# kensho-technologies/pyctcdecode

Measured on AMD Instinct MI355X. Metric: logit-frames/sec (whole node) at beam=100, V=1024, 4-gram LM, higher is better.
Workload: dtype f64

## Files before the change

### include/ctcdec.h

```cpp
#ifndef CTCDEC_H
#define CTCDEC_H

#include <stddef.h>
#include <stdint.h>

#ifdef __cplusplus
extern "C" {
#endif

typedef struct ctcdec_decoder ctcdec_decoder;
typedef struct ctcdec_result ctcdec_result;

enum ctcdec_status {
  CTCDEC_OK = 0,
  CTCDEC_ERR_ARG = -1,
  CTCDEC_ERR_IO = -2,
  CTCDEC_ERR_DEVICE = -3,
  CTCDEC_ERR_LIMIT = -4,
  CTCDEC_ERR_INTERNAL = -5
};

enum ctcdec_dtype { CTCDEC_F32 = 0, CTCDEC_F64 = 1, CTCDEC_F16 = 2, CTCDEC_BF16 = 3 };

#define CTCDEC_MAX_BEAM_WIDTH 256
#define CTCDEC_MAX_LM_ORDER 6
#define CTCDEC_MAX_VOCAB 65535
#define CTCDEC_MAX_LMS 4

typedef struct ctcdec_params {
  int32_t beam_width;
  int32_t prune_history;
  int32_t n_best;
  int32_t want_lm_state;
  double beam_prune_logp;
  double token_min_logp;
  double hotword_weight;
  double alpha;
  double beta;
  double unk_score_offset;
  double log_base_change;
  int32_t lm_score_boundary;
  int32_t first_frame;
  int32_t texts_only;
  int32_t token_frames;
} ctcdec_params;

enum ctcdec_token_logp { CTCDEC_TOKEN_LOGP_MEAN = 2, CTCDEC_TOKEN_LOGP_MIN = 3, CTCDEC_TOKEN_LOGP_MAX = 4 };

typedef struct ctcdec_lm_state {
  int32_t length;
  uint32_t words[CTCDEC_MAX_LM_ORDER - 1];
  float backoff[CTCDEC_MAX_LM_ORDER - 1];
} ctcdec_lm_state;

int ctcdec_create(const char* labels_blob, const int64_t* labels_off, int32_t n_labels,
                  int32_t is_bpe, int32_t device, ctcdec_decoder** out);
void ctcdec_destroy(ctcdec_decoder* dec);

int ctcdec_lm_load_arpa(ctcdec_decoder* dec, const char* path, int32_t* order_out);

int ctcdec_lm_save_flat(const ctcdec_decoder* dec, const char* path);
int ctcdec_lm_load_flat(ctcdec_decoder* dec, const char* path, int32_t* order_out);

int ctcdec_lm_load_kenlm(ctcdec_decoder* dec, const char* path, int32_t* order_out);
int ctcdec_is_kenlm_binary(const char* path);
int ctcdec_arpa_to_kenlm_binary(const char* arpa_path, const char* out_path, float probing_multiplier);

int ctcdec_lm_set_unigrams(ctcdec_decoder* dec, int32_t has_unigrams, const char* blob,
                           const int64_t* off, int64_t n_unigrams, int64_t* n_kept_out);

int ctcdec_lm_share(ctcdec_decoder* dst, const ctcdec_decoder* src);

int ctcdec_lm_clone(ctcdec_decoder* dst, const ctcdec_decoder* src);

int ctcdec_lm_share_multi(ctcdec_decoder* dst, const ctcdec_decoder* const* srcs, int32_t n);
int ctcdec_lm_set_params(ctcdec_decoder* dec, int32_t k , double alpha, double beta,
                         double unk_score_offset, int32_t lm_score_boundary);
int ctcdec_lm_count(const ctcdec_decoder* dec, int32_t* n_out);

int ctcdec_lm_prefix_flags(const ctcdec_decoder* dec, const char* str_utf8, int64_t len,
                           uint32_t* flags_out);

int ctcdec_lm_word_index(const ctcdec_decoder* dec, const char* word_utf8, int64_t len,
                         uint32_t* index_out);
int ctcdec_lm_word_string(const ctcdec_decoder* dec, uint32_t index, const char** str_out,
                          int64_t* len_out);

int ctcdec_lm_start_state(const ctcdec_decoder* dec, int32_t begin_sentence, ctcdec_lm_state* out);
int ctcdec_lm_base_score(const ctcdec_decoder* dec, const ctcdec_lm_state* in, uint32_t word_index,
                         ctcdec_lm_state* out, float* log10_prob_out);

int ctcdec_set_hotwords(ctcdec_decoder* dec, const char* blob, const int64_t* off, int64_t n_words);

int ctcdec_set_hotword_sets(ctcdec_decoder* dec, const char* blob, const int64_t* off, int64_t n_words,
                            const int64_t* set_off, int32_t n_sets, const double* set_weight,
                            const int32_t* utt_set, int32_t n_utts);

int ctcdec_decode_batch(ctcdec_decoder* dec, const void* const* utt_logits,
                        const int32_t* utt_frames, int32_t n_utts, int32_t dtype, int32_t is_device,
                        const ctcdec_params* params, const ctcdec_lm_state* start_states,
                        ctcdec_result** out);

typedef struct ctcdec_beam_in {
  double logit_score;
  double raw_lm_score;
  ctcdec_lm_state lm_state;
  int32_t last_char;
  int32_t partial_start;
  int32_t partial_end_frame;
  int32_t reserved;
  int64_t text_begin, text_end;
  int64_t partial_begin, partial_end;
  const ctcdec_lm_state* more_states;
} ctcdec_beam_in;
int ctcdec_decode_stream_batch(ctcdec_decoder* dec, const void* const* utt_logits,
                               const int32_t* utt_frames, int32_t n_streams, int32_t dtype,
                               int32_t is_device, const ctcdec_params* params,
                               const int32_t* first_frame ,
                               const ctcdec_beam_in* beams, const int64_t* beam_off ,
                               const char* text_blob, int32_t force_next_word, int32_t is_end,
                               ctcdec_result** out);

typedef struct ctcdec_stream ctcdec_stream;
int ctcdec_stream_open(ctcdec_decoder* dec, int32_t n_streams, const ctcdec_lm_state* start_states, ctcdec_stream** out);
int ctcdec_stream_push(ctcdec_stream* st, const void* const* chunk_logits, const int32_t* chunk_frames, int32_t dtype,
                       int32_t is_device, const ctcdec_params* params, const int32_t* first_frame,
                       int32_t force_next_word, int32_t is_end, int32_t want_result, ctcdec_result** out);
int ctcdec_stream_read(ctcdec_stream* st, const ctcdec_params* params, ctcdec_result** out);
int ctcdec_stream_import(ctcdec_stream* st, const ctcdec_beam_in* beams, const int64_t* beam_off ,
                         const char* text_blob, int64_t text_bytes);
int ctcdec_stream_frames(const ctcdec_stream* st, int64_t* frames_out);
int ctcdec_stream_ledger_bytes(const ctcdec_stream* st, int64_t* bytes_out);
void ctcdec_stream_close(ctcdec_stream* st);

int32_t ctcdec_result_num_utts(const ctcdec_result* r);
int32_t ctcdec_result_num_beams(const ctcdec_result* r, int32_t utt);
int ctcdec_result_text(const ctcdec_result* r, int32_t utt, int32_t beam, const char** str_out,
                       int64_t* len_out);
int ctcdec_result_scores(const ctcdec_result* r, int32_t utt, int32_t beam, double* logit_score,
                         double* lm_score);
int ctcdec_result_frames(const ctcdec_result* r, int32_t utt, int32_t beam, int32_t* n_words,
                         const int32_t** word_off, const int32_t** start, const int32_t** end);
int ctcdec_result_lm_state(const ctcdec_result* r, int32_t utt, int32_t beam, ctcdec_lm_state* out);
int ctcdec_result_lm_state_of(const ctcdec_result* r, int32_t utt, int32_t beam, int32_t k,
                              ctcdec_lm_state* out);
typedef struct ctcdec_packed {
  int64_t n_utts, n_beams, n_words;
  const int64_t* beam_off;
  const char* text_blob;
  const int64_t* text_off;
  const double* logit_score;
  const double* lm_score;
  const int64_t* word_cnt_off;
  const int32_t* word_byte_off;
  const int32_t* word_start;
  const int32_t* word_end;
  const ctcdec_lm_state* lm_state;
  const char* partial_blob;
  const int64_t* partial_off;
  const int32_t* src_beam;
  const int32_t* last_char;
  const int32_t* partial_start;
  const int32_t* partial_end;
  const double* raw_lm_score;
} ctcdec_packed;
int ctcdec_result_pack(ctcdec_result* r, ctcdec_packed* out);
int ctcdec_result_texts(ctcdec_result* r, const char** blob_out, const int64_t** off_out, int64_t* n_out);
int ctcdec_result_texts_joined(ctcdec_result* r, char sep, const char** blob_out, int64_t* bytes_out, int64_t* n_out);
int ctcdec_result_text_blocks(ctcdec_result* r, const char** pool_out, const int64_t** off_out, const int64_t** len_out,
                              int64_t* n_out);

int ctcdec_result_token_frames(ctcdec_result* r, const int64_t** tok_off, const int32_t** label, const int32_t** start,
                               const int32_t** end, int64_t* n_tokens);

int ctcdec_result_token_logp(ctcdec_result* r, const double** logp, int64_t* n_tokens);

typedef struct ctcdec_alignment ctcdec_alignment;
int ctcdec_align_batch(ctcdec_decoder* dec, const void* const* utt_logits, const int32_t* utt_frames, int32_t n_utts,
                       int32_t dtype, int32_t is_device, const int32_t* targets, const int64_t* target_off, int32_t fold,
                       int64_t bp_budget, ctcdec_alignment** out);
int ctcdec_alignment_paths(const ctcdec_alignment* a, const int64_t** path_off, const int32_t** path, const double** score,
                           int64_t* n_utts);
int ctcdec_alignment_tokens(const ctcdec_alignment* a, const int64_t** tok_off, const int32_t** label, const int32_t** start,
// ... 23 lines not shown
```

### pyctcdecode_amd/_binding.py

```python
from __future__ import annotations

import ctypes as C
import os
from typing import List, Optional, Sequence

import numpy as np

_HERE = os.path.dirname(os.path.abspath(__file__))
LIB_PATH = os.path.join(_HERE, "libctcdec.so")

MAX_CTX = 5


class Params(C.Structure):
    _fields_ = [
        ("beam_width", C.c_int32),
        ("prune_history", C.c_int32),
        ("n_best", C.c_int32),
        ("want_lm_state", C.c_int32),
        ("beam_prune_logp", C.c_double),
        ("token_min_logp", C.c_double),
        ("hotword_weight", C.c_double),
        ("alpha", C.c_double),
        ("beta", C.c_double),
        ("unk_score_offset", C.c_double),
        ("log_base_change", C.c_double),
        ("lm_score_boundary", C.c_int32),
        ("first_frame", C.c_int32),
        ("texts_only", C.c_int32),
        ("token_frames", C.c_int32),
    ]


class LmState(C.Structure):
    _fields_ = [("length", C.c_int32), ("words", C.c_uint32 * MAX_CTX), ("backoff", C.c_float * MAX_CTX)]


class Packed(C.Structure):
    _fields_ = [
        ("n_utts", C.c_int64),
        ("n_beams", C.c_int64),
        ("n_words", C.c_int64),
        ("beam_off", C.POINTER(C.c_int64)),
        ("text_blob", C.c_void_p),
        ("text_off", C.POINTER(C.c_int64)),
        ("logit_score", C.POINTER(C.c_double)),
        ("lm_score", C.POINTER(C.c_double)),
        ("word_cnt_off", C.POINTER(C.c_int64)),
        ("word_byte_off", C.POINTER(C.c_int32)),
        ("word_start", C.POINTER(C.c_int32)),
        ("word_end", C.POINTER(C.c_int32)),
        ("lm_state", C.POINTER(LmState)),
        ("partial_blob", C.c_void_p),
        ("partial_off", C.POINTER(C.c_int64)),
        ("src_beam", C.POINTER(C.c_int32)),
        ("last_char", C.POINTER(C.c_int32)),
        ("partial_start", C.POINTER(C.c_int32)),
        ("partial_end", C.POINTER(C.c_int32)),
        ("raw_lm_score", C.POINTER(C.c_double)),
    ]


class BeamIn(C.Structure):
    _fields_ = [
        ("logit_score", C.c_double),
        ("raw_lm_score", C.c_double),
        ("lm_state", LmState),
        ("last_char", C.c_int32),
        ("partial_start", C.c_int32),
        ("partial_end_frame", C.c_int32),
        ("reserved", C.c_int32),
        ("text_begin", C.c_int64),
        ("text_end", C.c_int64),
        ("partial_begin", C.c_int64),
        ("partial_end", C.c_int64),
        ("more_states", C.POINTER(LmState)),
    ]


_VP = C.c_void_p
_PROTOS = {
    "ctcdec_create": (C.c_int, [C.c_char_p, C.POINTER(C.c_int64), C.c_int32, C.c_int32, C.c_int32, C.POINTER(_VP)]),
    "ctcdec_destroy": (None, [_VP]),
    "ctcdec_lm_load_arpa": (C.c_int, [_VP, C.c_char_p, C.POINTER(C.c_int32)]),
    "ctcdec_lm_save_flat": (C.c_int, [_VP, C.c_char_p]),
    "ctcdec_lm_load_flat": (C.c_int, [_VP, C.c_char_p, C.POINTER(C.c_int32)]),
    "ctcdec_lm_load_kenlm": (C.c_int, [_VP, C.c_char_p, C.POINTER(C.c_int32)]),
    "ctcdec_is_kenlm_binary": (C.c_int, [C.c_char_p]),
    "ctcdec_arpa_to_kenlm_binary": (C.c_int, [C.c_char_p, C.c_char_p, C.c_float]),
    "ctcdec_lm_set_unigrams": (C.c_int, [_VP, C.c_int32, C.c_char_p, C.POINTER(C.c_int64), C.c_int64,
                                         C.POINTER(C.c_int64)]),
    "ctcdec_lm_share": (C.c_int, [_VP, _VP]),
    "ctcdec_lm_clone": (C.c_int, [_VP, _VP]),
    "ctcdec_lm_share_multi": (C.c_int, [_VP, C.POINTER(_VP), C.c_int32]),
    "ctcdec_lm_set_params": (C.c_int, [_VP, C.c_int32, C.c_double, C.c_double, C.c_double, C.c_int32]),
    "ctcdec_lm_count": (C.c_int, [_VP, C.POINTER(C.c_int32)]),
    "ctcdec_lm_prefix_flags": (C.c_int, [_VP, C.c_char_p, C.c_int64, C.POINTER(C.c_uint32)]),
    "ctcdec_lm_word_index": (C.c_int, [_VP, C.c_char_p, C.c_int64, C.POINTER(C.c_uint32)]),
    "ctcdec_lm_word_string": (C.c_int, [_VP, C.c_uint32, C.POINTER(_VP), C.POINTER(C.c_int64)]),
    "ctcdec_lm_start_state": (C.c_int, [_VP, C.c_int32, C.POINTER(LmState)]),
    "ctcdec_lm_base_score": (C.c_int, [_VP, C.POINTER(LmState), C.c_uint32, C.POINTER(LmState),
                                       C.POINTER(C.c_float)]),
    "ctcdec_set_hotwords": (C.c_int, [_VP, C.c_char_p, C.POINTER(C.c_int64), C.c_int64]),
    "ctcdec_set_hotword_sets": (C.c_int, [_VP, C.c_char_p, C.POINTER(C.c_int64), C.c_int64, C.POINTER(C.c_int64), C.c_int32,
                                          C.POINTER(C.c_double), C.POINTER(C.c_int32), C.c_int32]),
    "ctcdec_decode_batch": (C.c_int, [_VP, C.POINTER(_VP), C.POINTER(C.c_int32), C.c_int32, C.c_int32, C.c_int32,
                                      C.POINTER(Params), C.POINTER(LmState), C.POINTER(_VP)]),
    "ctcdec_decode_stream_batch": (C.c_int, [_VP, C.POINTER(_VP), C.POINTER(C.c_int32), C.c_int32, C.c_int32, C.c_int32,
                                             C.POINTER(Params), C.POINTER(C.c_int32), C.POINTER(BeamIn),
                                             C.POINTER(C.c_int64), C.c_char_p, C.c_int32, C.c_int32, C.POINTER(_VP)]),
    "ctcdec_stream_open": (C.c_int, [_VP, C.c_int32, C.POINTER(LmState), C.POINTER(_VP)]),
    "ctcdec_stream_push": (C.c_int, [_VP, C.POINTER(_VP), C.POINTER(C.c_int32), C.c_int32, C.c_int32, C.POINTER(Params),
                                     C.POINTER(C.c_int32), C.c_int32, C.c_int32, C.c_int32, C.POINTER(_VP)]),
    "ctcdec_stream_read": (C.c_int, [_VP, C.POINTER(Params), C.POINTER(_VP)]),
    "ctcdec_stream_import": (C.c_int, [_VP, C.POINTER(BeamIn), C.POINTER(C.c_int64), C.c_char_p, C.c_int64]),
    "ctcdec_stream_frames": (C.c_int, [_VP, C.POINTER(C.c_int64)]),
    "ctcdec_stream_ledger_bytes": (C.c_int, [_VP, C.POINTER(C.c_int64)]),
    "ctcdec_stream_close": (None, [_VP]),
    "ctcdec_result_num_utts": (C.c_int32, [_VP]),
    "ctcdec_result_num_beams": (C.c_int32, [_VP, C.c_int32]),
    "ctcdec_result_text": (C.c_int, [_VP, C.c_int32, C.c_int32, C.POINTER(_VP), C.POINTER(C.c_int64)]),
    "ctcdec_result_scores": (C.c_int, [_VP, C.c_int32, C.c_int32, C.POINTER(C.c_double), C.POINTER(C.c_double)]),
    "ctcdec_result_frames": (C.c_int, [_VP, C.c_int32, C.c_int32, C.POINTER(C.c_int32),
                                       C.POINTER(C.POINTER(C.c_int32)), C.POINTER(C.POINTER(C.c_int32)),
                                       C.POINTER(C.POINTER(C.c_int32))]),
    "ctcdec_result_lm_state": (C.c_int, [_VP, C.c_int32, C.c_int32, C.POINTER(LmState)]),
    "ctcdec_frame_survivors": (C.c_int, [_VP, _VP, C.c_int32, C.c_int32, C.c_int32, C.c_double, C.c_int32,
                                         C.POINTER(C.c_int32), C.POINTER(C.c_int32), C.POINTER(C.c_double)]),
    "ctcdec_result_lm_state_of": (C.c_int, [_VP, C.c_int32, C.c_int32, C.c_int32, C.POINTER(LmState)]),
    "ctcdec_result_pack": (C.c_int, [_VP, C.POINTER(Packed)]),
    "ctcdec_result_texts": (C.c_int, [_VP, C.POINTER(C.c_void_p), C.POINTER(C.POINTER(C.c_int64)), C.POINTER(C.c_int64)]),
    "ctcdec_result_texts_joined": (C.c_int, [_VP, C.c_char, C.POINTER(C.c_void_p), C.POINTER(C.c_int64), C.POINTER(C.c_int64)]),
    "ctcdec_result_text_blocks": (C.c_int, [_VP, C.POINTER(C.c_void_p), C.POINTER(C.POINTER(C.c_int64)),
                                           C.POINTER(C.POINTER(C.c_int64)), C.POINTER(C.c_int64)]),
    "ctcdec_result_token_frames": (C.c_int, [_VP, C.POINTER(C.POINTER(C.c_int64)), C.POINTER(C.POINTER(C.c_int32)),
                                            C.POINTER(C.POINTER(C.c_int32)), C.POINTER(C.POINTER(C.c_int32)),
                                            C.POINTER(C.c_int64)]),
    "ctcdec_result_token_logp": (C.c_int, [_VP, C.POINTER(C.POINTER(C.c_double)), C.POINTER(C.c_int64)]),
    "ctcdec_align_batch": (C.c_int, [_VP, C.POINTER(_VP), C.POINTER(C.c_int32), C.c_int32, C.c_int32, C.c_int32,
                                     C.POINTER(C.c_int32), C.POINTER(C.c_int64), C.c_int32, C.c_int64, C.POINTER(_VP)]),
    "ctcdec_alignment_paths": (C.c_int, [_VP, C.POINTER(C.POINTER(C.c_int64)), C.POINTER(C.POINTER(C.c_int32)),
                                         C.POINTER(C.POINTER(C.c_double)), C.POINTER(C.c_int64)]),
    "ctcdec_alignment_tokens": (C.c_int, [_VP, C.POINTER(C.POINTER(C.c_int64)), C.POINTER(C.POINTER(C.c_int32)),
                                          C.POINTER(C.POINTER(C.c_int32)), C.POINTER(C.POINTER(C.c_int32)),
                                          C.POINTER(C.POINTER(C.c_double)), C.POINTER(C.c_int64)]),
    "ctcdec_alignment_timing": (C.c_int, [_VP, C.POINTER(C.c_double), C.POINTER(C.c_int32)]),
    "ctcdec_alignment_free": (None, [_VP]),
    "ctcdec_result_timing": (C.c_int, [_VP, C.POINTER(C.c_double)]),
    "ctcdec_result_beam_kernel": (C.c_int, [_VP]),
    "ctcdec_device": (C.c_int, []),
    "ctcdec_result_free": (None, [_VP]),
    "ctcdec_profile_phases": (C.c_int, [_VP, C.c_int32, C.POINTER(C.c_uint64), C.c_int32]),
    "ctcdec_last_error": (C.c_char_p, []),
    "ctcdec_version": (C.c_char_p, []),
}
MAX_BEAM_WIDTH = 256
EXPORTED_SYMBOLS = tuple(_PROTOS)


class NativeError(RuntimeError):
    pass


class Library:

    def __init__(self, path: str = LIB_PATH):
        if not os.path.exists(path):
            raise ImportError(
                "%s is missing: build the HIP extension first (python -c 'import __graft_entry__ as g; "
                "g.build()'). pyctcdecode_amd has no CPU fallback." % path
            )
        self.path = path
        try:
            import torch
        except ImportError:
            pass
        self.dll = C.CDLL(path)
        for name, (res, args) in _PROTOS.items():
            fn = getattr(self.dll, name)
            fn.restype = res
            fn.argtypes = args

    def check(self, rc: int) -> None:
        if rc == 0:
            return
        msg = (self.dll.ctcdec_last_error() or b"").decode("utf-8", "replace")
        if rc == -1:
            raise ValueError(msg)
        if rc == -2:
            raise OSError(msg)
        if rc == -4:
            raise NotImplementedError(msg)
        raise NativeError("libctcdec error %d: %s" % (rc, msg))


_LIB: Optional[Library] = None
_PYTEXTS = None


def _pytexts():
    global _PYTEXTS
    if _PYTEXTS is None:
        path = os.path.join(_HERE, "_pytexts.so")
        _PYTEXTS = False
        if os.path.exists(path):
            try:
                dll = C.PyDLL(path)
                dll.ctcdec_py_split_texts.restype = C.py_object
                dll.ctcdec_py_split_texts.argtypes = [C.c_void_p, C.c_int64, C.c_int64, C.c_char]
                dll.ctcdec_py_texts_from_blocks.restype = C.py_object
                dll.ctcdec_py_texts_from_blocks.argtypes = [C.c_void_p, C.POINTER(C.c_int64), C.POINTER(C.c_int64), C.c_int64]
                dll.ctcdec_py_output_beams.restype = C.py_object
                dll.ctcdec_py_output_beams.argtypes = [C.py_object, C.c_int64, C.POINTER(C.c_int64), C.POINTER(C.c_int64), C.c_void_p,
                                                       C.POINTER(C.c_double), C.POINTER(C.c_double), C.POINTER(C.c_int64),
                                                       C.POINTER(C.c_int32), C.POINTER(C.c_int32), C.py_object, C.py_object]
                dll.ctcdec_py_lm_beams.restype = C.py_object
                dll.ctcdec_py_lm_beams.argtypes = [C.py_object, C.c_int64, C.POINTER(C.c_int64), C.POINTER(C.c_int64), C.c_void_p,
                                                   C.POINTER(C.c_int64), C.c_void_p, C.POINTER(C.c_int32), C.py_object,
                                                   C.POINTER(C.c_int64), C.POINTER(C.c_int32), C.POINTER(C.c_int32),
                                                   C.POINTER(C.c_int32), C.POINTER(C.c_int32), C.POINTER(C.c_double),
                                                   C.POINTER(C.c_double), C.py_object]
                _PYTEXTS = dll
            except (OSError, AttributeError):
                _PYTEXTS = False
    return _PYTEXTS


def texts_of(lib: "Library", res) -> Optional[list]:
    dll = _pytexts()
    if not dll:
        return None
    pool, off, ln, n = C.c_void_p(), C.POINTER(C.c_int64)(), C.POINTER(C.c_int64)(), C.c_int64()
    lib.check(lib.dll.ctcdec_result_text_blocks(res, C.byref(pool), C.byref(off), C.byref(ln), C.byref(n)))
    if n.value == 0:
        return []
    return dll.ctcdec_py_texts_from_blocks(pool, off, ln, n.value)


def output_beams(cls, pk: "Packed", states: Optional[list], frames_of=None) -> Optional[list]:
    dll = _pytexts()
    if not dll:
        return None
    return dll.ctcdec_py_output_beams(cls, pk.n_utts, pk.beam_off, pk.text_off, pk.text_blob, pk.logit_score, pk.lm_score,
                                      pk.word_cnt_off, pk.word_start, pk.word_end, states, frames_of)


def lm_beams(cls, n_streams: int, pk: "Packed", labels: list, frames_of=None) -> Optional[list]:
    dll = _pytexts()
    if not dll:
        return None
    return dll.ctcdec_py_lm_beams(cls, n_streams, pk.beam_off, pk.text_off, pk.text_blob, pk.partial_off, pk.partial_blob,
                                  pk.last_char, labels, pk.word_cnt_off, pk.word_start, pk.word_end, pk.partial_start,
                                  pk.partial_end, pk.logit_score, pk.lm_score, frames_of)


def split_texts(blob_ptr, nbytes: int, n: int, sep: bytes):
    dll = _pytexts()
    if dll:
        return dll.ctcdec_py_split_texts(blob_ptr, nbytes, n, sep)
    return C.string_at(blob_ptr, nbytes).decode("utf-8").split(sep.decode("ascii"))


def get_library() -> Library:
    global _LIB
    if _LIB is None:
        _LIB = Library()
    return _LIB


def pack_strings(strings: Sequence[str]):
    enc = [s.encode("utf-8") for s in strings]
    off = np.zeros(len(enc) + 1, dtype=np.int64)
    if enc:
        off[1:] = np.cumsum([len(e) for e in enc])
    blob = b"".join(enc)
    return blob, off


def off_ptr(off: np.ndarray):
    return off.ctypes.data_as(C.POINTER(C.c_int64))
```

### pyctcdecode_amd/csrc/api.cpp

```cpp
#include <math.h>
#include <cmath>
#include <stdio.h>
#include <stdlib.h>
#include <string.h>

#include <algorithm>
#include <atomic>
#include <chrono>
#include <condition_variable>
#include <functional>
#include <mutex>
#include <memory>
#include <string>
#include <thread>
#include <utility>
#include <vector>

#include "../../include/ctcdec.h"
#include "backend.h"
#include "beam_core.h"
#include "beam_wave.h"
#include "host_tables.h"

using namespace ctc;

static thread_local std::string g_err;
static std::mutex g_device_mu;
static int fail(int code, const std::string& msg) {
  g_err = msg;
  return code;
}

namespace {

template <bool HOST>
struct Buf {
  void* p = nullptr;
  size_t cap = 0;
  Buf() = default;
  Buf(const Buf&) = delete;
  Buf& operator=(const Buf&) = delete;
  Buf(Buf&& o) noexcept : p(std::exchange(o.p, nullptr)), cap(std::exchange(o.cap, 0)) {}
  Buf& operator=(Buf&& o) noexcept {
    std::swap(p, o.p);
    std::swap(cap, o.cap);
    return *this;
  }
  ~Buf() { drop(); }
  int ensure(size_t bytes, std::string* err) {
    if (bytes <= cap && p) return 0;
    drop();
    const size_t want = HOST ? bytes + bytes / 4 + 4096 : bytes + bytes / 8 + 256;
    p = HOST ? be::alloc_host(want, err) : be::alloc(want, err);
    if (!p) return -1;
    cap = want;
    return 0;
  }
  void drop() {
    if (p) HOST ? be::release_host(p) : be::release(p);
    p = nullptr;
    cap = 0;
  }
};
using DevBuf = Buf<false>;
using HostBuf = Buf<true>;

template <class T>
int upload(DevBuf& b, const std::vector<T>& v, std::string* err) {
  size_t bytes = std::max<size_t>(sizeof(T) * v.size(), 16);
  if (b.ensure(bytes, err)) return -1;
  if (!v.empty() && be::h2d(b.p, v.data(), sizeof(T) * v.size(), err)) return -1;
  return 0;
}

struct BeamResult {
  std::string text;
  std::vector<int32_t> word_off, start, end;
  double logit = 0, lm = 0;
  ctcdec_lm_state state;
  std::vector<ctcdec_lm_state> xstates;
  std::string partial;
  int32_t src = -1, last_char = -1, pstart = -1, pend = -1;
  double raw_lm = 0;
  std::vector<int32_t> tok;
};

struct StreamIn {
  const int32_t* first_frame;
  const ctcdec_beam_in* beams;
  const int64_t* beam_off;
  const char* text_blob;
  int32_t fold, eos;
};

}

class ReplayPool {
 public:
  explicit ReplayPool(int n) {
    for (int i = 0; i < n; ++i) workers_.emplace_back([this] { loop(); });
  }
  ~ReplayPool() {
    {
      std::lock_guard<std::mutex> g(m_);
      stop_ = true;
    }
    cv_.notify_all();
    for (auto& t : workers_) t.join();
  }
  int size() const { return (int)workers_.size(); }
  void run(int32_t n, int32_t chunk, const std::function<void(int32_t, int32_t)>& fn) {
    {
      std::lock_guard<std::mutex> g(m_);
      fn_ = &fn;
      n_ = n;
      chunk_ = chunk;
      next_.store(0);
      pending_ = (int)workers_.size();
      ++epoch_;
    }
    cv_.notify_all();
    work();
    std::unique_lock<std::mutex> g(m_);
    done_.wait(g, [this] { return pending_ == 0; });
    fn_ = nullptr;
  }

 private:
  void work() {
    for (;;) {
      int32_t u0 = next_.fetch_add(chunk_);
      if (u0 >= n_) return;
      (*fn_)(u0, std::min(n_, u0 + chunk_));
    }
  }
  void loop() {
    uint64_t seen = 0;
    for (;;) {
      {
        std::unique_lock<std::mutex> g(m_);
        cv_.wait(g, [&] { return stop_ || epoch_ != seen; });
        if (stop_) return;
        seen = epoch_;
      }
      work();
      {
        std::lock_guard<std::mutex> g(m_);
        if (--pending_ == 0) done_.notify_one();
      }
    }
  }
  std::vector<std::thread> workers_;
  std::mutex m_;
  std::condition_variable cv_, done_;
  const std::function<void(int32_t, int32_t)>* fn_ = nullptr;
  std::atomic<int32_t> next_{0};
  int32_t n_ = 0, chunk_ = 1;
  int pending_ = 0;
  uint64_t epoch_ = 0;
  bool stop_ = false;
};

struct ctcdec_decoder {
  std::unique_ptr<ReplayPool> replay_pool;
  HostAlphabet alpha;
  std::shared_ptr<HostLM> lm_ptr = std::make_shared<HostLM>();
  HostLM& lm_ref() { return *lm_ptr; }
  const HostLM& lm_ref() const { return *lm_ptr; }
  bool has_lm = false;
  std::unique_ptr<HostMulti> multi;
  double x_alpha[MAX_LMS] = {0}, x_beta[MAX_LMS] = {0}, x_unk[MAX_LMS] = {0};
  int32_t x_boundary[MAX_LMS] = {0};
  int n_lms() const { return multi ? (int)multi->lms.size() : 1; }
  int hist_order() const { return multi ? multi->order : lm_ptr->order; }
  HostHotwords hot;
  bool tables_dirty = true, hot_dirty = true;
  struct HotSets {
    bool armed = false;
    std::vector<std::vector<std::string>> words;
    std::vector<double> weight;
    std::vector<int32_t> utt_set;
    bool built = false;
    std::vector<HostHotwords> sets;
  };
  HotSets hot_next, hot_call;
  DevBuf d_hsets, d_htab, d_htok, d_hutt;
  HostBuf h_hot;
  DevBuf d_tok, d_tok_hot, d_uni, d_pref, d_hot;
  DevBuf d_xuni[MAX_LMS - 1], d_winfo[MAX_LMS], w_xstate, w_impx;
  HostBuf h_xstate;
  DevBuf w_logits, w_ptrs, w_row0, w_rowsum, w_isprob, w_scnt, w_sid, w_slp, w_flags, w_text, w_emit, w_toff,
      w_eoff, w_start, w_out, w_nout, w_status, w_tok, w_head, w_prof, w_imp, w_impoff, w_ff, w_cold, w_pay, w_tscr, w_tsoff, w_tpool,
      d_toktext, d_tokbytes, w_slow, w_order, w_side, w_truns, w_tlogp, w_tmiss, w_ledrow;
  DevBuf w_alse, w_alab, w_apath, w_atok, w_atlp, w_ascore, w_abp, w_autts;
  bool slicing = false;
  uint32_t max_label_bytes = 1;
  bool arenas_worst_case = false;
  HostBuf h_tok, h_out, h_small, h_truns;
  int dense_calls = 0;
  HostBuf h_stage;
  size_t stage_used = 0;
  bool profile = false;
  unsigned long long prof[N_PROF] = {0};
};

template <class T>
static int upload_staged(ctcdec_decoder* dec, DevBuf& b, const std::vector<T>& v, std::string* err) {
  const size_t bytes = sizeof(T) * v.size();
  const size_t room = dec->h_stage.p ? dec->h_stage.cap - dec->stage_used : 0;
  if (bytes == 0 || bytes > room) return upload(b, v, err);
  if (b.ensure(std::max<size_t>(bytes, 16), err)) return -1;
  char* src = (char*)dec->h_stage.p + dec->stage_used;
  memcpy(src, v.data(), bytes);
  dec->stage_used += (bytes + 63) & ~(size_t)63;
  return be::h2d_async(b.p, src, bytes, err);
}

struct HotCallScope {
  ctcdec_decoder* dec;
  explicit HotCallScope(ctcdec_decoder* d) : dec(d) {
    if (!dec) return;
    dec->hot_call = std::move(dec->hot_next);
    dec->hot_next = ctcdec_decoder::HotSets();
  }
  ~HotCallScope() {
    if (dec) dec->hot_call = ctcdec_decoder::HotSets();
  }
};

static void build_hot_sets(ctcdec_decoder::HotSets& h) {
  if (h.built) return;
  h.sets.resize(h.words.size());
  for (size_t k = 0; k < h.words.size(); ++k) h.sets[k].build_table(h.words[k]);
  bool none = false;
  for (int32_t& s : h.utt_set) {
    if (s < 0) {
      s = (int32_t)h.words.size();
      none = true;
    }
  }
  if (none) {
    h.sets.emplace_back();
    h.weight.push_back(0.0);
  }
  h.built = true;
}

static const HostHotwords& import_hot(const ctcdec_decoder* dec, int64_t u) {
  const ctcdec_decoder::HotSets& h = dec->hot_call;
  return h.armed ? h.sets[(size_t)h.utt_set[(size_t)u]] : dec->hot;
}

static int upload_hot_sets(ctcdec_decoder* dec, be::BeamArgs* ba, std::string* err) {
  ctcdec_decoder::HotSets& h = dec->hot_call;
  build_hot_sets(h);
  const size_t K = h.sets.size(), V = dec->alpha.labels.size(), n = h.utt_set.size();
  std::vector<size_t> toff(K + 1, 0);
  for (size_t k = 0; k < K; ++k) toff[k + 1] = toff[k] + h.sets[k].table.size();
  const size_t b_sets = K * sizeof(HotSet), b_utt = n * sizeof(int32_t), b_tab = toff[K] * sizeof(HotEntry);
  const size_t o_utt = (b_sets + 63) & ~(size_t)63, o_tab = (o_utt + b_utt + 63) & ~(size_t)63;
  if (dec->d_hsets.ensure(std::max<size_t>(b_sets, 16), err) || dec->d_hutt.ensure(std::max<size_t>(b_utt, 16), err) ||
      dec->d_htab.ensure(std::max<size_t>(b_tab, 16), err) || dec->d_htok.ensure(std::max<size_t>(K * V * sizeof(TokHot), 16), err) ||
      dec->h_hot.ensure(o_tab + b_tab + 64, err))
    return -1;
  char* stage = (char*)dec->h_hot.p;
  HotSet* hs = (HotSet*)stage;
  for (size_t k = 0; k < K; ++k) {
    const HostHotwords& w = h.sets[k];
    hs[k].hot = w.table.empty() ? nullptr : (const HotEntry*)dec->d_htab.p + toff[k];
    hs[k].hot_mask = w.mask;
    hs[k].tok_hot = (const TokHot*)dec->d_htok.p + k * V;
    hs[k].weight = h.weight[k];
    if (!w.table.empty()) memcpy(stage + o_tab + toff[k] * sizeof(HotEntry), w.table.data(), w.table.size() * sizeof(HotEntry));
  }
  memcpy(stage + o_utt, h.utt_set.data(), b_utt);
  if (be::h2d_async(dec->d_hsets.p, stage, b_sets, err) || be::h2d_async(dec->d_hutt.p, stage + o_utt, b_utt, err) ||
      (b_tab && be::h2d_async(dec->d_htab.p, stage + o_tab, b_tab, err)))
    return -1;
  ba->hot_sets = (const HotSet*)dec->d_hsets.p;
  ba->utt_hot = (const int32_t*)dec->d_hutt.p;
  ba->n_hot_sets = (int32_t)K;
  return 0;
}

// ... 421 lines not shown
        if (br != BR_APPEND && opener != NONE) {
          tk[opener * 3 + 1] = toks[k].wstart;
          opener = NONE;
        }
        if (br == BR_BOUNDARY || br == BR_APPEND) {
          last = tk.size() / 3;
          if (br == BR_BOUNDARY) opener = last;
          tk.push_back((int32_t)tok);
          tk.push_back(br == BR_APPEND ? toks[k].wstart - 1 : -1);
          tk.push_back(-1);
        }
      }
    }
    if (br == BR_BOUNDARY) {
      close_word(toks[k].wstart, toks[k].wend, true);
      text += d->alpha.clean[tok];
    } else if (br == BR_SPACE) {
      close_word(toks[k].wstart, toks[k].wend, true);
    } else if (br == BR_APPEND) {
      text += d->alpha.labels[tok];
    } else if (br == BR_FINAL) {
      close_word(toks[k].wstart, toks[k].wend, true);
    } else if (br == BR_IMPORT && st) {
      const ctcdec_beam_in& in = st->beams[imp0 + tok];
      r->src = (int32_t)tok;
      text.assign(st->text_blob + in.text_begin, (size_t)(in.text_end - in.text_begin));
      if (!text.empty()) text.push_back(' ');
      open = text.size();
      text.append(st->text_blob + in.partial_begin, (size_t)(in.partial_end - in.partial_begin));
    }
  }
  if (want_tok) {
    if (last != NONE) tk[last * 3 + 2] = open_e;
    if (opener != NONE) tk[opener * 3 + 1] = open_s;
  }
  r->partial.assign(text, open, std::string::npos);
  text.resize(open);
  if (!text.empty() && text.back() == ' ') text.pop_back();
  r->word_off.push_back((int32_t)text.size());
}

static void fill_result(const OutBeam& ob, const LmState* xs, int K, BeamResult* r) {
  r->logit = ob.logit_score;
  r->lm = ob.lm_score;
  export_lm_state(ob.state, &r->state);
  if (xs) {
    r->xstates.resize((size_t)(K - 1));
    for (int x = 0; x < K - 1; ++x) export_lm_state(xs[x], &r->xstates[(size_t)x]);
  }
  r->last_char = ob.last_char == NO_CHAR ? -1 : (int32_t)ob.last_char;
  r->pstart = ob.pstart;
  r->pend = ob.pend;
  r->raw_lm = ob.raw_lm;
}

static_assert(LOGP_MEAN == CTCDEC_TOKEN_LOGP_MEAN && LOGP_MIN == CTCDEC_TOKEN_LOGP_MIN && LOGP_MAX == CTCDEC_TOKEN_LOGP_MAX, "token_logp.h");
static int32_t logp_fold(const ctcdec_params* p) {
  return p && p->token_frames >= LOGP_MEAN && p->token_frames <= LOGP_MAX ? p->token_frames : 0;
}

using Clock = std::chrono::steady_clock;
static double ms(Clock::time_point a, Clock::time_point b) { return std::chrono::duration<double, std::milli>(b - a).count(); }
static size_t dtype_size(int32_t dtype) { return dtype == CTCDEC_F32 ? 4 : dtype == CTCDEC_F64 ? 8 : 2; }

enum LmStateErr { LM_STATE_OK = 0, LM_STATE_LENGTH, LM_STATE_WORD };
static LmStateErr copy_lm_state(const ctcdec_lm_state& in, size_t n_words, LmState* out) {
  memset(out, 0, sizeof(*out));
  if (in.length < 0 || in.length > MAX_CTX) return LM_STATE_LENGTH;
  out->len = in.length;
  for (int j = 0; j < out->len; ++j) {
    if (in.words[j] >= n_words) return LM_STATE_WORD;
    out->words[j] = in.words[j];
    out->backoff[j] = in.backoff[j];
  }
  return LM_STATE_OK;
}

typedef std::function<int(std::string*)> AfterLaunch;
struct DecodeMode {
  const StreamIn* stream = nullptr;
  ctcdec_stream* rs = nullptr;
  bool want_result = true;
  const AfterLaunch* after_launch = nullptr;
};
static int decode_impl(ctcdec_decoder* dec, const void* const* utt_logits, const int32_t* utt_frames, int32_t n_utts,
                       int32_t dtype, int32_t is_device, const ctcdec_params* p, const ctcdec_lm_state* start_states,
                       const DecodeMode& mode, ctcdec_result** out);
static int decode_host_sliced(ctcdec_decoder* dec, const void* const* utt_logits, const int32_t* utt_frames, int32_t n_utts,
                              int32_t dtype, const ctcdec_params* p, const ctcdec_lm_state* start_states, int n_slices,
                              ctcdec_result** out);
static int host_slices_wanted(const ctcdec_decoder* dec, const int32_t* utt_frames, int32_t n_utts, int32_t dtype);

int ctcdec_decode_batch(ctcdec_decoder* dec, const void* const* utt_logits, const int32_t* utt_frames,
                        int32_t n_utts, int32_t dtype, int32_t is_device, const ctcdec_params* p,
                        const ctcdec_lm_state* start_states, ctcdec_result** out) {
  HotCallScope hot_scope(dec);
  if (dec && p && out && !is_device && !dec->hot_call.armed && !logp_fold(p) && n_utts > 0 && utt_logits && utt_frames && dtype >= CTCDEC_F32 && dtype <= CTCDEC_BF16) {
    const int n_slices = host_slices_wanted(dec, utt_frames, n_utts, dtype);
    if (n_slices >= 2) {
      const int rc = decode_host_sliced(dec, utt_logits, utt_frames, n_utts, dtype, p, start_states, n_slices, out);
      if (rc != 1) return rc;
    }
  }
  return decode_impl(dec, utt_logits, utt_frames, n_utts, dtype, is_device, p, start_states, DecodeMode(), out);
}

int ctcdec_decode_stream_batch(ctcdec_decoder* dec, const void* const* utt_logits, const int32_t* utt_frames,
                               int32_t n_streams, int32_t dtype, int32_t is_device, const ctcdec_params* p,
                               const int32_t* first_frame, const ctcdec_beam_in* beams, const int64_t* beam_off,
                               const char* text_blob, int32_t force_next_word, int32_t is_end, ctcdec_result** out) {
  if (!first_frame || !beams || !beam_off || !text_blob) return fail(CTCDEC_ERR_ARG, "bad arguments");
  const StreamIn st{first_frame, beams, beam_off, text_blob, (force_next_word || is_end) ? 1 : 0, is_end ? 1 : 0};
  HotCallScope hot_scope(dec);
  return decode_impl(dec, utt_logits, utt_frames, n_streams, dtype, is_device, p, nullptr, DecodeMode{&st}, out);
}

static std::string build_import(const ctcdec_decoder* dec, const StreamIn& st, int64_t k, ImportBeam* m,
                                LmState* more , const HostHotwords& hot) {
  const ctcdec_beam_in& in = st.beams[k];
  memset(m, 0, sizeof(*m));
  if (in.text_end < in.text_begin || in.partial_end < in.partial_begin) return "bad beam text range";
  const char* t = st.text_blob + in.text_begin;
  const size_t tn = (size_t)(in.text_end - in.text_begin);
  const uint32_t n_hist = dec->has_lm ? (uint32_t)std::max(1, dec->hist_order() - 1) : 1u;
  uint64_t th = 0;
  std::vector<uint64_t> wh;
  uint32_t hw = 0;
  size_t a = 0;
  while (a < tn) {
    while (a < tn && t[a] == ' ') ++a;
    size_t b = a;
    while (b < tn && t[b] != ' ') ++b;
    if (b > a) {
      uint64_t h = hash_bytes(t + a, b - a);
      th = text_push(th, h);
      wh.push_back(h);
      uint32_t ml = 0, cp = 0;
      if (!hot.table.empty() && hot_lookup(hot.table.data(), hot.mask, h, &ml, &cp) && cp) ++hw;
    }
    a = b;
  }
  m->text_h = th;
  m->hw_cnt = hw;
  m->ring_cnt = (uint32_t)std::min<size_t>(n_hist, wh.size());
  for (uint32_t j = 0; j < m->ring_cnt; ++j) m->ring[j] = wh[wh.size() - 1 - j];
  const char* pp = st.text_blob + in.partial_begin;
  const size_t pn = (size_t)(in.partial_end - in.partial_begin);
  m->part_h = hash_bytes(pp, pn);
  m->plen = utf8_length(pp, pn);
  if (m->plen > 0xFFFF) return "partial word too long";
  uint32_t m2 = 0, wid = 0;
  if (pn > 0) {
    uint32_t fl = 0, w = 0;
    const std::vector<PrefixEntry>& ptab = dec->multi ? dec->multi->prefix_table : dec->lm_ref().prefix_table;
    const uint64_t pmask = dec->multi ? dec->multi->prefix_mask : dec->lm_ref().prefix_mask;
    if (dec->has_lm && prefix_lookup(ptab.data(), pmask, m->part_h, &w, &fl)) {
      m2 |= PF_ON_TABLE | (fl & PF_PARTIAL_MASK);
      wid = w;
    }
    uint32_t ml = 0, cp = 0;
    if (!hot.table.empty() && hot_lookup(hot.table.data(), hot.mask, m->part_h, &ml, &cp))
      m2 |= M2_HOT_ON | (cp ? M2_HOT_COMPLETE : 0u) | ((ml & 0xFFFFu) << 8);
  }
  m->m2 = m2;
  m->word_id = wid;
  if (in.last_char >= (int32_t)dec->alpha.labels.size()) return "last_char out of range";
  m->last_char = in.last_char < 0 ? NO_CHAR : (uint32_t)in.last_char;
  m->pstart = in.partial_start;
  m->pend = in.partial_end_frame;
  m->logit_score = in.logit_score;
  m->raw_lm = dec->has_lm ? in.raw_lm_score : 0.0;
  const char* const bad_state[] = {nullptr, "bad LM state in beam", "bad LM state word in beam"};
  if (dec->has_lm) {
    if (const LmStateErr e = copy_lm_state(in.lm_state, dec->lm_ref().words.size(), &m->state)) return bad_state[e];
  }
  if (dec->multi) {
    if (!in.more_states) return "beam lacks the states of the further language models";
    for (int x = 1; x < dec->n_lms(); ++x)
      if (const LmStateErr e = copy_lm_state(in.more_states[x - 1], dec->multi->lms[(size_t)x]->words.size(), &more[x - 1]))
        return bad_state[e];
  }
  return "";
}


struct PruneStage {
  ctcdec_decoder* dec = nullptr;
  const std::vector<const void*>* ptrs = nullptr;
  int32_t n_utts = 0, dtype = 0;
  int64_t R = 0;
  int V = 0;
  double token_min_logp = 0;
  bool resident = false;
  int max_surv = 0;
  uint32_t flags[8] = {0, 0, 0, 0, 0, 0, 0, 0};
  uint32_t surv_total = 0;
  Clock::time_point t_setup, t_queued, t_flags;
};

struct DecodeCall : DecodeMode {
  ctcdec_decoder* dec = nullptr;
  const ctcdec_params* p = nullptr;
  const void* const* utt_logits = nullptr;
  const int32_t* utt_frames = nullptr;
  const ctcdec_lm_state* start_states = nullptr;
  ctcdec_result** out = nullptr;
  int32_t n_utts = 0, dtype = 0, is_device = 0, fold = 0;
  int V = 0, K = 1, B = 0, n_best = 0;
  int64_t R = 0;
  std::vector<int64_t> row0;
  std::vector<const void*> ptrs;
  std::vector<uint64_t> toff, eoff;
  bool arenas_full = false;
  unsigned long long tok_cap = 0;
  size_t xstate_bytes = 0;
  bool device_texts = false, by_input = false, late_beam = false;
  be::BeamArgs ba{};
  PruneStage prune;
  uint32_t *n_out = nullptr, *status = nullptr;
  unsigned long long* heads_pinned = nullptr;
  unsigned long long head = 0;
  bool outgrown_redone = false;
  int32_t led = 0;
  std::vector<int64_t> led_rows;
  bool host_timing = false;
  Clock::time_point t_begin, t_launch, t_kernel, t_end;
  std::string err;
  std::unique_ptr<ctcdec_result> res;
  std::unique_lock<std::mutex> device_lock;
};

static int check_stream_tokens(DecodeCall& c) {
  const ctcdec_stream* rs = c.rs;
  if (c.p->token_frames != 0 && rs->has_import)
    return fail(CTCDEC_ERR_ARG, "token frames are not available to a stream that holds imported beams: their chains do not reach back");
  const bool first = rs->pushes == 0;
  if (c.fold && !first && rs->led_fold != c.fold)
    return fail(CTCDEC_ERR_ARG, rs->led_fold ? "a stream keeps the confidence fold its first chunk asked for"
                                             : "token confidences have to be asked for from a stream's first chunk on");
  c.led = first ? c.fold : rs->led_fold;
  if (c.led && !first)
    for (int32_t u = 0; u < c.n_utts; ++u)
      if ((int64_t)c.stream->first_frame[u] != (int64_t)rs->led_first[(size_t)u] + rs->frames[(size_t)u])
        return fail(CTCDEC_ERR_ARG, "stream " + std::to_string(u) + ": first_frame " + std::to_string(c.stream->first_frame[u]) +
                                        " does not continue the stream (token confidences: expected " +
                                        std::to_string((int64_t)rs->led_first[(size_t)u] + rs->frames[(size_t)u]) + ")");
  return CTCDEC_OK;
}

static int check_call(DecodeCall& c) {
  const ctcdec_params* p = c.p;
  if (!c.dec || !p || !c.out || c.n_utts < 0 || (c.n_utts > 0 && (!c.utt_logits || !c.utt_frames)))
    return fail(CTCDEC_ERR_ARG, "bad arguments");
  if (c.dtype < CTCDEC_F32 || c.dtype > CTCDEC_BF16) return fail(CTCDEC_ERR_ARG, "dtype must be f32, f64, f16 or bf16");
  if (p->beam_width < 1) return fail(CTCDEC_ERR_ARG, "beam_width must be >= 1");
  if (p->beam_width > CTCDEC_MAX_BEAM_WIDTH)
    return fail(CTCDEC_ERR_LIMIT, "beam_width above the supported maximum of 256");
  c.fold = logp_fold(p);
  if (c.fold && c.stream && !c.rs)
    return fail(CTCDEC_ERR_ARG, "token confidences are not available to streaming decodes whose beams the caller hands in");
  if (c.rs)
    if (int rc = check_stream_tokens(c)) return rc;
  c.t_begin = Clock::now();
  c.res.reset(new ctcdec_result());
  c.res->utts.resize((size_t)c.n_utts);
  return CTCDEC_OK;
}

static int open_call(DecodeCall& c) {
  ctcdec_decoder* dec = c.dec;
  const int32_t n_utts = c.n_utts;
  std::string& err = c.err;
  c.K = dec->has_lm ? dec->n_lms() : 1;
  if (dec->hot_call.armed) {
    if ((int32_t)dec->hot_call.utt_set.size() != n_utts) return fail(CTCDEC_ERR_ARG, "hot-word sets armed for another number of utterances");
    if (c.stream && !c.rs) build_hot_sets(dec->hot_call);
  }
  c.device_lock = std::unique_lock<std::mutex>(g_device_mu);
  if (be::bind_thread(&err)) return fail(CTCDEC_ERR_DEVICE, err);
  if (sync_tables(dec, &err)) return fail(CTCDEC_ERR_DEVICE, err);
  c.V = (int)dec->alpha.labels.size();
  c.B = c.p->beam_width;
  c.n_best = c.p->n_best > 0 ? std::min(c.p->n_best, c.B) : c.B;
  c.host_timing = getenv("CTCDEC_HOST_TIMING") != nullptr;
  dec->stage_used = 0;
  if (dec->h_stage.ensure((size_t)n_utts * (64 + sizeof(LmState) * (size_t)c.K) + 4096, &err)) return fail(CTCDEC_ERR_DEVICE, err);
  c.row0.assign((size_t)n_utts + 1, 0);
  for (int32_t u = 0; u < n_utts; ++u) {
    if (c.utt_frames[u] < 0) return fail(CTCDEC_ERR_ARG, "negative frame count");
    c.row0[(size_t)u + 1] = c.row0[(size_t)u] + c.utt_frames[u];
  }
  c.R = c.row0[(size_t)n_utts];
  return CTCDEC_OK;
}

static int stage_logits(DecodeCall& c) {
  ctcdec_decoder* dec = c.dec;
  std::string& err = c.err;
  const int32_t n_utts = c.n_utts;
  const size_t row_bytes = (size_t)c.V * dtype_size(c.dtype);
  c.ptrs.resize((size_t)n_utts);
  if (c.is_device) {
    for (int32_t u = 0; u < n_utts; ++u) c.ptrs[(size_t)u] = c.utt_logits[u];
  } else {
    if (dec->w_logits.ensure((size_t)std::max<int64_t>(c.R, 1) * row_bytes, &err)) return fail(CTCDEC_ERR_DEVICE, err);
    for (int32_t u = 0; u < n_utts;) {
      char* dst = (char*)dec->w_logits.p + (size_t)c.row0[(size_t)u] * row_bytes;
// ... 52 lines not shown
  for (int32_t u = 0; u <= n_utts; ++u) eo[(size_t)u] = (uint64_t)u * cap;
  if (upload(rs->eoff, eo, &err)) return fail(CTCDEC_ERR_DEVICE, err);
  rs->emit = std::move(grown);
  rs->emit_cap = cap;
  return CTCDEC_OK;
}

static int stage_imports(DecodeCall& c) {
  ctcdec_decoder* dec = c.dec;
  const StreamIn* stream = c.stream;
  std::string& err = c.err;
  const int32_t n_utts = c.n_utts;
  const int K = c.K;
  const int64_t n_imp_total = stream->beam_off[n_utts];
  std::vector<ImportBeam> imps((size_t)std::max<int64_t>(n_imp_total, 1));
  std::vector<LmState> imps_x(K > 1 ? (size_t)std::max<int64_t>(n_imp_total, 1) * (size_t)(K - 1) : 0);
  std::vector<int64_t> ioff(stream->beam_off, stream->beam_off + n_utts + 1);
  std::vector<int32_t> ff(stream->first_frame, stream->first_frame + n_utts);
  for (int32_t u = 0; u < n_utts; ++u) {
    int64_t cnt = ioff[(size_t)u + 1] - ioff[(size_t)u];
    if (cnt < 1 || cnt > beam_bucket(c.B))
      return fail(CTCDEC_ERR_ARG, "a stream must carry between 1 and beam-capacity beams");
    c.ba.max_import = std::max<int32_t>(c.ba.max_import, (int32_t)cnt);
    for (int64_t k = ioff[(size_t)u]; k < ioff[(size_t)u + 1]; ++k) {
      std::string e = build_import(dec, *stream, k, &imps[(size_t)k], K > 1 ? &imps_x[(size_t)k * (size_t)(K - 1)] : nullptr,
                                   import_hot(dec, u));
      if (!e.empty()) return fail(CTCDEC_ERR_ARG, e);
    }
  }
  if (upload(dec->w_imp, imps, &err) || upload(dec->w_impoff, ioff, &err) || upload(dec->w_ff, ff, &err))
    return fail(CTCDEC_ERR_DEVICE, err);
  if (K > 1 && upload(dec->w_impx, imps_x, &err)) return fail(CTCDEC_ERR_DEVICE, err);
  return CTCDEC_OK;
}

static int reserve_beam_workspace(DecodeCall& c) {
  ctcdec_decoder* dec = c.dec;
  std::string& err = c.err;
  const int32_t n_utts = c.n_utts;
  c.tok_cap = (unsigned long long)c.n_best * (unsigned long long)(c.R + 2 * (int64_t)n_utts);
  if (c.rs) {
    unsigned long long depth = 0;
    for (int32_t u = 0; u < n_utts; ++u)
      depth += (unsigned long long)(c.rs->frames[(size_t)u] + c.utt_frames[u] + c.rs->pushes + 3);
    c.tok_cap = c.want_result ? (unsigned long long)c.n_best * depth : 1ull;
  }
  if (dec->w_text.ensure(c.toff[(size_t)n_utts] * sizeof(TextNode), &err) ||
      (!c.rs && (dec->w_emit.ensure(c.eoff[(size_t)n_utts] * sizeof(EmitNode), &err) || upload_staged(dec, dec->w_eoff, c.eoff, &err))) ||
      upload_staged(dec, dec->w_toff, c.toff, &err) || dec->w_out.ensure((size_t)n_utts * c.n_best * sizeof(OutBeam), &err) ||
      dec->w_nout.ensure((size_t)n_utts * 4, &err) || dec->w_status.ensure((size_t)n_utts * 4, &err) ||
      dec->w_tok.ensure((size_t)std::max<unsigned long long>(c.tok_cap, 1) * sizeof(EmitNode), &err) ||
      dec->w_head.ensure(16, &err) || dec->w_cold.ensure((size_t)n_utts * 2 * COLD_STRIDE * sizeof(ColdRec), &err))
    return fail(CTCDEC_ERR_DEVICE, err);
  return CTCDEC_OK;
}

static int stage_start_states(DecodeCall& c) {
  ctcdec_decoder* dec = c.dec;
  const int K = c.K;
  c.xstate_bytes = K > 1 ? (size_t)c.n_utts * c.n_best * (size_t)(K - 1) * sizeof(LmState) : 0;
  if (!(c.stream && !c.rs) && dec->has_lm) {
    std::vector<LmState> st((size_t)c.n_utts * K);
    for (int32_t u = 0; u < c.n_utts; ++u) {
      for (int k = 0; k < K; ++k) {
        LmState& s = st[(size_t)u * K + k];
        const HostLM& lm = K > 1 ? *dec->multi->lms[(size_t)k] : dec->lm_ref();
        const ctcdec_lm_state* given = c.start_states ? &c.start_states[(size_t)u * K + k] : nullptr;
        if (!given || given->length < 0) {
          const bool boundary = k == 0 ? c.p->lm_score_boundary != 0 : dec->x_boundary[k] != 0;
          memset(&s, 0, sizeof(s));
          lm.start_state(boundary, &s);
        } else if (const LmStateErr e = copy_lm_state(*given, lm.words.size(), &s)) {
          return fail(CTCDEC_ERR_ARG, e == LM_STATE_LENGTH ? "LM start state too long" : "bad LM state word");
        }
      }
    }
    if (upload_staged(dec, dec->w_start, st, &c.err)) return fail(CTCDEC_ERR_DEVICE, c.err);
    c.ba.start_states = (const LmState*)dec->w_start.p;
  }
  if (c.xstate_bytes && dec->w_xstate.ensure(c.xstate_bytes, &c.err)) return fail(CTCDEC_ERR_DEVICE, c.err);
  return CTCDEC_OK;
}

static int reserve_device_texts(DecodeCall& c) {
  ctcdec_decoder* dec = c.dec;
  std::vector<uint64_t> soff((size_t)c.n_utts + 1, 0);
  for (int32_t u = 0; u < c.n_utts; ++u)
    soff[(size_t)u + 1] = soff[(size_t)u] + (((uint64_t)c.utt_frames[u] + 2) * (uint64_t)(dec->max_label_bytes + 1) + 15) / 16 * 16;
  if (dec->w_tscr.ensure((size_t)soff[(size_t)c.n_utts] + 16, &c.err) || dec->w_tpool.ensure((size_t)soff[(size_t)c.n_utts] + 16, &c.err) ||
      upload_staged(dec, dec->w_tsoff, soff, &c.err))
    return fail(CTCDEC_ERR_DEVICE, c.err);
  c.ba.text_scratch = (uint8_t*)dec->w_tscr.p;
  c.ba.text_soff = (const uint64_t*)dec->w_tsoff.p;
  c.ba.text_pool = (uint8_t*)dec->w_tpool.p;
  c.ba.text_pool_cap = soff[(size_t)c.n_utts];
  return CTCDEC_OK;
}

static int stage_longest_first(DecodeCall& c) {
  const int32_t* utt_frames = c.utt_frames;
  if (c.n_utts <= be::cus() * 2 || getenv("CTCDEC_NO_LPT_ORDER")) return CTCDEC_OK;
  bool ragged = false;
  for (int32_t u = 1; u < c.n_utts; ++u) ragged = ragged || utt_frames[u] != utt_frames[0];
  if (!ragged) return CTCDEC_OK;
  std::vector<int32_t> order((size_t)c.n_utts);
  for (int32_t u = 0; u < c.n_utts; ++u) order[(size_t)u] = u;
  std::stable_sort(order.begin(), order.end(), [&](int32_t x, int32_t y) { return utt_frames[x] > utt_frames[y]; });
  if (upload(c.dec->w_order, order, &c.err)) return fail(CTCDEC_ERR_DEVICE, c.err);
  c.ba.order = (const int32_t*)c.dec->w_order.p;
  return CTCDEC_OK;
}

static int fill_beam_args(DecodeCall& c) {
  ctcdec_decoder* dec = c.dec;
  const ctcdec_params* p = c.p;
  const StreamIn* stream = c.stream;
  ctcdec_stream* rs = c.rs;
  be::BeamArgs& ba = c.ba;
  device_tables(dec, &ba.tables);
  DecodeParams& dp = ba.params;
  memset(&dp, 0, sizeof(dp));
  dp.beam_width = c.B;
  dp.prune_history = p->prune_history ? 1 : 0;
  dp.n_best = c.n_best;
  dp.first_frame = p->first_frame;
  dp.beam_prune_logp = p->beam_prune_logp;
  dp.token_min_logp = p->token_min_logp;
  dp.hot_weight = p->hotword_weight;
  dp.alpha = p->alpha;
  dp.beta = p->beta;
  dp.unk = p->unk_score_offset;
  dp.log_base_change = p->log_base_change;
  dp.score_boundary = p->lm_score_boundary ? 1 : 0;
  dp.fold = stream ? stream->fold : 1;
  dp.eos = stream ? stream->eos : 1;
  dp.no_label_runs = getenv("CTCDEC_NO_LABEL_RUNS") != nullptr ? 1 : 0;
  c.device_texts = p->texts_only != 0 && p->token_frames == 0 && c.n_best == 1 && !stream && getenv("CTCDEC_HOST_REPLAY") == nullptr;
  dp.texts_only = c.device_texts ? 1 : 0;
  ba.n_utts = c.n_utts;
  ba.utt_row0 = (const int64_t*)dec->w_row0.p;
  ba.text_nodes = (TextNode*)dec->w_text.p;
  ba.text_off = (const uint64_t*)dec->w_toff.p;
  ba.out_xstates = c.xstate_bytes ? (LmState*)dec->w_xstate.p : nullptr;
  ba.out = (OutBeam*)dec->w_out.p;
  ba.out_stride = c.n_best;
  ba.n_out = (uint32_t*)dec->w_nout.p;
  ba.status = (uint32_t*)dec->w_status.p;
  ba.tok_pool = (EmitNode*)dec->w_tok.p;
  ba.tok_pool_head = (unsigned long long*)dec->w_head.p;
  ba.tok_pool_cap = c.tok_cap;
  ba.first_frames = stream ? (const int32_t*)dec->w_ff.p : nullptr;
  ba.cold = (ColdRec*)dec->w_cold.p;
  ba.want_out = 1;
  ba.total_rows = c.R;
  if (c.device_texts)
    if (int rc = reserve_device_texts(c)) return rc;
  if (int rc = stage_longest_first(c)) return rc;
  if (rs) {
    ba.emit_nodes = (EmitNode*)rs->emit.p;
    ba.emit_off = (const uint64_t*)rs->eoff.p;
    ba.imports = (const ImportBeam*)rs->carry.p;
    ba.import_xstates = c.K > 1 ? (const LmState*)rs->carry_x.p : nullptr;
    ba.resident_in = 1;
    ba.carry_out = (ImportBeam*)rs->carry.p;
    ba.carry_xstates = c.K > 1 ? (LmState*)rs->carry_x.p : nullptr;
    ba.sstate = (StreamState*)rs->sstate.p;
    ba.carry_stride = ctcdec_stream::CAP;
    ba.want_out = c.want_result ? 1 : 0;
  } else {
    ba.emit_nodes = (EmitNode*)dec->w_emit.p;
    ba.emit_off = (const uint64_t*)dec->w_eoff.p;
    if (stream) {
      ba.imports = (const ImportBeam*)dec->w_imp.p;
      ba.import_xstates = c.K > 1 ? (const LmState*)dec->w_impx.p : nullptr;
      ba.import_off = (const int64_t*)dec->w_impoff.p;
    }
  }
  if (dec->profile) {
    if (dec->w_prof.ensure(N_PROF * 8, &c.err) || be::zero(dec->w_prof.p, N_PROF * 8, &c.err)) return fail(CTCDEC_ERR_DEVICE, c.err);
    ba.prof = (unsigned long long*)dec->w_prof.p;
  }
  if (dec->w_flags.ensure(32, &c.err) || dec->w_head.ensure(16, &c.err)) return fail(CTCDEC_ERR_DEVICE, c.err);
  c.by_input = !rs && be::beam_kernel_depends_on_input(ba);
  c.late_beam = rs != nullptr || c.by_input;
  return CTCDEC_OK;
}

static int reserve_pay(DecodeCall& c) {
  be::BeamArgs& ba = c.ba;
  ba.pay = nullptr;
  ba.pay_stride = 0;
  if (be::wave_kernel_chosen(ba)) {
    ba.pay_stride = (uint64_t)wave_pay_stride(ba.params);
    if (c.dec->w_pay.ensure((size_t)c.n_utts * (size_t)ba.pay_stride * sizeof(PoolPay), &c.err)) return fail(CTCDEC_ERR_DEVICE, c.err);
    ba.pay = (PoolPay*)c.dec->w_pay.p;
  }
  return CTCDEC_OK;
}

static int run_beam(DecodeCall& c) {
  if (be::zero(c.dec->w_head.p, 16, &c.err)) return fail(CTCDEC_ERR_DEVICE, c.err);
  if (c.dec->hot_call.armed && !c.ba.hot_sets && upload_hot_sets(c.dec, &c.ba, &c.err)) return fail(CTCDEC_ERR_DEVICE, c.err);
  if (be::launch_beam(c.ba, &c.err)) return fail(CTCDEC_ERR_DEVICE, c.err);
  return CTCDEC_OK;
}

static int beam_ready(DecodeCall& c, int max_surv) {
  c.ba.surv_cnt = (const uint32_t*)c.dec->w_scnt.p;
  c.ba.surv_id = (const uint16_t*)c.dec->w_sid.p;
  c.ba.surv_lp = (const double*)c.dec->w_slp.p;
  c.ba.params.max_surv = max_surv;
  return c.by_input ? CTCDEC_OK : reserve_pay(c);
}

static int max_surv_bound(double token_min_logp, int V) {
  int max_surv = V;
  if (token_min_logp > log(1e-15)) {
    double bound = floor(exp(-token_min_logp)) + 2.0;
    if (bound < (double)V) max_surv = (int)bound;
  }
  return max_surv < 1 ? 1 : max_surv;
}

static int prune_stage(PruneStage& s, DecodeCall* beam) {
  ctcdec_decoder* dec = s.dec;
  std::string err;
  const int V = s.V;
  const size_t rows = (size_t)std::max<int64_t>(s.R, 1);
  uint32_t* flags = s.flags;
  s.max_surv = max_surv_bound(s.token_min_logp, V);
  for (int attempt = 0;; ++attempt) {
    const size_t max_surv = (size_t)s.max_surv;
    if (dec->w_rowsum.ensure(rows * 8, &err) || dec->w_isprob.ensure((size_t)s.n_utts * 4, &err) ||
        dec->w_scnt.ensure(rows * 4, &err) || dec->w_sid.ensure(rows * max_surv * 2, &err) ||
        dec->w_slp.ensure(rows * max_surv * 8, &err) || dec->w_flags.ensure(32, &err) || dec->w_slow.ensure(rows * 4, &err))
      return fail(CTCDEC_ERR_DEVICE, err);
    if (be::zero(dec->w_flags.p, 32, &err)) return fail(CTCDEC_ERR_DEVICE, err);
    be::PruneArgs pa;
    pa.utt_logits = (const void* const*)dec->w_ptrs.p;
    pa.utt_row0 = (const int64_t*)dec->w_row0.p;
    pa.n_utts = s.n_utts;
    pa.n_rows = s.R;
    pa.n_labels = V;
    pa.dtype = s.dtype;
    pa.token_min_logp = s.token_min_logp;
    pa.max_surv = s.max_surv;
    pa.row_sum = (double*)dec->w_rowsum.p;
    pa.utt_is_prob = (uint32_t*)dec->w_isprob.p;
    pa.surv_cnt = (uint32_t*)dec->w_scnt.p;
    pa.surv_id = (uint16_t*)dec->w_sid.p;
    pa.surv_lp = (double*)dec->w_slp.p;
    pa.overflow = (uint32_t*)dec->w_flags.p;
    pa.pass = 0;
    pa.row_base = 0;
    pa.slow_rows = (uint32_t*)dec->w_slow.p;
    const bool sliced = beam && dec->slicing;
    pa.utt_side = sliced ? (uint32_t*)dec->w_side.p : nullptr;
    pa.utt_sum = sliced ? (double*)((char*)dec->w_side.p + (((size_t)s.n_utts * 4 + 15) & ~(size_t)15)) : nullptr;
    pa.dense_hint = 0;
    if (beam && dec->dense_calls > 0 && !s.resident) {
      pa.dense_hint = 1;
      if (attempt == 0) --dec->dense_calls;
    }
    pa.rows_aligned16 = 1;
    pa.rows_aligned4 = 1;
    for (const void* q : *s.ptrs) {
      if (((uintptr_t)q & 15u) != 0) pa.rows_aligned16 = 0;
      if (((uintptr_t)q & 3u) != 0) pa.rows_aligned4 = 0;
    }
    if (beam)
      if (int rc = beam_ready(*beam, s.max_surv)) return rc;
    const bool early_beam = beam && !beam->late_beam;
    s.t_setup = Clock::now();
    if (be::launch_prune(pa, &err)) return fail(CTCDEC_ERR_DEVICE, err);
    if (early_beam)
      if (int rc = run_beam(*beam)) return rc;
    s.t_queued = Clock::now();
    if (be::d2h(flags, dec->w_flags.p, 32, &err)) return fail(CTCDEC_ERR_DEVICE, err);
    s.t_flags = Clock::now();
    s.surv_total = flags[4];
    if (beam && V <= 128 && s.R >= 1024 && (uint64_t)flags[3] * 2 > (uint64_t)s.R) dec->dense_calls = 16;
    if (flags[2]) {
      if (be::launch_sniff_exact(pa, &err) || be::d2h(flags, dec->w_flags.p, 16, &err)) return fail(CTCDEC_ERR_DEVICE, err);
    }
    if (flags[1]) {
      pa.pass = 1;
      if (be::zero(dec->w_flags.p, 4, &err) || be::zero((char*)dec->w_flags.p + 16, 4, &err)) return fail(CTCDEC_ERR_DEVICE, err);
      if (be::launch_prune(pa, &err)) return fail(CTCDEC_ERR_DEVICE, err);
      if (early_beam)
        if (int rc = run_beam(*beam)) return rc;
      if (be::d2h(flags, dec->w_flags.p, 32, &err)) return fail(CTCDEC_ERR_DEVICE, err);
      s.surv_total = flags[4];
    }
    if (!flags[0]) return CTCDEC_OK;
    if (s.max_surv == V) return fail(CTCDEC_ERR_INTERNAL, "survivor overflow at full vocabulary");
    s.max_surv = V;
  }
}

static int reserve_ledger(DecodeCall& c) {
  ctcdec_stream* rs = c.rs;
  std::string& err = c.err;
  const int32_t n = c.n_utts;
  const bool first = rs->pushes == 0;
  if (first) {
    rs->led_used.assign((size_t)n, 0);
    rs->led_first.assign(c.stream->first_frame, c.stream->first_frame + n);
  }
  uint64_t need_rows = 0, need_ent = 0;
  for (int32_t u = 0; u < n; ++u) {
    const uint64_t chunk = (uint64_t)c.utt_frames[u] * (uint64_t)c.prune.max_surv;
    if (chunk > UINT32_MAX || (uint64_t)rs->frames[(size_t)u] + (uint64_t)c.utt_frames[u] > UINT32_MAX)
      return fail(CTCDEC_ERR_LIMIT, "token confidences: a chunk of more than 2^32 survivor entries, or a stream of more than 2^32 frames");
    need_rows = std::max<uint64_t>(need_rows, (uint64_t)rs->frames[(size_t)u] + (uint64_t)c.utt_frames[u]);
    need_ent = std::max<uint64_t>(need_ent, rs->led_used[(size_t)u] + chunk);
  }
  if (need_rows > rs->led_row_cap || need_ent > rs->led_ent_cap || !rs->led_off.p) {
    const uint64_t row_cap = std::max<uint64_t>(std::max<uint64_t>(2 * need_rows, 2 * rs->led_row_cap), 1024);
    const uint64_t ent_cap = std::max<uint64_t>(std::max<uint64_t>(2 * need_ent, 2 * rs->led_ent_cap), 4096);
    DevBuf off, id, lp;
    if (off.ensure((size_t)n * (row_cap + 1) * 8, &err) || id.ensure((size_t)n * ent_cap * 2, &err) || lp.ensure((size_t)n * ent_cap * 8, &err))
      return fail(CTCDEC_ERR_DEVICE, err);
    for (int32_t u = 0; u < n && rs->led_off.p && !first; ++u) {
      const size_t rows = (size_t)rs->frames[(size_t)u], used = (size_t)rs->led_used[(size_t)u];
      if (be::d2d((char*)off.p + (size_t)u * (row_cap + 1) * 8, (const char*)rs->led_off.p + (size_t)u * (rs->led_row_cap + 1) * 8, (rows + 1) * 8, &err) ||
          (used && (be::d2d((char*)id.p + (size_t)u * ent_cap * 2, (const char*)rs->led_id.p + (size_t)u * rs->led_ent_cap * 2, used * 2, &err) ||
                    be::d2d((char*)lp.p + (size_t)u * ent_cap * 8, (const char*)rs->led_lp.p + (size_t)u * rs->led_ent_cap * 8, used * 8, &err))))
        return fail(CTCDEC_ERR_DEVICE, err);
    }
    rs->led_off = std::move(off);
    rs->led_id = std::move(id);
    rs->led_lp = std::move(lp);
    rs->led_row_cap = row_cap;
    rs->led_ent_cap = ent_cap;
  }
  if (first && be::zero((char*)rs->sstate.p + rs->sstate_bytes(), (size_t)n * 8 + 8, &err)) return fail(CTCDEC_ERR_DEVICE, err);
  rs->led_fold = c.led;
  return CTCDEC_OK;
}

static int append_ledger(DecodeCall& c) {
  ctcdec_stream* rs = c.rs;
  ctcdec_decoder* dec = c.dec;
  const int32_t n = c.n_utts;
  const uint32_t max_surv = (uint32_t)c.prune.max_surv;
#ifdef CTC_SIM
  const uint32_t* cnt = (const uint32_t*)dec->w_scnt.p;
  const uint16_t* sid = (const uint16_t*)dec->w_sid.p;
  const double* slp = (const double*)dec->w_slp.p;
  uint64_t* used_out = (uint64_t*)((char*)rs->sstate.p + rs->sstate_bytes());
  for (int32_t u = 0; u < n; ++u) {
    uint64_t* ro = (uint64_t*)rs->led_off.p + (size_t)u * (rs->led_row_cap + 1);
    uint16_t* did = (uint16_t*)rs->led_id.p + (size_t)u * rs->led_ent_cap;
    double* dlp = (double*)rs->led_lp.p + (size_t)u * rs->led_ent_cap;
    const size_t r0 = (size_t)rs->frames[(size_t)u];
    if (r0 == 0) ro[0] = 0;
    uint64_t base = ro[r0];
    for (int32_t t = 0; t < c.utt_frames[u]; ++t) {
      const size_t src = (size_t)c.row0[(size_t)u] + (size_t)t;
      const uint32_t k = ledger_row_count(cnt[src], max_surv);
      if (base + k > rs->led_ent_cap || r0 + (size_t)t + 1 > rs->led_row_cap) {
        used_out[n] = 1;
        break;
      }
      ledger_put_row(sid + src * max_surv, slp + src * max_surv, k, did + base, dlp + base);
      base += k;
      ro[r0 + (size_t)t + 1] = base;
    }
    used_out[u] = base;
  }
#else
  std::vector<uint32_t> r0((size_t)n);
  for (int32_t u = 0; u < n; ++u) r0[(size_t)u] = (uint32_t)rs->frames[(size_t)u];
  if (upload_staged(dec, dec->w_ledrow, r0, &c.err)) return fail(CTCDEC_ERR_DEVICE, c.err);
  be::LedgerAppendArgs la;
  la.n_streams = n;
  la.utt_row0 = (const int64_t*)dec->w_row0.p;
  la.surv_cnt = (const uint32_t*)dec->w_scnt.p;
  la.surv_id = (const uint16_t*)dec->w_sid.p;
  la.surv_lp = (const double*)dec->w_slp.p;
  la.max_surv = (int32_t)max_surv;
  la.led_row0 = (const uint32_t*)dec->w_ledrow.p;
  la.row_off = (uint64_t*)rs->led_off.p;
  la.id = (uint16_t*)rs->led_id.p;
  la.lp = (double*)rs->led_lp.p;
  la.row_cap = rs->led_row_cap;
  la.ent_cap = rs->led_ent_cap;
  la.used_out = (uint64_t*)((char*)rs->sstate.p + rs->sstate_bytes());
  la.overrun = la.used_out + n;
  if (be::launch_ledger_append(la, &c.err)) return fail(CTCDEC_ERR_DEVICE, c.err);
#endif
  return CTCDEC_OK;
}

static int prune_and_launch(DecodeCall& c) {
  PruneStage& s = c.prune;
  s = PruneStage{c.dec, &c.ptrs, c.n_utts, c.dtype, c.R, c.V, c.p->token_min_logp, c.rs != nullptr};
  s.t_setup = s.t_queued = s.t_flags = c.t_begin;
  if (int rc = prune_stage(s, &c)) return rc;
  if (c.by_input) {
    const double mean = c.R > 0 ? (double)s.surv_total / (double)c.R : 0.0;
    c.ba.surv_x16 = (int32_t)std::min(1.0e6, std::max(1.0, mean * 16.0 + 0.5));
    if (int rc = reserve_pay(c)) return rc;
  }
  if (c.led)
    if (int rc = reserve_ledger(c)) return rc;
  if (c.late_beam)
    if (int rc = run_beam(c)) return rc;
  return c.led && c.R > 0 ? append_ledger(c) : CTCDEC_OK;
}

static int redo_outgrown(DecodeCall& c) {
  ctcdec_decoder* dec = c.dec;
  std::string& err = c.err;
  const int32_t n_utts = c.n_utts;
  if (getenv("CTCDEC_ARENA_TRACE")) fprintf(stderr, "[ctcdec host] node arenas outgrown: beam stage redone with the worst case\n");
  dec->arenas_worst_case = true;
  c.arenas_full = true;
  c.outgrown_redone = true;
  size_arenas(c, true);
  if (dec->w_text.ensure(c.toff[(size_t)n_utts] * sizeof(TextNode), &err) ||
      dec->w_emit.ensure(c.eoff[(size_t)n_utts] * sizeof(EmitNode), &err) || upload(dec->w_toff, c.toff, &err) ||
      upload(dec->w_eoff, c.eoff, &err))
    return fail(CTCDEC_ERR_DEVICE, err);
  c.ba.text_nodes = (TextNode*)dec->w_text.p;
  c.ba.emit_nodes = (EmitNode*)dec->w_emit.p;
  c.ba.text_off = (const uint64_t*)dec->w_toff.p;
  c.ba.emit_off = (const uint64_t*)dec->w_eoff.p;
  if (be::zero(dec->w_head.p, 16, &err) || be::launch_beam(c.ba, &err) ||
      be::d2h(c.n_out, dec->w_nout.p, (size_t)n_utts * 4, &err) || be::d2h(c.status, dec->w_status.p, (size_t)n_utts * 4, &err) ||
      be::d2h(&c.head, dec->w_head.p, 8, &err))
    return fail(CTCDEC_ERR_DEVICE, err);
  return CTCDEC_OK;
}

static int refresh_stream_mirrors(DecodeCall& c) {
  ctcdec_stream* rs = c.rs;
  const size_t n = (size_t)c.n_utts;
  bool overrun = false;
  if (c.led) {
    rs->led_back.resize(2 * n + n + 1);
    if (be::d2h(rs->led_back.data(), rs->sstate.p, rs->sstate_bytes() + n * 8 + 8, &c.err)) return fail(CTCDEC_ERR_DEVICE, c.err);
    memcpy(rs->mirror.data(), rs->led_back.data(), rs->sstate_bytes());
    for (size_t u = 0; u < n; ++u) rs->led_used[u] = rs->led_back[2 * n + u];
    overrun = rs->led_back[3 * n] != 0;
  } else if (be::d2h(rs->mirror.data(), rs->sstate.p, rs->sstate_bytes(), &c.err)) {
    return fail(CTCDEC_ERR_DEVICE, c.err);
  }
  for (int32_t u = 0; u < c.n_utts; ++u) rs->frames[(size_t)u] += c.utt_frames[u];
  rs->pushes += 1;
  if (c.led) c.led_rows.assign(rs->frames.begin(), rs->frames.end());
  if (c.stream->eos) {
    for (auto& m : rs->mirror) {
      m.n_carry = 0;
      m.emit_next = 1;
      m.status = 0;
    }
    if (be::h2d(rs->sstate.p, rs->mirror.data(), (size_t)c.n_utts * sizeof(StreamState), &c.err)) return fail(CTCDEC_ERR_DEVICE, c.err);
    rs->has_import = false;
    std::fill(rs->frames.begin(), rs->frames.end(), 0);
    rs->pushes = 0;
    rs->led_fold = 0;
  }
  if (overrun) return fail(CTCDEC_ERR_INTERNAL, "survivor ledger: a chunk ran past the room reserved for it");
  return CTCDEC_OK;
}

static int collect_counters(DecodeCall& c) {
  ctcdec_decoder* dec = c.dec;
  std::string& err = c.err;
  const int32_t n_utts = c.n_utts;
  c.t_launch = Clock::now();
  if (dec->h_small.ensure((size_t)n_utts * 8 + 16, &err) ||
      dec->h_out.ensure((size_t)n_utts * c.n_best * sizeof(OutBeam), &err))
    return fail(CTCDEC_ERR_DEVICE, err);
  c.n_out = (uint32_t*)dec->h_small.p;
  c.status = c.n_out + n_utts;
  c.heads_pinned = (unsigned long long*)(c.status + n_utts);
  if (be::d2h_async(c.n_out, dec->w_nout.p, (size_t)n_utts * 4, &err) ||
      be::d2h_async(c.status, dec->w_status.p, (size_t)n_utts * 4, &err) || be::d2h_async(c.heads_pinned, dec->w_head.p, 16, &err) ||
      be::sync(&err))
    return fail(CTCDEC_ERR_DEVICE, err);
  c.head = c.heads_pinned[0];
  if (!c.arenas_full) {
    bool outgrown = false;
    for (int32_t u = 0; u < n_utts; ++u) outgrown = outgrown || (c.status[u] & (ST_TEXT_OVERFLOW | ST_EMIT_OVERFLOW)) != 0;
    if (outgrown)
      if (int rc = redo_outgrown(c)) return rc;
  }
  c.t_kernel = Clock::now();
  if (c.rs)
    if (int rc = refresh_stream_mirrors(c)) return rc;
  for (int32_t u = 0; u < n_utts; ++u)
    if (c.status[u] & ST_NO_BEAMS)
      return fail(CTCDEC_ERR_ARG, "max() arg is an empty sequence (utterance " + std::to_string(u) +
                                      ": no beam survived -- non-finite scores or a positive beam_prune_logp)");
  for (int32_t u = 0; u < n_utts; ++u)
    if (c.status[u]) return fail(CTCDEC_ERR_INTERNAL, "beam kernel status " + std::to_string(c.status[u]) +
                                                          " for utterance " + std::to_string(u));
  return CTCDEC_OK;
}

static int kernel_stats(DecodeCall& c) {
  ctcdec_result* res = c.res.get();
#ifndef CTC_SIM
  if (c.led && c.R > 0 && c.host_timing)
    fprintf(stderr, "[ctcdec host] survivor ledger: surv_ledger_append kernel %.4f ms, %zu bytes reserved\n", be::last_ledger_append_ms(),
            c.rs->led_bytes());
#endif
  be::last_timing(&res->ms[0], &res->ms[1]);
  res->beam_kernel = be::last_beam_kernel();
  if (c.dec->profile && be::d2h(c.dec->prof, c.dec->w_prof.p, N_PROF * 8, &c.err)) return fail(CTCDEC_ERR_DEVICE, c.err);
  return CTCDEC_OK;
}
static void close_call(DecodeCall& c) {
  c.t_end = Clock::now();
  c.res->ms[2] = ms(c.t_begin, c.t_end);
  *c.out = c.res.release();
}

static int finish_device_texts(DecodeCall& c) {
  ctcdec_result* res = c.res.get();
  std::string& err = c.err;
  unsigned long long heads[2] = {c.heads_pinned[0], c.heads_pinned[1]};
  if (c.outgrown_redone && be::d2h(heads, c.dec->w_head.p, 16, &err)) return fail(CTCDEC_ERR_DEVICE, err);
  res->device_texts = true;
  res->dev_out.resize((size_t)c.n_utts);
  res->dev_texts.resize((size_t)heads[1]);
  if (be::d2h(res->dev_out.data(), c.dec->w_out.p, (size_t)c.n_utts * sizeof(OutBeam), &err) ||
      (heads[1] && be::d2h(&res->dev_texts[0], c.dec->w_tpool.p, (size_t)heads[1], &err)))
    return fail(CTCDEC_ERR_DEVICE, err);
  for (int32_t u = 0; u < c.n_utts; ++u) {
    const OutBeam& ob = res->dev_out[(size_t)u];
    if (c.n_out[u] != 1 || (unsigned long long)ob.tok_off + ob.tok_cnt > heads[1]) return fail(CTCDEC_ERR_INTERNAL, "text pool range");
  }
  if (int rc = kernel_stats(c)) return rc;
  close_call(c);
  if (c.host_timing) {
    const PruneStage& s = c.prune;
    fprintf(stderr, "[ctcdec host] texts from the device: %llu bytes, native call %.3f ms (kernels %.3f + %.3f): setup %.3f, launches %.3f, "
                    "wait for the kernels %.3f, counters back %.3f, records + texts back %.3f\n", heads[1], res->ms[2], res->ms[0], res->ms[1],
            ms(c.t_begin, s.t_setup), ms(s.t_setup, s.t_queued), ms(s.t_queued, s.t_flags), ms(s.t_flags, c.t_kernel), ms(c.t_kernel, Clock::now()));
  }
  return CTCDEC_OK;
}

static int finish_stream_push(DecodeCall& c) {
  const ctcdec_result* res = c.res.get();
  if (int rc = kernel_stats(c)) return rc;
  close_call(c);
  if (c.host_timing)
    fprintf(stderr, "[ctcdec host] stream push: setup+prune+launch %.3f ms, wait beam kernel %.3f ms, total %.3f ms (prune kernel %.3f, beam kernel %.3f)\n",
            ms(c.t_begin, c.t_launch), ms(c.t_launch, c.t_kernel), ms(c.t_begin, Clock::now()), res->ms[0], res->ms[1]);
  return CTCDEC_OK;
}

static int stream_token_confidences(DecodeCall& c);
static int token_confidences(DecodeCall& c) {
  if (c.rs) return stream_token_confidences(c);
  ctcdec_decoder* dec = c.dec;
  ctcdec_result* res = c.res.get();
  std::string& err = c.err;
  const int max_surv = c.prune.max_surv;
  double logp_ms[3] = {0, 0, 0};
  auto t0 = Clock::now();
  if (c.R > (int64_t)UINT32_MAX) return fail(CTCDEC_ERR_LIMIT, "token confidences: more than 2^32 frames in one call");
  size_t nt = 0;
  for (const auto& beams : res->utts)
    for (const BeamResult& b : beams) nt += b.tok.size() / 3;
  if (dec->h_truns.ensure(std::max<size_t>(nt, 1) * sizeof(TokRun), &err)) return fail(CTCDEC_ERR_DEVICE, err);
  TokRun* runs = (TokRun*)dec->h_truns.p;
  size_t o = 0;
  for (int32_t u = 0; u < c.n_utts; ++u)
    for (const BeamResult& b : res->utts[(size_t)u]) {
      const int32_t* t = b.tok.data();
      for (size_t k = 0, n = b.tok.size() / 3; k < n; ++k, ++o, t += 3) {
        const int64_t s = (int64_t)t[1] - c.p->first_frame, e = (int64_t)t[2] - c.p->first_frame;
        if (t[0] < 0 || t[0] >= c.V || s < 0 || e <= s || e > c.utt_frames[u]) return fail(CTCDEC_ERR_INTERNAL, "token frames out of range");
        runs[o] = TokRun{(uint32_t)(c.row0[(size_t)u] + s), (uint32_t)(e - s), (uint32_t)t[0]};
      }
    }
  res->tk_logp.resize(nt);
  uint32_t missing = 0;
#ifdef CTC_SIM
  for (size_t i = 0; i < nt; ++i) {
    const uint32_t* cnt = (const uint32_t*)dec->w_scnt.p;
    const uint16_t* sid = (const uint16_t*)dec->w_sid.p;
    const double* slp = (const double*)dec->w_slp.p;
    missing += c.fold == LOGP_MEAN  ? token_logp_of<LOGP_MEAN>(runs[i], cnt, sid, slp, (uint32_t)max_surv, &res->tk_logp[i])
               : c.fold == LOGP_MIN ? token_logp_of<LOGP_MIN>(runs[i], cnt, sid, slp, (uint32_t)max_surv, &res->tk_logp[i])
                                    : token_logp_of<LOGP_MAX>(runs[i], cnt, sid, slp, (uint32_t)max_surv, &res->tk_logp[i]);
  }
  (void)t0;
#else
  if (nt) {
    if (dec->w_truns.ensure(nt * sizeof(TokRun), &err) || be::h2d(dec->w_truns.p, runs, nt * sizeof(TokRun), &err) ||
        dec->w_tlogp.ensure(nt * 8, &err) || dec->w_tmiss.ensure(16, &err) || be::zero(dec->w_tmiss.p, 16, &err))
      return fail(CTCDEC_ERR_DEVICE, err);
    be::TokenLogpArgs ta;
    ta.runs = (const TokRun*)dec->w_truns.p;
    ta.n_tokens = (int64_t)nt;
    ta.fold = c.fold;
    ta.surv_cnt = (const uint32_t*)dec->w_scnt.p;
    ta.surv_id = (const uint16_t*)dec->w_sid.p;
    ta.surv_lp = (const double*)dec->w_slp.p;
    ta.max_surv = max_surv;
    ta.out = (double*)dec->w_tlogp.p;
    ta.missing = (uint32_t*)dec->w_tmiss.p;
    auto t1 = Clock::now();
    if (be::launch_token_logp(ta, &err)) return fail(CTCDEC_ERR_DEVICE, err);
    if (c.host_timing) logp_ms[1] = be::last_token_logp_ms();
    auto t2 = Clock::now();
    if (be::d2h(res->tk_logp.data(), dec->w_tlogp.p, nt * 8, &err) || be::d2h(&missing, dec->w_tmiss.p, 4, &err))
      return fail(CTCDEC_ERR_DEVICE, err);
    logp_ms[0] = ms(t0, t1);
    logp_ms[2] = ms(t2, Clock::now());
  }
#endif
  if (missing)
    return fail(CTCDEC_ERR_INTERNAL, "token confidences: " + std::to_string(missing) + " token frames whose label is not among the frame's survivors");
  res->has_logp = true;
  if (c.host_timing)
    fprintf(stderr, "[ctcdec host] token confidences: %zu tokens, pack + upload %.3f ms, kernel %.3f ms, download %.3f ms\n", nt,
            logp_ms[0], logp_ms[1], logp_ms[2]);
  return CTCDEC_OK;
// ... 42 lines not shown
    be::LedgerLogpArgs ta;
    ta.runs = (const LedgerRun*)dec->w_truns.p;
    ta.n_tokens = (int64_t)nt;
    ta.fold = c.fold;
    ta.row_off = (const uint64_t*)rs->led_off.p;
    ta.id = (const uint16_t*)rs->led_id.p;
    ta.lp = (const double*)rs->led_lp.p;
    ta.row_cap = rs->led_row_cap;
    ta.ent_cap = rs->led_ent_cap;
    ta.out = (double*)dec->w_tlogp.p;
    ta.missing = (uint32_t*)dec->w_tmiss.p;
    if (be::launch_ledger_logp(ta, &err)) return fail(CTCDEC_ERR_DEVICE, err);
    if (c.host_timing) kernel_ms = be::last_ledger_logp_ms();
    if (be::d2h(res->tk_logp.data(), dec->w_tlogp.p, nt * 8, &err) || be::d2h(&missing, dec->w_tmiss.p, 4, &err))
      return fail(CTCDEC_ERR_DEVICE, err);
  }
#endif
  if (missing)
    return fail(CTCDEC_ERR_INTERNAL, "token confidences: " + std::to_string(missing) + " token frames whose label is not in the frame's ledger row");
  res->has_logp = true;
  if (c.host_timing)
    fprintf(stderr, "[ctcdec host] stream token confidences: %zu tokens, token_logp_ledger kernel %.3f ms, all of it %.3f ms\n", nt, kernel_ms,
            ms(t0, Clock::now()));
  return CTCDEC_OK;
}

static int finish_beams(DecodeCall& c) {
  ctcdec_decoder* dec = c.dec;
  ctcdec_result* res = c.res.get();
  std::string& err = c.err;
  const int32_t n_utts = c.n_utts;
  const int n_best = c.n_best, K = c.K;
  const unsigned long long head = c.head;
  const OutBeam* obs = (const OutBeam*)dec->h_out.p;
  if (be::d2h(dec->h_out.p, dec->w_out.p, (size_t)n_utts * n_best * sizeof(OutBeam), &err))
    return fail(CTCDEC_ERR_DEVICE, err);
  if (dec->h_tok.ensure((size_t)head * sizeof(EmitNode) + 16, &err)) return fail(CTCDEC_ERR_DEVICE, err);
  const EmitNode* toks = (const EmitNode*)dec->h_tok.p;
  if (head && be::d2h(dec->h_tok.p, dec->w_tok.p, (size_t)head * sizeof(EmitNode), &err))
    return fail(CTCDEC_ERR_DEVICE, err);
  const LmState* xst = nullptr;
  if (c.xstate_bytes) {
    if (dec->h_xstate.ensure(c.xstate_bytes, &err) || be::d2h(dec->h_xstate.p, dec->w_xstate.p, c.xstate_bytes, &err))
      return fail(CTCDEC_ERR_DEVICE, err);
    xst = (const LmState*)dec->h_xstate.p;
  }
  auto t_copy = Clock::now();
  if (int rc = kernel_stats(c)) return rc;
  for (int32_t u = 0; u < n_utts; ++u)
    for (uint32_t k = 0; k < c.n_out[u]; ++k) {
      const OutBeam& ob = obs[(size_t)u * n_best + k];
      if ((unsigned long long)ob.tok_off + ob.tok_cnt > head) return fail(CTCDEC_ERR_INTERNAL, "token pool range");
    }
  const bool want_tok = c.p->token_frames != 0;
  const StreamIn* stream = c.stream;
  res->has_tokens = want_tok;
  auto replay_range = [&](int32_t u0, int32_t u1) {
    for (int32_t u = u0; u < u1; ++u) {
      auto& beams = res->utts[(size_t)u];
      beams.resize(c.n_out[u]);
      for (uint32_t k = 0; k < c.n_out[u]; ++k) {
        const OutBeam& ob = obs[(size_t)u * n_best + k];
        BeamResult& r = beams[k];
        fill_result(ob, xst ? &xst[((size_t)u * n_best + k) * (size_t)(K - 1)] : nullptr, K, &r);
        replay(dec, toks + ob.tok_off, ob.tok_cnt, stream, stream ? stream->beam_off[u] : 0, &r, want_tok, (int32_t)ob.pad[0],
               (int32_t)ob.pad[1]);
      }
    }
  };
  if (head > 50000 && n_utts >= 16) {
    if (!dec->replay_pool) {
      unsigned want = 31u;
      if (const char* env = getenv("CTCDEC_REPLAY_THREADS")) want = (unsigned)std::max(0, atoi(env) - 1);
      const unsigned hw = std::max(1u, std::thread::hardware_concurrency());
      dec->replay_pool.reset(new ReplayPool((int)std::min(want, hw > 1 ? hw - 1 : 0u)));
    }
    const std::function<void(int32_t, int32_t)> job = replay_range;
    dec->replay_pool->run(n_utts, 4, job);
  } else {
    replay_range(0, n_utts);
  }
  if (c.fold)
    if (int rc = token_confidences(c)) return rc;
  close_call(c);
  if (c.host_timing)
    fprintf(stderr, "[ctcdec host] setup+launch %.3f ms, wait kernels %.3f ms, copy back %.3f ms (%llu tokens), replay %.3f ms\n",
            ms(c.t_begin, c.t_launch), ms(c.t_launch, c.t_kernel), ms(c.t_kernel, t_copy), head, ms(t_copy, c.t_end));
  return CTCDEC_OK;
}

static int decode_impl(ctcdec_decoder* dec, const void* const* utt_logits, const int32_t* utt_frames, int32_t n_utts,
                       int32_t dtype, int32_t is_device, const ctcdec_params* p, const ctcdec_lm_state* start_states,
                       const DecodeMode& mode, ctcdec_result** out) {
  DecodeCall c{mode, dec, p, utt_logits, utt_frames, start_states, out, n_utts, dtype, is_device};
  if (int rc = check_call(c)) return rc;
  if (n_utts == 0) {
    *out = c.res.release();
    return CTCDEC_OK;
  }
  if (int rc = open_call(c)) return rc;
  if (int rc = stage_logits(c)) return rc;
  c.arenas_full = c.rs != nullptr || dec->arenas_worst_case || getenv("CTCDEC_WORST_CASE_ARENAS") != nullptr;
  size_arenas(c, c.arenas_full);
  if (int rc = c.rs ? stage_resident_input(c) : c.stream ? stage_imports(c) : CTCDEC_OK) return rc;
  if (int rc = reserve_beam_workspace(c)) return rc;
  if (int rc = stage_start_states(c)) return rc;
  if (int rc = fill_beam_args(c)) return rc;
  if (int rc = prune_and_launch(c)) return rc;
  if (c.after_launch && *c.after_launch && (*c.after_launch)(&c.err)) return fail(CTCDEC_ERR_DEVICE, c.err);
  if (int rc = collect_counters(c)) return rc;
  return c.device_texts ? finish_device_texts(c) : c.want_result ? finish_beams(c) : finish_stream_push(c);
}

int ctcdec_stream_open(ctcdec_decoder* dec, int32_t n_streams, const ctcdec_lm_state* start_states, ctcdec_stream** out) {
  if (!dec || !out || n_streams < 1) return fail(CTCDEC_ERR_ARG, "bad arguments");
  std::string err;
  std::lock_guard<std::mutex> device_lock(g_device_mu);
  if (be::bind_thread(&err)) return fail(CTCDEC_ERR_DEVICE, err);
  std::unique_ptr<ctcdec_stream> st(new ctcdec_stream());
  st->dec = dec;
  st->n = n_streams;
  st->K = dec->has_lm ? dec->n_lms() : 1;
  if (start_states && dec->has_lm) st->start_states.assign(start_states, start_states + (size_t)n_streams * st->K);
  st->mirror.assign((size_t)n_streams, StreamState{0u, 1u, 0u, 0u});
  st->frames.assign((size_t)n_streams, 0);
  st->imp_off.assign((size_t)n_streams + 1, 0);
  if (st->carry.ensure((size_t)n_streams * ctcdec_stream::CAP * sizeof(ImportBeam), &err) ||
      (st->K > 1 && st->carry_x.ensure((size_t)n_streams * ctcdec_stream::CAP * (size_t)(st->K - 1) * sizeof(LmState), &err)) ||
      st->sstate.ensure((size_t)n_streams * (sizeof(StreamState) + 8) + 8, &err) ||
      be::h2d(st->sstate.p, st->mirror.data(), (size_t)n_streams * sizeof(StreamState), &err))
    return fail(CTCDEC_ERR_DEVICE, err);
  *out = st.release();
  return CTCDEC_OK;
}

int ctcdec_stream_push(ctcdec_stream* st, const void* const* chunk_logits, const int32_t* chunk_frames, int32_t dtype,
                       int32_t is_device, const ctcdec_params* params, const int32_t* first_frame, int32_t force_next_word,
                       int32_t is_end, int32_t want_result, ctcdec_result** out) {
  if (!st || !params || !chunk_frames) return fail(CTCDEC_ERR_ARG, "bad arguments");
  if ((want_result || is_end) && !out) return fail(CTCDEC_ERR_ARG, "a result is wanted but there is nowhere to put it");
  std::vector<int32_t> ff((size_t)st->n);
  const bool led = st->led_fold != 0 && st->pushes > 0;
  for (int32_t u = 0; u < st->n; ++u)
    ff[(size_t)u] = first_frame ? first_frame[u] : (int32_t)st->frames[(size_t)u] + (led ? st->led_first[(size_t)u] : 0);
  const StreamIn sin{ff.data(), st->has_import ? st->imp_beams.data() : nullptr, st->imp_off.data(), st->imp_blob.data(),
                     (force_next_word || is_end) ? 1 : 0, is_end ? 1 : 0};
  ctcdec_result* res = nullptr;
  HotCallScope hot_scope(st->dec);
  const int rc = decode_impl(st->dec, chunk_logits, chunk_frames, st->n, dtype, is_device, params,
                             st->start_states.empty() ? nullptr : st->start_states.data(),
                             DecodeMode{&sin, st, want_result != 0 || is_end != 0}, &res);
  if (rc != CTCDEC_OK) return rc;
  if (out) *out = res;
  else ctcdec_result_free(res);
  return CTCDEC_OK;
}

int ctcdec_stream_read(ctcdec_stream* st, const ctcdec_params* params, ctcdec_result** out) {
  if (!st || !params || !out) return fail(CTCDEC_ERR_ARG, "bad arguments");
  std::vector<const void*> ptrs((size_t)st->n, nullptr);
  std::vector<int32_t> zero((size_t)st->n, 0);
  return ctcdec_stream_push(st, ptrs.data(), zero.data(), CTCDEC_F32, 0, params, nullptr, 0, 0, 1, out);
}

int ctcdec_stream_import(ctcdec_stream* st, const ctcdec_beam_in* beams, const int64_t* beam_off, const char* text_blob,
                         int64_t text_bytes) {
  if (!st || !beams || !beam_off || !text_blob || text_bytes < 0) return fail(CTCDEC_ERR_ARG, "bad arguments");
  ctcdec_decoder* dec = st->dec;
  HotCallScope hot_scope(dec);
  if (dec->hot_call.armed) {
    if ((int32_t)dec->hot_call.utt_set.size() != st->n) return fail(CTCDEC_ERR_ARG, "hot-word sets armed for another number of streams");
    build_hot_sets(dec->hot_call);
  }
  std::string err;
  std::lock_guard<std::mutex> device_lock(g_device_mu);
  if (be::bind_thread(&err)) return fail(CTCDEC_ERR_DEVICE, err);
  if (sync_tables(dec, &err)) return fail(CTCDEC_ERR_DEVICE, err);
  const int K = st->K;
  const StreamIn sin{nullptr, beams, beam_off, text_blob, 0, 0};
  std::vector<ImportBeam> imps((size_t)st->n * ctcdec_stream::CAP);
  std::vector<LmState> imps_x(K > 1 ? imps.size() * (size_t)(K - 1) : 0);
  for (int32_t u = 0; u < st->n; ++u) {
    const int64_t cnt = beam_off[u + 1] - beam_off[u];
    if (cnt < 1 || cnt > ctcdec_stream::CAP) return fail(CTCDEC_ERR_ARG, "a stream must carry between 1 and 256 beams");
    for (int64_t k = 0; k < cnt; ++k) {
      const size_t slot = (size_t)u * ctcdec_stream::CAP + (size_t)k;
      std::string e = build_import(dec, sin, beam_off[u] + k, &imps[slot], K > 1 ? &imps_x[slot * (size_t)(K - 1)] : nullptr,
                                   import_hot(dec, u));
      if (!e.empty()) return fail(CTCDEC_ERR_ARG, e);
    }
  }
  for (int32_t u = 0; u < st->n; ++u) st->mirror[(size_t)u].n_carry = (uint32_t)(beam_off[u + 1] - beam_off[u]);
  if (be::h2d(st->carry.p, imps.data(), imps.size() * sizeof(ImportBeam), &err) ||
// ... 790 lines not shown
```

### pyctcdecode_amd/csrc/backend.h

```cpp
#pragma once
#include <stddef.h>
#include <stdint.h>

#include <string>

#include "beam_core.h"
#include "ctc_align.h"
#include "surv_ledger.h"
#include "token_logp.h"

namespace ctc {
namespace be {

const char* name();
int init(int device, std::string* err);
int bind_thread(std::string* err);
int current_device();
void* alloc(size_t bytes, std::string* err);
void release(void* p);
void* alloc_host(size_t bytes, std::string* err);
void release_host(void* p);
int h2d(void* dst, const void* src, size_t bytes, std::string* err);
int d2h(void* dst, const void* src, size_t bytes, std::string* err);
int d2d(void* dst, const void* src, size_t bytes, std::string* err);
int zero(void* dst, size_t bytes, std::string* err);
int sync(std::string* err);
int h2d_2d_overlapped(void* dst, size_t dpitch, const void* src, size_t spitch, size_t width, size_t height, std::string* err);
int d2h_async(void* dst, const void* src, size_t bytes, std::string* err);
int h2d_async(void* dst, const void* src, size_t bytes, std::string* err);
int cus();

struct PruneArgs {
  const void* const* utt_logits;
  const int64_t* utt_row0;
  int32_t n_utts;
  int64_t n_rows;
  int32_t n_labels;
  int32_t dtype;
  double token_min_logp;
  int32_t max_surv;
  double* row_sum;
  uint32_t* utt_is_prob;
  uint32_t* surv_cnt;
  uint16_t* surv_id;
  double* surv_lp;
  uint32_t* overflow;
  int32_t pass;
  int32_t rows_aligned16;
  int32_t rows_aligned4;
  int64_t row_base;
  uint32_t* slow_rows;
  uint32_t* utt_side;
  double* utt_sum;
  int32_t dense_hint;
  int32_t f32_np;
  const uint8_t* np_prog;
  const uint16_t* np_leaf;
  int32_t np_n_leaf;
  int32_t np_uniform8;
};
int launch_prune(const PruneArgs& a, std::string* err);
int launch_sniff_exact(const PruneArgs& a, std::string* err);

struct BeamArgs {
  DeviceTables tables;
  DecodeParams params;
  int32_t n_utts;
  const int64_t* utt_row0;
  const uint32_t* surv_cnt;
  const uint16_t* surv_id;
  const double* surv_lp;
  TextNode* text_nodes;
  EmitNode* emit_nodes;
  const uint64_t* text_off;
  const uint64_t* emit_off;
  const LmState* start_states;
  LmState* out_xstates;
  OutBeam* out;
  int32_t out_stride;
  uint32_t* n_out;
  uint32_t* status;
  EmitNode* tok_pool;
  unsigned long long* tok_pool_head;
  unsigned long long tok_pool_cap;
  unsigned long long* prof;
  const ImportBeam* imports;
  const LmState* import_xstates;
  const int64_t* import_off;
  const int32_t* first_frames;
  ColdRec* cold;
  PoolPay* pay;
  uint64_t pay_stride;
  int32_t max_import;
  ImportBeam* carry_out;
  LmState* carry_xstates;
  StreamState* sstate;
  int32_t carry_stride;
  int32_t want_out;
  uint8_t* text_scratch;
  const uint64_t* text_soff;
  uint8_t* text_pool;
  unsigned long long text_pool_cap;
  const int32_t* order;
  int32_t resident_in;
  int32_t surv_x16;
  int64_t total_rows;
  unsigned long long* wave_clock;
  int32_t prio_mode;
  unsigned long long* progress;
  unsigned long long total_frames;
  float inv_n_utts;
  const float* block_weight;
  const HotSet* hot_sets = nullptr;
  const int32_t* utt_hot = nullptr;
  int32_t n_hot_sets = 0;
};
int launch_beam(const BeamArgs& a, std::string* err);
bool wave_kernel_chosen(const BeamArgs& a);
bool beam_kernel_depends_on_input(const BeamArgs& a);

struct TokenLogpArgs {
  const TokRun* runs;
  int64_t n_tokens;
  int32_t fold;
  const uint32_t* surv_cnt;
  const uint16_t* surv_id;
  const double* surv_lp;
  int32_t max_surv;
  double* out;
  uint32_t* missing;
};
int launch_token_logp(const TokenLogpArgs& a, std::string* err);
double last_token_logp_ms();

struct LedgerAppendArgs {
  int32_t n_streams;
  const int64_t* utt_row0;
  const uint32_t* surv_cnt;
  const uint16_t* surv_id;
  const double* surv_lp;
  int32_t max_surv;
  const uint32_t* led_row0;
  uint64_t* row_off;
  uint16_t* id;
  double* lp;
  uint64_t row_cap, ent_cap;
  uint64_t* used_out;
  uint64_t* overrun;
};
int launch_ledger_append(const LedgerAppendArgs& a, std::string* err);
struct LedgerLogpArgs {
  const LedgerRun* runs;
  int64_t n_tokens;
  int32_t fold;
  const uint64_t* row_off;
  const uint16_t* id;
  const double* lp;
  uint64_t row_cap, ent_cap;
  double* out;
  uint32_t* missing;
};
int launch_ledger_logp(const LedgerLogpArgs& a, std::string* err);
double last_ledger_append_ms();
double last_ledger_logp_ms();

struct RowLseArgs {
  const void* const* utt_logits;
  const int64_t* utt_row0;
  const uint32_t* utt_is_prob;
  int32_t n_utts;
  int64_t n_rows;
  int32_t n_labels;
  int32_t dtype;
  double* lse;
};
int launch_row_lse(const RowLseArgs& a, std::string* err);
struct ViterbiArgs {
  const AlignUtt* utts;
  int32_t n_utts;
  int32_t n_labels;
  int32_t dtype;
  int32_t blank;
  int32_t fold;
  int32_t max_chunks;
  double clip_lo;
};
int launch_ctc_viterbi(const ViterbiArgs& a, std::string* err);
void align_timing_reset();
void align_timing(double* row_lse_ms, double* viterbi_ms);

void last_timing(double* prune_ms, double* beam_ms);
int last_beam_kernel();

}
}
```

### pyctcdecode_amd/csrc/backend_hip.hip

```cpp
#include <hip/hip_runtime.h>
#include <hip/hip_fp16.h>
#include <algorithm>
#include <type_traits>
#include <vector>
#include <math.h>
#include <stdio.h>
#include <stdlib.h>

#include "backend.h"
#include "beam_core.h"
#include "beam_wave.h"
#include "set_order.h"
#include "np_f32.h"
#include "set_order_small.h"
#include "np_sum.h"
#include "text_wave.h"
#include "wave_ops_hip.h"

namespace ctc {
namespace be {

static hipStream_t g_stream = nullptr;
static hipStream_t g_copy_stream = nullptr;
static hipEvent_t g_ev[3] = {nullptr, nullptr, nullptr};
static int g_device = -1;
static int g_cus = 256;
static bool g_timing_valid = false;

#define HIP_TRY(expr)                                                                    \
  do {                                                                                   \
    hipError_t e_ = (expr);                                                              \
    if (e_ != hipSuccess) {                                                              \
      if (err) *err = std::string(#expr) + ": " + hipGetErrorString(e_);                 \
      return -1;                                                                         \
    }                                                                                    \
  } while (0)

const char* name() { return "hip-gfx950"; }

int init(int device, std::string* err) {
  if (g_stream) {
    int n = 0;
    (void)hipGetDeviceCount(&n);
    if (device < 0 || device >= n) device = 0;
    if (device != g_device) {
      if (err) *err = "this process already decodes on device " + std::to_string(g_device) + "; device " + std::to_string(device) +
                      " needs its own process (one process per GPU)";
      return -1;
    }
    return bind_thread(err);
  }
  int n = 0;
  hipError_t e = hipGetDeviceCount(&n);
  if (e != hipSuccess || n == 0) {
    if (err) *err = "no HIP device available (libctcdec has no CPU fallback)";
    return -1;
  }
  if (device < 0 || device >= n) device = 0;
  HIP_TRY(hipSetDevice(device));
  if (!g_stream) {
    HIP_TRY(hipStreamCreateWithFlags(&g_stream, hipStreamNonBlocking));
    HIP_TRY(hipStreamCreateWithFlags(&g_copy_stream, hipStreamNonBlocking));
    for (int k = 0; k < 3; ++k) HIP_TRY(hipEventCreate(&g_ev[k]));
  }
  g_device = device;
  hipDeviceProp_t prop;
  if (hipGetDeviceProperties(&prop, device) == hipSuccess && prop.multiProcessorCount > 0) g_cus = prop.multiProcessorCount;
  return 0;
}

int bind_thread(std::string* err) {
  if (g_device >= 0) HIP_TRY(hipSetDevice(g_device));
  return 0;
}
int current_device() { return g_device; }

void* alloc(size_t bytes, std::string* err) {
  void* p = nullptr;
  hipError_t e = hipMalloc(&p, bytes ? bytes : 16);
  if (e != hipSuccess) {
    if (err) *err = std::string("hipMalloc(") + std::to_string(bytes) + "): " + hipGetErrorString(e);
    return nullptr;
  }
  return p;
}
void release(void* p) { (void)hipFree(p); }
void* alloc_host(size_t bytes, std::string* err) {
  void* p = nullptr;
  hipError_t e = hipHostMalloc(&p, bytes ? bytes : 16, hipHostMallocDefault);
  if (e != hipSuccess) {
    if (err) *err = std::string("hipHostMalloc(") + std::to_string(bytes) + "): " + hipGetErrorString(e);
    return nullptr;
  }
  return p;
}
void release_host(void* p) { (void)hipHostFree(p); }
int h2d(void* d, const void* s, size_t n, std::string* err) {
  HIP_TRY(hipMemcpyAsync(d, s, n, hipMemcpyHostToDevice, g_stream));
  HIP_TRY(hipStreamSynchronize(g_stream));
  return 0;
}
int h2d_2d_overlapped(void* d, size_t dpitch, const void* s, size_t spitch, size_t width, size_t height, std::string* err) {
  hipStream_t copy = g_copy_stream;
  if (height == 0 || width == 0) return 0;
  if (height == 1 || (dpitch == width && spitch == width)) HIP_TRY(hipMemcpyAsync(d, s, width * height, hipMemcpyHostToDevice, copy));
  else HIP_TRY(hipMemcpy2DAsync(d, dpitch, s, spitch, width, height, hipMemcpyHostToDevice, copy));
  HIP_TRY(hipStreamSynchronize(copy));
  return 0;
}
int d2h(void* d, const void* s, size_t n, std::string* err) {
  HIP_TRY(hipMemcpyAsync(d, s, n, hipMemcpyDeviceToHost, g_stream));
  HIP_TRY(hipStreamSynchronize(g_stream));
  return 0;
}
int d2d(void* d, const void* s, size_t n, std::string* err) {
  HIP_TRY(hipMemcpyAsync(d, s, n, hipMemcpyDeviceToDevice, g_stream));
  return 0;
}
int zero(void* d, size_t n, std::string* err) {
  HIP_TRY(hipMemsetAsync(d, 0, n, g_stream));
  return 0;
}
int sync(std::string* err) {
  HIP_TRY(hipStreamSynchronize(g_stream));
  return 0;
}

int d2h_async(void* d, const void* s, size_t n, std::string* err) {
  HIP_TRY(hipMemcpyAsync(d, s, n, hipMemcpyDeviceToHost, g_stream));
  return 0;
}
int h2d_async(void* d, const void* s, size_t n, std::string* err) {
  HIP_TRY(hipMemcpyAsync(d, s, n, hipMemcpyHostToDevice, g_stream));
  return 0;
}
int cus() { return g_cus; }

void last_timing(double* prune_ms, double* beam_ms) {
  *prune_ms = 0;
  *beam_ms = 0;
  if (!g_timing_valid) return;
  float a = 0, b = 0;
  if (hipEventSynchronize(g_ev[2]) != hipSuccess) return;
  if (hipEventElapsedTime(&a, g_ev[0], g_ev[1]) == hipSuccess) *prune_ms = a;
  if (hipEventElapsedTime(&b, g_ev[1], g_ev[2]) == hipSuccess) *beam_ms = b;
}

template <typename T>
__device__ __forceinline__ double ld(const T* p, size_t i) {
  return (double)p[i];
}
struct half_bits { uint16_t u; };
struct bf16_bits { uint16_t u; };
template <>
__device__ __forceinline__ double ld<half_bits>(const half_bits* p, size_t i) {
  return (double)__half2float(__ushort_as_half(p[i].u));
}
template <>
__device__ __forceinline__ double ld<bf16_bits>(const bf16_bits* p, size_t i) {
  return (double)__uint_as_float(((uint32_t)p[i].u) << 16);
}

__device__ __forceinline__ int find_utt(const int64_t* row0, int n_utts, int64_t row) {
  int lo = 0, hi = n_utts - 1;
  while (lo < hi) {
    int mid = (lo + hi + 1) >> 1;
    if (row0[mid] <= row) lo = mid; else hi = mid - 1;
  }
  return lo;
}

constexpr int PRUNE_WAVES = 4;

__global__ __launch_bounds__(64) void utt_sniff(PruneArgs a) {
  const int u = blockIdx.x;
  const int lane = threadIdx.x;
  const int64_t r0 = a.utt_row0[u], r1 = a.utt_row0[u + 1];
  double s = 0.0, c = 0.0;
  {
// ... 1770 lines not shown
    wa.progress = nullptr;
    wa.total_frames = 0;
    wa.inv_n_utts = 0.f;
    wa.block_weight = nullptr;
    const bool dump_times = getenv("CTCDEC_WAVE_TIMES") != nullptr;
    if (wa.prio_mode >= 32 || dump_times) {
      static unsigned long long* g_progress = nullptr;
      if (!g_progress) HIP_TRY(hipMalloc((void**)&g_progress, 16));
      HIP_TRY(hipMemsetAsync(g_progress, 0, 16, g_stream));
      wa.progress = g_progress;
      wa.total_frames = (unsigned long long)a.total_rows;
      wa.inv_n_utts = 1.0f / (float)a.n_utts;
      if (a.total_rows >= (1ll << 32)) wa.prio_mode = 0;
      if (wa.prio_mode == 33 || dump_times) {
        static float* g_weigh = nullptr;
        static int g_weigh_cap = 0;
        if (a.n_utts > g_weigh_cap) {
          if (g_weigh) HIP_TRY(hipFree(g_weigh));
          g_weigh = nullptr;
          g_weigh_cap = 0;
          HIP_TRY(hipMalloc((void**)&g_weigh, (size_t)a.n_utts * 16));
          g_weigh_cap = a.n_utts;
        }
        WeighArgs w;
        w.utt_row0 = a.utt_row0;
        w.surv_cnt = a.surv_cnt;
        w.n_utts = a.n_utts;
        w.total = g_weigh;
        w.per_frame = g_weigh + (size_t)a.n_utts;
        w.block_weight = g_weigh + (size_t)a.n_utts * 2;
        w.order = (int32_t*)(g_weigh + (size_t)a.n_utts * 3);
        const bool keep_order = a.order != nullptr || getenv("CTCDEC_NO_PLACE") != nullptr || a.n_utts > PLACE_MAX || wa.prio_mode != 33;
        w.given_order = a.order;
        w.simds = keep_order ? -1 : 4 * g_cus;
        w.gain = getenv("CTCDEC_WEIGH_GAIN") ? (float)atof(getenv("CTCDEC_WEIGH_GAIN")) : WEIGH_GAIN;
        w.snake = getenv("CTCDEC_PLACE_SNAKE") ? atoi(getenv("CTCDEC_PLACE_SNAKE")) : 1;
        hipLaunchKernelGGL(utt_weigh, dim3((unsigned)a.n_utts), dim3(64), 0, g_stream, w);
        hipLaunchKernelGGL(utt_place, dim3((unsigned)((a.n_utts + PLACE_PER_BLOCK - 1) / PLACE_PER_BLOCK)), dim3(256), 0, g_stream, w);
        HIP_TRY(hipGetLastError());
        wa.block_weight = w.block_weight;
        if (!keep_order) wa.order = w.order;
      }
    }
    const char* wt = getenv("CTCDEC_WAVE_TIMES");
    wa.wave_clock = nullptr;
    if (wt && wt[0]) HIP_TRY(hipMalloc((void**)&wa.wave_clock, (size_t)a.n_utts * 32));
    const int rc = launch_wave(wa, g_stream, err);
    if (rc) return rc;
    HIP_TRY(hipGetLastError());
    if (wa.wave_clock) {
      std::vector<unsigned long long> h((size_t)a.n_utts * 4);
      HIP_TRY(hipStreamSynchronize(g_stream));
      HIP_TRY(hipMemcpy(h.data(), wa.wave_clock, h.size() * 8, hipMemcpyDeviceToHost));
      HIP_TRY(hipFree(wa.wave_clock));
      if (FILE* f = fopen(wt, "wb")) {
        fwrite(h.data(), 8, h.size(), f);
        fclose(f);
      }
      if (wa.block_weight) {
        std::vector<float> bw((size_t)a.n_utts);
        HIP_TRY(hipMemcpy(bw.data(), wa.block_weight, bw.size() * 4, hipMemcpyDeviceToHost));
        if (FILE* f = fopen((std::string(wt) + ".w").c_str(), "wb")) {
          fwrite(bw.data(), 4, bw.size(), f);
          fclose(f);
        }
      }
    }
    g_last_kernel = 1;
  } else if (a.n_utts > 0) {
    const char* gt = getenv("CTCDEC_GROUP_THREADS");
    const bool wide = a.tables.n_lms <= 1 && (gt ? gt[0] == '5' : a.n_utts <= g_cus);
    LdsShape shape = make_shape(a.params.beam_width, a.params.max_surv, group_cand(beam_bucket(a.params.beam_width), wide));
    size_t lds = lds_bytes(shape);
    if (lds > 160 * 1024) {
      if (err) *err = "beam table does not fit LDS (" + std::to_string(lds) + " bytes)";
      return -1;
    }
    int rc;
    rc = launch_group(a, shape, lds, a.tables.n_lms > 1 ? 2 : (wide ? 1 : 0), g_stream, err);
    if (rc) return rc;
    HIP_TRY(hipGetLastError());
    g_last_kernel = 2;
  }
  if (a.n_utts > 0 && a.params.texts_only && a.text_scratch) {
    hipLaunchKernelGGL(assemble_texts, dim3((unsigned)a.n_utts), dim3(64), 0, g_stream, a);
    HIP_TRY(hipGetLastError());
  }
  HIP_TRY(hipEventRecord(g_ev[2], g_stream));
  g_timing_valid = true;
  return 0;
}

template <int FOLD>
__global__ __launch_bounds__(256) void token_logp(TokenLogpArgs a) {
  const int64_t i = (int64_t)blockIdx.x * 256 + threadIdx.x;
  if (i >= a.n_tokens) return;
  double v;
  const uint32_t missing = token_logp_of<FOLD>(a.runs[i], a.surv_cnt, a.surv_id, a.surv_lp, (uint32_t)a.max_surv, &v);
  a.out[i] = v;
  if (missing) atomicAdd(a.missing, missing);
}

static hipEvent_t g_logp_ev[2] = {nullptr, nullptr};
int launch_token_logp(const TokenLogpArgs& a, std::string* err) {
  if (a.n_tokens <= 0) return 0;
  if (!g_logp_ev[0])
    for (int k = 0; k < 2; ++k) HIP_TRY(hipEventCreate(&g_logp_ev[k]));
  const dim3 grid((unsigned)((a.n_tokens + 255) / 256)), block(256);
  HIP_TRY(hipEventRecord(g_logp_ev[0], g_stream));
  if (a.fold == LOGP_MEAN) hipLaunchKernelGGL(token_logp<LOGP_MEAN>, grid, block, 0, g_stream, a);
  else if (a.fold == LOGP_MIN) hipLaunchKernelGGL(token_logp<LOGP_MIN>, grid, block, 0, g_stream, a);
  else if (a.fold == LOGP_MAX) hipLaunchKernelGGL(token_logp<LOGP_MAX>, grid, block, 0, g_stream, a);
  else {
    if (err) *err = "unknown token_logp fold";
    return -1;
  }
  HIP_TRY(hipGetLastError());
  HIP_TRY(hipEventRecord(g_logp_ev[1], g_stream));
  return 0;
}
double last_token_logp_ms() {
  float ms = 0.f;
  if (!g_logp_ev[1] || hipEventSynchronize(g_logp_ev[1]) != hipSuccess) return 0.0;
  return hipEventElapsedTime(&ms, g_logp_ev[0], g_logp_ev[1]) == hipSuccess ? (double)ms : 0.0;
}

int launch_row_lse_on(const RowLseArgs& a, hipStream_t stream, std::string* err);
int launch_ctc_viterbi_on(const ViterbiArgs& a, hipStream_t stream, std::string* err);
int launch_row_lse(const RowLseArgs& a, std::string* err) { return launch_row_lse_on(a, g_stream, err); }
int launch_ctc_viterbi(const ViterbiArgs& a, std::string* err) { return launch_ctc_viterbi_on(a, g_stream, err); }

__global__ __launch_bounds__(64) void surv_ledger_append(LedgerAppendArgs a) {
  const uint32_t u = blockIdx.x, lane = threadIdx.x;
  const int64_t src0 = a.utt_row0[u];
  const uint32_t T = (uint32_t)(a.utt_row0[u + 1] - src0);
  const uint32_t r0 = a.led_row0[u];
  const uint32_t max_surv = (uint32_t)a.max_surv;
  uint64_t* ro = a.row_off + (size_t)u * (a.row_cap + 1);
  uint16_t* did = a.id + (size_t)u * a.ent_cap;
  double* dlp = a.lp + (size_t)u * a.ent_cap;
  if ((uint64_t)r0 + T > a.row_cap) {
    if (lane == 0) *a.overrun = 1;
    return;
  }
  uint64_t base = 0;
  if (r0 == 0) {
    if (lane == 0) ro[0] = 0;
  } else {
    base = ro[r0];
  }
  bool bad = false;
  for (uint32_t t0 = 0; t0 < T; t0 += 64) {
    const uint32_t t = t0 + lane;
    const size_t src = (size_t)(src0 + t);
    const uint32_t cnt = t < T ? ledger_row_count(a.surv_cnt[src], max_surv) : 0u;
    const uint32_t incl = wave_incl_scan_u32(cnt);
    const uint32_t total = (uint32_t)__builtin_amdgcn_readlane((int)incl, 63);
    const uint64_t end = base + incl;
    if (t < T) {
      if (end <= a.ent_cap) {
        ro[(size_t)r0 + t + 1] = end;
        ledger_put_row(a.surv_id + src * max_surv, a.surv_lp + src * max_surv, cnt, did + (end - cnt), dlp + (end - cnt));
      } else {
        bad = true;
      }
    }
    base += total;
// ... 60 lines not shown
```

### pyctcdecode_amd/csrc/beam_wave.h

```cpp
#pragma once
#include "beam_core.h"

namespace ctc {

typedef uint32_t u32x4 __attribute__((vector_size(16)));
typedef uint32_t u32x4a __attribute__((vector_size(16), may_alias));
typedef uint32_t u32x2a __attribute__((vector_size(8), may_alias));

CTC_HD uint64_t pack64(uint32_t lo, uint32_t hi) { return ((uint64_t)hi << 32) | lo; }
CTC_HD double bits_f64(uint64_t u) {
  union { uint64_t u; double d; } c;
  c.u = u;
  return c.d;
}
CTC_HD uint64_t f64_bits(double d) {
  union { uint64_t u; double d; } c;
  c.d = d;
  return c.u;
}
CTC_HD float bits_f32(uint32_t u) {
  union { uint32_t u; float f; } c;
  c.u = u;
  return c.f;
}
// ... 58 lines not shown
  LPtr<u32x4> pk;
  LPtr<uint64_t> pa;
  LPtr<u32x4> stage;
  LPtr<u32x4> lab;
  LPtr<uint64_t> table;
  LPtr<uint32_t> gmask;
  LPtr<double> scr;
  LPtr<uint32_t> sel;
  LPtr<uint64_t> a64, b64, c64;
  LPtr<uint32_t> b32, c32;
};

template <int BW>
CTC_HD size_t wave_lds_carve(WaveLds& o, lds_bytes_t base) {
  typedef WaveShape<BW> S;
  lds_bytes_t p = base;
  o.hA = lds_take<u32x4>(p, 16 * BW);
  o.hB = lds_take<u32x4>(p, 16 * BW);
  o.hC = lds_take<u32x4>(p, 16 * BW);
  o.a64.p = (CTC_LDS uint64_t*)o.hA.p;
  o.b64.p = (CTC_LDS uint64_t*)o.hB.p;
  o.c64.p = (CTC_LDS uint64_t*)o.hC.p;
  o.b32.p = (CTC_LDS uint32_t*)o.hB.p;
  o.c32.p = (CTC_LDS uint32_t*)o.hC.p;
  o.pk = lds_take<u32x4>(p, 16 * S::P);
  o.pa = lds_take<uint64_t>(p, 8 * S::P);
  lds_bytes_t stage0 = p;
  o.stage.p = (CTC_LDS u32x4*)p;
  o.lab = lds_take<u32x4>(p, 16 * 4 * WAVE_LAB);
  lds_bytes_t shared0 = p;
  o.table = lds_take<uint64_t>(p, 8 * S::TS);
  o.gmask.p = (CTC_LDS uint32_t*)shared0;
  o.scr.p = (CTC_LDS double*)shared0;
  o.sel.p = (CTC_LDS uint32_t*)shared0;
  size_t shared = (size_t)(p - shared0);
  if (shared < (size_t)(8 * BW)) shared = align16((size_t)(8 * BW));
  if ((size_t)(shared0 - stage0) + shared < (size_t)S::STAGE) shared = (size_t)S::STAGE - (size_t)(shared0 - stage0);
  p = shared0 + shared;
  return (size_t)(p - base);
}
template <int BW>
CTC_HD size_t wave_lds_bytes() {
  WaveLds tmp;
  return wave_lds_carve<BW>(tmp, (lds_bytes_t) nullptr);
}

CTC_HD bool wave_eligible(const DeviceTables& t, const DecodeParams& p) {
  return t.n_lms <= 1 && p.beam_width <= 128 && p.max_surv <= WAVE_SURV_CAP;
}
CTC_HD int wave_bucket(int beam_width) { return beam_width <= 64 ? 64 : beam_width <= 100 ? 100 : 128; }
CTC_HD size_t wave_pay_stride(const DecodeParams& p) { return (size_t)p.max_surv * (size_t)wave_bucket(p.beam_width); }

constexpr int W_PROF_LOAD = 0, W_PROF_COMP = 1, W_PROF_GEN = 2, W_PROF_MATCH = 3, W_PROF_FOLD = 4, W_PROF_SCORE = 5,
              W_PROF_RANK = 6, W_PROF_BUILD = 7, W_PROF_FINAL = 8, W_PROF_COMPACT = 9, W_PROF_PUSH = 10, W_PROF_PFTOK = 11,
              W_PROF_GATHER = 12, W_PROF_BIG = 13, W_PROF_TABLES = 14, W_PROF_RUN = 15, W_PROF_ST_COMP = 16, W_PROF_ST_PUSH = 17,
              W_PROF_ST_BUILD = 18, W_PROF_N = 19;

template <class Ctx, int BW, int ORD = MAX_CTX + 1, bool PROF = false>
struct WaveDecoder {
  typedef WaveShape<BW> S;
  static constexpr int SLB = S::SLB;
  static constexpr int P = S::P;
  static constexpr int PE = S::PE;

  Ctx& ctx;
  WaveLds& L;
  const UttIO& io;
  const int lane;

  int N = 1;
  uint32_t pool_n = 0;
  uint32_t pay_n = 0;
  uint64_t runmax = 0;
  uint64_t kth_key = 0;
  uint32_t text_next = 1, emit_next = 1, status = 0;
  uint32_t fflag = 0;
  uint32_t need = 0;
  uint32_t par = 0;
  uint32_t pf_cnt = 0, pf_id = 0;
  double pf_lp = 0.0;
  bool pf_live = false;
  bool run_ok = false;
  unsigned long long t_last = 0;

  CTC_HD WaveDecoder(Ctx& c, WaveLds& l, const UttIO& i) : ctx(c), L(l), io(i), lane(c.lane) {}

  CTC_HD const DeviceTables& tab() const { return ctx.tables(); }
  CTC_HD const DecodeParams& prm() const { return ctx.params(); }
  struct Hot {
    const PrefixEntry* prefixes;
    uint64_t prefix_mask;
    const HotEntry* hot;
    uint64_t hot_mask;
    const TokHot* tok_hot;
    double prune_logp, hot_weight, unk;
    uint32_t has_lm, has_trie, prune_history, beam_width;
  } H;
  CTC_HD void load_hot() {
    const DeviceTables& T_ = tab();
    const DecodeParams& P_ = prm();
    H.prefixes = T_.prefixes;
    H.prefix_mask = T_.prefix_mask;
    const HotSet hs = io.hot_set ? *io.hot_set : HotSet{T_.hot, T_.hot_mask, T_.tok_hot, P_.hot_weight};
    H.hot = hs.hot;
    H.hot_mask = hs.hot_mask;
    H.tok_hot = hs.tok_hot;
    H.prune_logp = P_.beam_prune_logp;
    H.hot_weight = hs.weight;
    H.unk = P_.unk;
    H.has_lm = T_.has_lm ? 1u : 0u;
    H.has_trie = T_.has_trie ? 1u : 0u;
    H.prune_history = P_.prune_history ? 1u : 0u;
    H.beam_width = (uint32_t)P_.beam_width;
  }

  static constexpr int CTX = (ORD - 1 < 3) ? 3 : (ORD - 1 > MAX_CTX ? MAX_CTX : (ORD - 1 <= 3 ? 3 : MAX_CTX));
  static constexpr int NODE_BYTES = CTX <= 3 ? 64 : 128;
  struct Node {
    double raw;
    uint32_t hw_cnt, ring_cnt;
    LmState st;
    uint64_t ring[MAX_CTX];
  };
  CTC_HD u32x4a* node_ptr(uint32_t idx) const { return (u32x4a*)((char*)io.text_nodes + (size_t)idx * (size_t)NODE_BYTES); }
  CTC_HD void node_load(uint32_t idx, Node& n) const {
    const u32x4a* p = node_ptr(idx);
    const u32x4 c0 = p[0], c1 = p[1], c2 = p[2], c3 = p[3];
    n.raw = bits_f64(q_lo(c0));
    n.hw_cnt = c0[2];
    n.ring_cnt = c0[3] & 0xFFu;
    n.st.len = (int32_t)(c0[3] >> 8);
    if (CTX <= 3) {
      n.st.words[0] = c1[0]; n.st.words[1] = c1[1]; n.st.words[2] = c1[2]; n.st.words[3] = 0; n.st.words[4] = 0;
      n.st.backoff[0] = bits_f32(c1[3]); n.st.backoff[1] = bits_f32(c2[0]); n.st.backoff[2] = bits_f32(c2[1]);
      n.st.backoff[3] = 0.f; n.st.backoff[4] = 0.f;
      n.ring[0] = q_hi(c2); n.ring[1] = q_lo(c3); n.ring[2] = q_hi(c3); n.ring[3] = 0; n.ring[4] = 0;
    } else {
      const u32x4 c4 = p[4], c5 = p[5];
      n.st.words[0] = c1[0]; n.st.words[1] = c1[1]; n.st.words[2] = c1[2]; n.st.words[3] = c1[3]; n.st.words[4] = c2[0];
      n.st.backoff[0] = bits_f32(c2[1]); n.st.backoff[1] = bits_f32(c2[2]); n.st.backoff[2] = bits_f32(c2[3]);
      n.st.backoff[3] = bits_f32(c3[0]); n.st.backoff[4] = bits_f32(c3[1]);
      n.ring[0] = q_hi(c3); n.ring[1] = q_lo(c4); n.ring[2] = q_hi(c4); n.ring[3] = q_lo(c5); n.ring[4] = q_hi(c5);
    }
  }
  CTC_HD void node_store(uint32_t idx, const Node& n) const {
    u32x4a* p = node_ptr(idx);
    const uint64_t rb = f64_bits(n.raw);
    p[0] = mk4((uint32_t)rb, (uint32_t)(rb >> 32), n.hw_cnt, (n.ring_cnt & 0xFFu) | ((uint32_t)n.st.len << 8));
    if (CTX <= 3) {
      p[1] = mk4(n.st.words[0], n.st.words[1], n.st.words[2], f32_bits(n.st.backoff[0]));
      p[2] = mk4(f32_bits(n.st.backoff[1]), f32_bits(n.st.backoff[2]), (uint32_t)n.ring[0], (uint32_t)(n.ring[0] >> 32));
      p[3] = mk4q(n.ring[1], n.ring[2]);
    } else {
      p[1] = mk4(n.st.words[0], n.st.words[1], n.st.words[2], n.st.words[3]);
      p[2] = mk4(n.st.words[4], f32_bits(n.st.backoff[0]), f32_bits(n.st.backoff[1]), f32_bits(n.st.backoff[2]));
      p[3] = mk4(f32_bits(n.st.backoff[3]), f32_bits(n.st.backoff[4]), (uint32_t)n.ring[0], (uint32_t)(n.ring[0] >> 32));
      p[4] = mk4q(n.ring[1], n.ring[2]);
      p[5] = mk4q(n.ring[3], n.ring[4]);
    }
  }

  template <int PHASE>
  CTC_HD void tick() {
    if (PROF && io.prof && lane == 0) {
      unsigned long long now = ctx.clock();
      io.prof[PHASE] += now - t_last;
// ... 1244 lines not shown
      uint64_t mlo[SLB], mhi[SLB];
      group_masks<SLB>(valid, rep, mlo, mhi);
CTC_UNROLL
      for (int j = 0; j < SLB; ++j) {
        const uint32_t v = (uint32_t)(j * 64 + lane);
        is_rep[j] = valid[j] && rep[j] == v;
        if (is_rep[j]) {
          while (mlo[j]) {
            const uint32_t mbit = (uint32_t)ctx.ctz64(mlo[j]);
            mlo[j] &= mlo[j] - 1ull;
            lg[j] = lse2(lg[j], bits_f64(L.b64[mbit * 2]));
            donor[j] = mbit;
          }
          while (mhi[j]) {
            const uint32_t mbit = (uint32_t)(64 + ctx.ctz64(mhi[j]));
            mhi[j] &= mhi[j] - 1ull;
            lg[j] = lse2(lg[j], bits_f64(L.b64[mbit * 2]));
            donor[j] = mbit;
          }
        }
      }
    }
    double score[SLB];
    uint64_t pass_key = 0;
CTC_UNROLL
    for (int j = 0; j < SLB; ++j) {
      score[j] = 0.0;
      if (!is_rep[j]) continue;
      const uint32_t v = (uint32_t)(j * 64 + lane);
      if (fold) {
        const uint32_t d = donor[j];
        const u32x4 d1 = L.hB[d], d2 = L.hC[d];
        const uint32_t m2 = d1[3];
        const uint32_t pl = d1[2] >> 16;
        double lmhw;
        if (eos) {
          const ColdRec dcr = cold_cur()[d];
          Node src;
          node_load(dcr.tnode, src);
          const uint32_t cnt = src.hw_cnt + ((pl > 0 && (m2 & M2_HOT_COMPLETE)) ? 1u : 0u);
          if (tab().has_lm) {
            LmState st = src.st, end;
            const uint32_t wid = pl > 0 ? dcr.wid : 0u;
            const uint32_t wfl = pl > 0 ? m2 : 0u;
            const float base_s = lm_base_score<ORD>(tab(), st, wid, &end);
            double end_score = 0.0;
            if (prm().score_boundary) {
              LmState tmp;
              end_score = (double)lm_base_score<ORD>(tab(), end, tab().eos_id, &tmp);
            }
            const double raw = src.raw + lm_word_score(tab(), prm(), base_s, wfl, end_score, true);
            lmhw = raw + H.hot_weight * (double)cnt;
          } else {
            lmhw = H.hot_weight * (double)cnt;
          }
        } else {
          lmhw = pl > 0 ? cold_cur()[d].c_lmhw : bits_f64(q_lo(d2));
        }
        score[j] = tab().has_lm ? lg[j] + lmhw : lg[j] + lmhw + 0.0;
      } else {
        const u32x4 k1 = L.hB[v];
        const uint32_t pl = k1[2] >> 16;
        score[j] = total_score(tab(), lg[j], bits_f64(L.c64[v * 2]), pl > 0 ? cold_cur()[v].pscore : 0.0, pl);
      }
      const uint64_t k = asc_key(score[j]);
      if (k > pass_key) pass_key = k;
    }
    runmax = ctx.wave_max_u64(pass_key);
    if (runmax < asc_key(-INFINITY)) runmax = asc_key(-INFINITY);
CTC_UNROLL
    for (int j = 0; j < SLB; ++j) {
      if ((uint32_t)(j * 64) >= Q) continue;
      pool_put(is_rep[j], mk4q(score_sort_key(score[j]), 0), (uint32_t)(j * 64 + lane), donor[j], lg[j], f64_bits(score[j]), 0u,
               0u, 0u);
    }
    ctx.wsync();
    uint32_t n = rank_pool(key_to_score(runmax) + prm().beam_prune_logp, false);
    if (n > (uint32_t)prm().beam_width) n = (uint32_t)prm().beam_width;
    if (n == 0) status |= ST_NO_BEAMS;
    if (io.carry_out && !eos) carry_beams(n, fold);
    uint32_t n_out = io.want_out ? n : 0u;
    if (prm().n_best > 0 && n_out > (uint32_t)prm().n_best) n_out = (uint32_t)prm().n_best;
    if (prm().texts_only != 0 && n_out > 0) {
      if (lane == 0) {
        const uint64_t a2 = L.pa[L.sel[0] & 0x7FFFFFFFu];
        const PoolPay& pp = io.pay[((uint32_t)a2 >> 16) & 0xFFFFu];
        const uint32_t d = (uint32_t)(a2 >> 32);
        OutBeam& ob = io.out[0];
        ob.logit_score = pp.logit;
        ob.lm_score = bits_f64(pp.part_h);
        ob.raw_lm = 0.0;
        ob.tok_off = 0;
        ob.tok_cnt = 0;
        ob.state.len = -1;
        ob.last_char = NO_CHAR;
        ob.pstart = ob.pend = -1;
        ob.pad[0] = 0;
        ob.pad[1] = cold_cur()[d].enode;
        *io.n_out = 1;
        *io.status = status;
      }
      return;
    }
    uint32_t len[SLB], off[SLB];
    uint32_t total = 0;
CTC_UNROLL
    for (int j = 0; j < SLB; ++j) {
      const uint32_t r = (uint32_t)(j * 64 + lane);
      len[j] = 0;
      off[j] = 0;
      if (r < n_out) {
        const uint32_t d = (uint32_t)(L.pa[L.sel[r] & 0x7FFFFFFFu] >> 32);
        len[j] = cold_cur()[d].depth + ((fold && (L.b32[d * 4 + 2] >> 16) > 0) ? 1u : 0u);
      }
      off[j] = total + ctx.wave_excl_sum_u32(len[j]);
      total += ctx.wave_sum_u32(len[j]);
    }
    unsigned long long base = 0;
    if (lane == 0) {
      base = ctx.global_add(io.tok_pool_head, (unsigned long long)total);
      if (base + total > io.tok_pool_cap) {
        status |= ST_TOK_OVERFLOW;
        base = 0;
      }
    }
    base = ctx.bcast64(base, 0);
    status = ctx.wave_or_u32(status);
    const bool tok_ok = !(status & ST_TOK_OVERFLOW);
CTC_UNROLL
    for (int j = 0; j < SLB; ++j) {
      const uint32_t r = (uint32_t)(j * 64 + lane);
      if (r >= n_out) continue;
      const uint64_t a2 = L.pa[L.sel[r] & 0x7FFFFFFFu];
      const PoolPay& pp = io.pay[((uint32_t)a2 >> 16) & 0xFFFFu];
      const uint32_t d = (uint32_t)(a2 >> 32);
      const ColdRec cr = cold_cur()[d];
      OutBeam& ob = io.out[r];
      ob.logit_score = pp.logit;
      ob.lm_score = bits_f64(pp.part_h);
      const u32x4 d1 = L.hB[d], d2 = L.hC[d];
      const uint32_t meta1 = d1[2];
      const uint32_t pl = meta1 >> 16;
      const bool closes = fold && pl > 0;
      const uint32_t o = (uint32_t)(base + off[j]);
      ob.tok_off = o;
      ob.tok_cnt = tok_ok ? len[j] : 0;
      ob.pad[0] = (uint32_t)cr.pstart;
      ob.pad[1] = (uint32_t)cr.pend;
      ob.last_char = fold ? NO_CHAR : (meta1 & 0xFFFFu);
      ob.pstart = fold ? -1 : cr.pstart;
      ob.pend = fold ? -1 : cr.pend;
      Node node;
      node_load(closes ? cr.cnode : cr.tnode, node);
      ob.raw_lm = node.raw;
      if (!tab().has_lm) {
        ob.state.len = -1;
CTC_UNROLL
        for (int k = 0; k < MAX_CTX; ++k) {
          ob.state.words[k] = 0;
          ob.state.backoff[k] = 0.f;
        }
      } else if (eos) {
        Node src;
        node_load(cr.tnode, src);
        LmState st = src.st, after;
        lm_base_score<ORD>(tab(), st, pl > 0 ? cr.wid : 0u, &after);
        ob.state = after;
      } else {
        ob.state = node.st;
      }
      if (tok_ok) {
        uint32_t pos = o + len[j];
        if (closes) {
          EmitNode fin;
          fin.parent = 0;
          fin.tok_branch = BR_FINAL << 16;
          fin.wstart = cr.pstart;
          fin.wend = cr.pend;
          io.tok_pool[--pos] = fin;
        }
        uint32_t e = cr.enode;
// ... 98 lines not shown
```

### pyctcdecode_amd/csrc/beam_wave_hip.hip

```cpp
#include <hip/hip_runtime.h>
#include <stdio.h>
#include <stdlib.h>

#include <string>

#include "backend.h"
#include "beam_core.h"
#include "beam_wave.h"
#include "wave_ops_hip.h"

namespace ctc {
namespace be {

#define HIP_TRY_W(expr)                                                                  \
  do {                                                                                   \
    hipError_t e_ = (expr);                                                              \
    if (e_ != hipSuccess) {                                                              \
      if (err) *err = std::string(#expr) + ": " + hipGetErrorString(e_);                 \
      return -1;                                                                         \
    }                                                                                    \
  } while (0)

typedef const BeamArgs __attribute__((address_space(4))) * KernArgs;
struct WaveGpuCtx {
  int lane;
  KernArgs ka;
  __device__ __forceinline__ void set_prio(uint32_t p) {
    switch (p) {
      case 0: __builtin_amdgcn_s_setprio(0); break;
      case 1: __builtin_amdgcn_s_setprio(1); break;
      case 2: __builtin_amdgcn_s_setprio(2); break;
      default: __builtin_amdgcn_s_setprio(3); break;
    }
  }
  __device__ __forceinline__ void frame_done(int t, int t2, int T) {
    if ((((uint32_t)t ^ (uint32_t)t2) >> 4) == 0u) return;
    const KernArgs k = fresh();
    const int32_t mode = k->prio_mode;
    if (mode == 0) return;
    if (mode < 32) {
      uint32_t hw;
      asm volatile("s_getreg_b32 %0, hwreg(HW_REG_HW_ID, 0, 4)" : "=s"(hw));
      set_prio((hw + ((uint32_t)t2 >> (mode - 1))) & 3u);
      return;
    }
    const uint32_t units = (((uint32_t)t2 >> 4) - ((uint32_t)t >> 4)) << 4;
    unsigned long long old = 0;
    if (lane == 0) old = atomicAdd(k->progress, (unsigned long long)units);
    const uint32_t done = (uint32_t)__builtin_amdgcn_readfirstlane((int)(uint32_t)old) + units;
    const float avg_left = (float)((uint32_t)k->total_frames - done) * k->inv_n_utts;
    const float weight = mode == 33 ? k->block_weight[blockIdx.x] : 1.f;
    const float d = (float)(T - t2) * weight - avg_left;
    set_prio(d > 24.f ? 3u : d > 0.f ? 2u : d > -24.f ? 1u : 0u);
  }
  __device__ __forceinline__ void start_prio(int T) {
    const KernArgs k = fresh();
    if (k->prio_mode != 33) return;
    const float d = (float)T * k->block_weight[blockIdx.x] - (float)(uint32_t)k->total_frames * k->inv_n_utts;
    set_prio(d > 24.f ? 3u : d > 0.f ? 2u : d > -24.f ? 1u : 0u);
  }
  __device__ __forceinline__ KernArgs fresh() const {
    KernArgs p = ka;
    asm volatile("" : "+s"(p));
    return p;
  }
  __device__ __forceinline__ const DeviceTables& tables() const { return *(const DeviceTables*)&fresh()->tables; }
  __device__ __forceinline__ const DecodeParams& params() const { return *(const DecodeParams*)&fresh()->params; }
  __device__ __forceinline__ void wsync() {
    __builtin_amdgcn_fence(__ATOMIC_SEQ_CST, "wavefront");
    __builtin_amdgcn_wave_barrier();
  }
  __device__ __forceinline__ void mem_sync() {
    __builtin_amdgcn_fence(__ATOMIC_SEQ_CST, "workgroup");
    __builtin_amdgcn_wave_barrier();
  }
  __device__ __forceinline__ void vm_wait() { __builtin_amdgcn_s_waitcnt(0x0F70); }
  __device__ __forceinline__ uint64_t ballot(bool p) { return __ballot(p); }
  __device__ __forceinline__ int popc64(uint64_t x) { return __popcll(x); }
  __device__ __forceinline__ int clz64(uint64_t x) { return __clzll((long long)x); }
  __device__ __forceinline__ int ctz64(uint64_t x) { return __builtin_ctzll(x); }
  __device__ __forceinline__ int clz32(uint32_t x) { return __clz((int)x); }
  __device__ __forceinline__ int ctz32(uint32_t x) { return __builtin_ctz(x); }
  __device__ __forceinline__ uint32_t uni32(uint32_t v) { return (uint32_t)__builtin_amdgcn_readfirstlane((int)v); }
  __device__ __forceinline__ uint32_t opaque32(uint32_t v) {
    asm volatile("" : "+v"(v));
    return v;
  }
  __device__ __forceinline__ uint32_t bcast32(uint32_t v, int src) {
    return (uint32_t)__builtin_amdgcn_readlane((int)v, __builtin_amdgcn_readfirstlane(src));
  }
  __device__ __forceinline__ uint32_t shfl32(uint32_t v, int src) {
    return (uint32_t)__builtin_amdgcn_ds_bpermute(src << 2, (int)v);
  }
  __device__ __forceinline__ uint64_t bcast64(uint64_t v, int src) {
    const int s = __builtin_amdgcn_readfirstlane(src);
    const uint32_t lo = (uint32_t)__builtin_amdgcn_readlane((int)(uint32_t)v, s);
    const uint32_t hi = (uint32_t)__builtin_amdgcn_readlane((int)(uint32_t)(v >> 32), s);
    return ((uint64_t)hi << 32) | lo;
  }
  __device__ __forceinline__ uint64_t wave_max_u64(uint64_t v) { return wave_max_u64_split(v); }
  __device__ __forceinline__ uint32_t wave_or_u32(uint32_t v) {
    if (__ballot((v & 0xFFu) != 0u) == 0ull) return v;
    uint32_t r = 0;
#pragma unroll
    for (int b = 0; b < 8; ++b)
      if (__ballot((v >> b) & 1u)) r |= 1u << b;
    return r | (v & ~0xFFu);
  }
  __device__ __forceinline__ uint32_t wave_excl_sum_u32(uint32_t v) {
    uint32_t incl = v;
#pragma unroll
    for (int off = 1; off < 64; off <<= 1) {
      const uint32_t o = (uint32_t)__shfl_up((int)incl, off, 64);
      if ((int)(threadIdx.x & 63) >= off) incl += o;
    }
    return incl - v;
  }
  __device__ __forceinline__ uint32_t wave_sum_u32(uint32_t v) {
    int x = (int)v;
    x += __builtin_amdgcn_update_dpp(0, x, 0x111, 0xf, 0xf, false);
    x += __builtin_amdgcn_update_dpp(0, x, 0x112, 0xf, 0xf, false);
    x += __builtin_amdgcn_update_dpp(0, x, 0x114, 0xf, 0xf, false);
    x += __builtin_amdgcn_update_dpp(0, x, 0x118, 0xf, 0xf, false);
    x += __builtin_amdgcn_update_dpp(0, x, 0x142, 0xa, 0xf, false);
    x += __builtin_amdgcn_update_dpp(0, x, 0x143, 0xc, 0xf, false);
    return (uint32_t)__builtin_amdgcn_readlane(x, 63);
  }
  __device__ __forceinline__ void lds_max_u64(CTC_LDS uint64_t* p, uint64_t v) {
    __hip_atomic_fetch_max(p, v, __ATOMIC_RELAXED, __HIP_MEMORY_SCOPE_WAVEFRONT);
  }
  __device__ __forceinline__ void lds_or_u32(CTC_LDS uint32_t* p, uint32_t v) {
    __hip_atomic_fetch_or(p, v, __ATOMIC_RELAXED, __HIP_MEMORY_SCOPE_WAVEFRONT);
  }
  __device__ __forceinline__ unsigned long long clock() { return (unsigned long long)wall_clock64(); }
  __device__ __forceinline__ unsigned long long global_add(unsigned long long* p, unsigned long long v) {
    return atomicAdd(p, v);
  }
};

template <int BW, int ORD, bool PROF>
__global__ __launch_bounds__(64) __attribute__((amdgpu_waves_per_eu(BW <= 100 ? 4 : 3, BW <= 100 ? 4 : 3))) void beam_wave(BeamArgs a) {
  extern __shared__ __attribute__((aligned(16))) char smem[];
  const int u = a.order ? a.order[blockIdx.x] : (int)blockIdx.x;
  WaveLds view;
  wave_lds_carve<BW>(view, (lds_bytes_t)smem);
  UttIO io;
  const int64_t r0 = a.utt_row0[u];
  io.surv_cnt = a.surv_cnt + r0;
  io.surv_id = a.surv_id + (size_t)r0 * a.params.max_surv;
  io.surv_lp = a.surv_lp + (size_t)r0 * a.params.max_surv;
  io.T = (int32_t)(a.utt_row0[u + 1] - r0);
  io.text_nodes = a.text_nodes + a.text_off[u];
  io.text_cap = (uint32_t)(a.text_off[u + 1] - a.text_off[u]);
  io.emit_nodes = a.emit_nodes + a.emit_off[u];
  io.emit_cap = (uint32_t)(a.emit_off[u + 1] - a.emit_off[u]);
  io.start_state = a.start_states ? a.start_states + (size_t)u : nullptr;
  io.out_xstates = nullptr;
  io.out = a.out + (size_t)u * a.out_stride;
  io.n_out = a.n_out + u;
  io.status = a.status + u;
  io.tok_pool = a.tok_pool;
  io.tok_pool_head = a.tok_pool_head;
  io.tok_pool_cap = a.tok_pool_cap;
  io.prof = (u == 0) ? a.prof : nullptr;
  io.imports = (a.imports && !a.resident_in) ? a.imports + a.import_off[u] : nullptr;
  io.n_import = (a.imports && !a.resident_in) ? (int32_t)(a.import_off[u + 1] - a.import_off[u]) : 0;
  io.import_xstates = nullptr;
  io.first_frame = a.first_frames ? a.first_frames[u] : a.params.first_frame;
  io.cold = a.cold + (size_t)u * 2 * COLD_STRIDE;
  io.pay = a.pay + (size_t)u * a.pay_stride;
  io.carry_out = a.carry_out ? a.carry_out + (size_t)u * a.carry_stride : nullptr;
  io.carry_xstates = (a.carry_out && a.carry_xstates) ? a.carry_xstates + (size_t)u * a.carry_stride * (1u - 1) : nullptr;
  io.sstate = a.sstate ? a.sstate + u : nullptr;
  io.emit_start = a.sstate ? a.sstate[u].emit_next : 0u;
  io.want_out = a.want_out;
  io.hot_set = a.utt_hot ? a.hot_sets + a.utt_hot[u] : nullptr;
  if (a.resident_in) {
    io.imports = a.imports + (size_t)u * a.carry_stride;
    io.n_import = (int32_t)a.sstate[u].n_carry;
    io.import_xstates = a.import_xstates ? a.import_xstates + (size_t)u * a.carry_stride * 0 : nullptr;
  }
  WaveGpuCtx ctx{(int)threadIdx.x, (KernArgs)__builtin_amdgcn_kernarg_segment_ptr()};
  unsigned long long* rec = a.wave_clock ? a.wave_clock + (size_t)blockIdx.x * 4 : nullptr;
  asm volatile("" : "+v"(rec));
  if (rec && threadIdx.x == 0) {
    rec[0] = wall_clock64();
    rec[3] = (unsigned long long)io.T | ((unsigned long long)(uint32_t)u << 32);
  }
  ctx.start_prio(io.T);
  WaveDecoder<WaveGpuCtx, BW, ORD, PROF> dec(ctx, view, io);
  dec.run();
  if (rec && threadIdx.x == 0) {
    uint32_t hw, xcc;
    asm volatile("s_getreg_b32 %0, hwreg(HW_REG_HW_ID)" : "=s"(hw));
    asm volatile("s_getreg_b32 %0, hwreg(HW_REG_XCC_ID)" : "=s"(xcc));
    rec[1] = wall_clock64();
    rec[2] = (unsigned long long)hw | ((unsigned long long)xcc << 32);
  }
}


template <int BW, int ORD, bool PROF>
static int launch_wave_p(const BeamArgs& a, hipStream_t stream, std::string* err) {
  const size_t lds = wave_lds_bytes<BW>();
  HIP_TRY_W(hipFuncSetAttribute((const void*)beam_wave<BW, ORD, PROF>, hipFuncAttributeMaxDynamicSharedMemorySize, (int)lds));
  hipLaunchKernelGGL((beam_wave<BW, ORD, PROF>), dim3((unsigned)a.n_utts), dim3(64), lds, stream, a);
  return 0;
}
template <int BW, int ORD>
static int launch_wave_t(const BeamArgs& a, hipStream_t stream, std::string* err) {
  return a.prof ? launch_wave_p<BW, ORD, true>(a, stream, err) : launch_wave_p<BW, ORD, false>(a, stream, err);
}
template <int BW>
static int launch_wave_bw(const BeamArgs& a, hipStream_t stream, std::string* err) {
  if (!a.tables.has_lm || a.tables.lm_order <= 4) return launch_wave_t<BW, 4>(a, stream, err);
  return launch_wave_t<BW, MAX_CTX + 1>(a, stream, err);
}

int launch_wave(const BeamArgs& a, hipStream_t stream, std::string* err) {
  switch (wave_bucket(a.params.beam_width)) {
    case 64: return launch_wave_bw<64>(a, stream, err);
    case 100: return launch_wave_bw<100>(a, stream, err);
    default: return launch_wave_bw<128>(a, stream, err);
  }
}

}
}
```

### pyctcdecode_amd/csrc/pytexts.c

```c
#define PY_SSIZE_T_CLEAN
#include <Python.h>
#include <stdint.h>
#include <string.h>

PyObject* ctcdec_py_split_texts(const char* blob, int64_t nbytes, int64_t n, char sep) {
  PyObject* list = PyList_New((Py_ssize_t)n);
  if (!list) return NULL;
  const char* p = blob;
  const char* end = blob + nbytes;
  for (int64_t i = 0; i < n; ++i) {
    const char* q = (i + 1 < n) ? (const char*)memchr(p, sep, (size_t)(end - p)) : end;
    if (!q) {
      Py_DECREF(list);
      PyErr_SetString(PyExc_ValueError, "fewer texts in the blob than announced");
      return NULL;
    }
    PyObject* s = PyUnicode_DecodeUTF8(p, (Py_ssize_t)(q - p), "strict");
    if (!s) {
      Py_DECREF(list);
      return NULL;
    }
    PyList_SET_ITEM(list, (Py_ssize_t)i, s);
    p = q + 1;
  }
  return list;
}

PyObject* ctcdec_py_texts_from_blocks(const char* pool, const int64_t* off, const int64_t* len, int64_t n) {
  PyObject* list = PyList_New((Py_ssize_t)n);
  if (!list) return NULL;
  for (int64_t i = 0; i < n; ++i) {
    PyObject* s = PyUnicode_DecodeUTF8(pool + off[i], (Py_ssize_t)len[i], "strict");
    if (!s) {
      Py_DECREF(list);
      return NULL;
    }
    PyList_SET_ITEM(list, (Py_ssize_t)i, s);
  }
  return list;
}

static PyObject *k_text, *k_state, *k_frames, *k_logit, *k_lm;

static int beam_attr_names(void) {
  if (k_text) return 0;
  k_text = PyUnicode_InternFromString("text");
  k_state = PyUnicode_InternFromString("last_lm_state");
  k_frames = PyUnicode_InternFromString("text_frames");
  k_logit = PyUnicode_InternFromString("logit_score");
  k_lm = PyUnicode_InternFromString("lm_score");
  return (k_text && k_state && k_frames && k_logit && k_lm) ? 0 : -1;
}

static PyObject* word_frames(const char* p, int64_t len, int64_t n_words, const int32_t* ws, const int32_t* we) {
  PyObject* frames = PyList_New((Py_ssize_t)n_words);
  if (!frames) return NULL;
  const char* end = p + len;
  for (int64_t j = 0; j < n_words; ++j) {
    if (len == 0 || p > end) {
      Py_DECREF(frames);
      PyErr_SetString(PyExc_IndexError, "list index out of range");
      return NULL;
    }
    const char* q = (const char*)memchr(p, ' ', (size_t)(end - p));
    if (!q) q = end;
    PyObject* w = PyUnicode_DecodeUTF8(p, (Py_ssize_t)(q - p), "strict");
    PyObject* a = w ? PyLong_FromLong((long)ws[j]) : NULL;
    PyObject* b = a ? PyLong_FromLong((long)we[j]) : NULL;
    PyObject* span = b ? PyTuple_Pack(2, a, b) : NULL;
    PyObject* item = span ? PyTuple_Pack(2, w, span) : NULL;
    Py_XDECREF(w);
    Py_XDECREF(a);
    Py_XDECREF(b);
    Py_XDECREF(span);
    if (!item) {
      Py_DECREF(frames);
      return NULL;
    }
    PyList_SET_ITEM(frames, (Py_ssize_t)j, item);
    p = q + 1;
  }
  return frames;
}

PyObject* ctcdec_py_output_beams(PyObject* cls, int64_t n_utts, const int64_t* beam_off, const int64_t* text_off,
                                 const char* text_blob, const double* logit, const double* lm, const int64_t* word_cnt_off,
                                 const int32_t* word_start, const int32_t* word_end, PyObject* states, PyObject* frames_of) {
  if (beam_attr_names() < 0) return NULL;
  if (!PyType_Check(cls)) {
    PyErr_SetString(PyExc_TypeError, "OutputBeam class expected");
    return NULL;
  }
  PyTypeObject* tp = (PyTypeObject*)cls;
  const int with_states = states != NULL && states != Py_None;
  PyObject* out = PyList_New((Py_ssize_t)n_utts);
  if (!out) return NULL;
  for (int64_t u = 0; u < n_utts; ++u) {
    const int64_t k0 = beam_off[u], k1 = beam_off[u + 1];
    PyObject* beams = PyList_New((Py_ssize_t)(k1 - k0));
    if (!beams) goto fail;
    PyList_SET_ITEM(out, (Py_ssize_t)u, beams);
    for (int64_t k = k0; k < k1; ++k) {
      const char* tp0 = text_blob + text_off[k];
      const int64_t tlen = text_off[k + 1] - text_off[k];
      const int64_t w0 = word_cnt_off[k], w1 = word_cnt_off[k + 1];
      PyObject* obj = tp->tp_alloc(tp, 0);
      if (!obj) goto fail;
      PyList_SET_ITEM(beams, (Py_ssize_t)(k - k0), obj);
      PyObject* text = PyUnicode_DecodeUTF8(tp0, (Py_ssize_t)tlen, "strict");
      const int lazy = frames_of != NULL && frames_of != Py_None;
      PyObject* frames = !text ? NULL
                         : lazy ? PyObject_CallFunction(frames_of, "OLL", text, (long long)w0, (long long)w1)
                                : word_frames(tp0, tlen, w1 - w0, word_start ? word_start + w0 : NULL, word_end ? word_end + w0 : NULL);
      PyObject* lg = frames ? PyFloat_FromDouble(logit[k]) : NULL;
      PyObject* ls = lg ? PyFloat_FromDouble(lm[k]) : NULL;
      PyObject* st = Py_None;
      if (ls && with_states) {
        st = PyList_GetItem(states, (Py_ssize_t)k);
        if (!st) {
          Py_DECREF(text);
          Py_DECREF(frames);
// ... 114 lines not shown
```

### pyctcdecode_amd/decoder.py

```python
from __future__ import annotations

import ctypes as C
import dataclasses
import logging
import math
import os
import threading
from typing import Any, Collection, Dict, Iterable, List, Optional, Sequence, Tuple, TypeVar

import numpy as np

from . import _binding as B
from .alphabet import Alphabet, verify_alphabet_coverage
from .constants import (
    DEFAULT_ALPHA,
    DEFAULT_BEAM_WIDTH,
    DEFAULT_BETA,
    DEFAULT_HOTWORD_WEIGHT,
    DEFAULT_MIN_TOKEN_LOGP,
    DEFAULT_PRUNE_BEAMS,
    DEFAULT_PRUNE_LOGP,
    DEFAULT_SCORE_LM_BOUNDARY,
    DEFAULT_UNK_LOGP_OFFSET,
    LOG_BASE_CHANGE_FACTOR,
# ... 911 lines not shown
        lm.reset_params(**{name: value for name, value in given.items() if value is not None})

    @classmethod
    def clear_class_models(cls) -> None:
        cls.model_container = {}

    def cleanup(self) -> None:
        if self._model_key in BeamSearchDecoderCTC.model_container:
            del BeamSearchDecoderCTC.model_container[self._model_key]

    @property
    def _language_model(self) -> Optional[AbstractLanguageModel]:
        return BeamSearchDecoderCTC.model_container[self._model_key]

    def _check_logits_dimension(self, logits: Any) -> None:
        if len(logits.shape) != 2:
            raise ValueError(
                "Input logits have %s dimensions, but need 2: (time, vocabulary)" % len(logits.shape)
            )
        if logits.shape[-1] != len(self._idx2vocab):
            raise ValueError(
                "Input logits shape is %s, but vocabulary is size %s. "
                "Need logits of shape: (time, vocabulary)" % (tuple(logits.shape), len(self._idx2vocab))
            )

    def _set_hotwords(self, hotwords: Optional[Iterable[str]]) -> None:
        unigrams = HotwordScorer.build_scorer(hotwords).unigrams
        key = tuple(unigrams)
        if key == self._hot_key:
            return
        blob, off = B.pack_strings(unigrams)
        self._lib.check(self._lib.dll.ctcdec_set_hotwords(self._handle, blob, B.off_ptr(off), len(unigrams)))
        self._hot_key = key

    def _arm_hot_sets(self, hot) -> None:
        sets, utt_set = hot
        words = [w for ws, _ in sets for w in ws]
        blob, off = B.pack_strings(words)
        set_off = np.zeros(len(sets) + 1, dtype=np.int64)
        if sets:
            set_off[1:] = np.cumsum([len(ws) for ws, _ in sets])
        weight = np.array([w for _, w in sets] or [0.0], dtype=np.float64)
        idx = np.array(utt_set or [0], dtype=np.int32)
        self._lib.check(self._lib.dll.ctcdec_set_hotword_sets(
            self._handle, blob, B.off_ptr(off), len(words), B.off_ptr(set_off), len(sets),
            weight.ctypes.data_as(C.POINTER(C.c_double)), idx.ctypes.data_as(C.POINTER(C.c_int32)), len(utt_set)))

    def _resolve_hot(self, hotwords, hotword_weight, n: int):
        hot = _per_utt_hot(hotwords, hotword_weight, n)
        if hot is None:
            return hotwords, hotword_weight, None
        sets, utt_set = hot
        if all(k == utt_set[0] for k in utt_set):
            if utt_set[0] < 0:
                return None, DEFAULT_HOTWORD_WEIGHT, None
            words, w = sets[utt_set[0]]
            return list(words), w, None
        return None, DEFAULT_HOTWORD_WEIGHT, hot

    def _params(self, beam_width, beam_prune_logp, token_min_logp, prune_history, hotword_weight, n_best) -> B.Params:
        lm = self._members[0] if self._members else None
        with self._call_lock:
            for k, m in enumerate(self._members[1:], start=1):
                self._lib.check(self._lib.dll.ctcdec_lm_set_params(
                    self._handle, k, float(m.alpha), float(m.beta), float(m.unk_score_offset), int(bool(m.score_boundary))))
        p = B.Params()
        p.beam_width = int(beam_width)
        p.prune_history = int(bool(prune_history))
        p.n_best = int(n_best)
        p.want_lm_state = 1
        p.beam_prune_logp = float(beam_prune_logp)
        p.token_min_logp = float(token_min_logp)
        p.hotword_weight = float(hotword_weight)
        p.alpha = float(lm.alpha) if lm is not None else 0.0
        p.beta = float(lm.beta) if lm is not None else 0.0
        p.unk_score_offset = float(lm.unk_score_offset) if lm is not None else 0.0
        p.log_base_change = LOG_BASE_CHANGE_FACTOR
        p.lm_score_boundary = int(bool(lm.score_boundary)) if lm is not None else 0
        p.first_frame = 0
        p.texts_only = 0
        p.token_frames = 0
        return p

    def _run(self, logits_list: Sequence[Any], params: B.Params, hotwords, start_states=None, hot_sets=None):
        with self._call_lock:
            return self._run_locked(logits_list, params, hotwords, start_states, hot_sets)

    def _run_locked(self, logits_list: Sequence[Any], params: B.Params, hotwords, start_states=None, hot_sets=None):
        if hot_sets is None:
            self._set_hotwords(hotwords)
        batch = _Batch(logits_list, len(self._idx2vocab))
        if batch.is_device and batch.device_index is not None and batch.device_index != self._device:
            raise ValueError("the logits live on cuda:%d but this decoder was built for cuda:%d (one process per GPU: "
                             "LOCAL_RANK / CTCDEC_DEVICE pick the device)" % (batch.device_index, self._device))
        n = len(batch.ptrs)
        ptrs, frames = _c_arrays(batch)
        st_arr = None
        n_lms = len(self._members)
        if start_states is not None and n_lms > 0:
            st_arr = (B.LmState * max(n * n_lms, 1))()
            for k, s in enumerate(start_states):
                if s is None:
                    for j in range(n_lms):
                        st_arr[k * n_lms + j].length = -1
                    continue
                if n_lms > 1:
                    if not isinstance(s, MultiLanguageModelState):
                        raise AssertionError(
                            f"Wrong input state type found. Expected MultiLanguageModelState, got {type(s)}")
                    if len(s.states) != n_lms:
                        raise AssertionError(
                            f"Number of states ({len(s.states)}) does not match number of language models ({n_lms}).")
                    parts = s.states
                else:
                    parts = [s]
                for j, part in enumerate(parts):
                    if not isinstance(part, KenlmState):
                        raise AssertionError(f"Wrong input state type found. Expected KenlmState, got {type(part)}")
                    st_arr[k * n_lms + j] = part.state.to_c()
        res = C.c_void_p()
        if hot_sets is not None:
            self._arm_hot_sets(hot_sets)
        self._lib.check(
            self._lib.dll.ctcdec_decode_batch(self._handle, ptrs, frames, n, batch.dtype, int(batch.is_device),
                                              C.byref(params), st_arr, C.byref(res))
        )
        ms = (C.c_double * 3)()
        self._lib.dll.ctcdec_result_timing(res, ms)
        self.last_timing_ms = (float(ms[0]), float(ms[1]), float(ms[2]))
        self.last_beam_kernel = int(self._lib.dll.ctcdec_result_beam_kernel(res))
        return res

    def _unpack(self, res: C.c_void_p, with_state: bool) -> List[List[OutputBeam]]:
        pk = B.Packed()
        self._lib.check(self._lib.dll.ctcdec_result_pack(res, C.byref(pk)))
        nb, nw, nu = int(pk.n_beams), int(pk.n_words), int(pk.n_utts)
        beam_off = np.ctypeslib.as_array(pk.beam_off, shape=(nu + 1,))
        out: List[List[OutputBeam]] = []
        if nb == 0:
            return [[] for _ in range(nu)]
        has_lm = self._language_model is not None
        if not os.environ.get("CTCDEC_PY_UNPACK"):
            states = None
            if with_state and has_lm:
                states = []
                for u in range(nu):
                    for k in range(int(beam_off[u]), int(beam_off[u + 1])):
                        states.append(self._beam_state(res, pk, u, k, k - int(beam_off[u])))
            frames_of = None
            if not os.environ.get("CTCDEC_EAGER_FRAMES"):
                if nw:
                    ws = np.ctypeslib.as_array(pk.word_start, shape=(nw,)).copy()
                    we = np.ctypeslib.as_array(pk.word_end, shape=(nw,)).copy()
                else:
                    ws = we = np.zeros(0, dtype=np.int32)
                frames_of = _lazy_word_frames_factory(ws, we)
            built = B.output_beams(OutputBeam, pk, states, frames_of)
            if built is not None:
                return built
        text_off = np.ctypeslib.as_array(pk.text_off, shape=(nb + 1,))
        blob = C.string_at(pk.text_blob, int(text_off[nb])) if text_off[nb] else b""
        logit = np.ctypeslib.as_array(pk.logit_score, shape=(nb,))
        lm = np.ctypeslib.as_array(pk.lm_score, shape=(nb,))
        wco = np.ctypeslib.as_array(pk.word_cnt_off, shape=(nb + 1,))
        if nw:
            wstart = np.ctypeslib.as_array(pk.word_start, shape=(nw,))
            wend = np.ctypeslib.as_array(pk.word_end, shape=(nw,))
        for u in range(nu):
            beams = []
            for k in range(int(beam_off[u]), int(beam_off[u + 1])):
                text = blob[int(text_off[k]) : int(text_off[k + 1])].decode("utf-8")
                words = text.split(" ") if text else []
                w0, w1 = int(wco[k]), int(wco[k + 1])
                frames = [(words[j], (int(wstart[w0 + j]), int(wend[w0 + j]))) for j in range(w1 - w0)]
                state = self._beam_state(res, pk, u, k, k - int(beam_off[u])) if (with_state and has_lm) else None
                beams.append(OutputBeam(text, state, frames, float(logit[k]), float(lm[k])))
            out.append(beams)
        return out

    def _beam_state(self, res, pk, u: int, k: int, j_in_utt: int) -> AbstractLMState:
        state: AbstractLMState = KenlmState(NgramState.from_c(pk.lm_state[k]))
        if len(self._members) > 1:
            parts = [state]
            for j in range(1, len(self._members)):
                cst = B.LmState()
                self._lib.check(self._lib.dll.ctcdec_result_lm_state_of(res, u, j_in_utt, j, C.byref(cst)))
                parts.append(KenlmState(NgramState.from_c(cst)))
            state = MultiLanguageModelState(parts)
        return state

    def decode_beams(
        self,
        logits: Any,
        beam_width: int = DEFAULT_BEAM_WIDTH,
        beam_prune_logp: float = DEFAULT_PRUNE_LOGP,
        token_min_logp: float = DEFAULT_MIN_TOKEN_LOGP,
        prune_history: bool = DEFAULT_PRUNE_BEAMS,
        hotwords: Optional[Iterable[str]] = None,
        hotword_weight: float = DEFAULT_HOTWORD_WEIGHT,
        lm_start_state: Optional[AbstractLMState] = None,
        token_frames: bool = False,
        confidence: Optional[str] = None,
    ) -> List[OutputBeam]:
        self._check_logits_dimension(logits)
        fold = _confidence_fold(confidence)
        params = self._params(beam_width, beam_prune_logp, token_min_logp, prune_history, hotword_weight, 0)
        params.token_frames = fold or int(bool(token_frames))
        res = self._run([logits], params, hotwords, [lm_start_state])
        try:
            beams = self._unpack(res, True)
            return (self._with_tokens(res, beams, bool(fold)) if params.token_frames else beams)[0]
        finally:
            self._lib.dll.ctcdec_result_free(res)

    def decode(
        self,
        logits: Any,
        beam_width: int = DEFAULT_BEAM_WIDTH,
        beam_prune_logp: float = DEFAULT_PRUNE_LOGP,
        token_min_logp: float = DEFAULT_MIN_TOKEN_LOGP,
        hotwords: Optional[Iterable[str]] = None,
        hotword_weight: float = DEFAULT_HOTWORD_WEIGHT,
        lm_start_state: Optional[AbstractLMState] = None,
    ) -> str:
        self._check_logits_dimension(logits)
        params = self._params(beam_width, beam_prune_logp, token_min_logp, True, hotword_weight, 1)
        res = self._run([logits], params, hotwords, [lm_start_state])
        try:
            return self._unpack(res, False)[0][0].text
        finally:
            self._lib.dll.ctcdec_result_free(res)

    def decode_batch(
        self,
        pool: Any,
        logits_list: Sequence[Any],
        beam_width: int = DEFAULT_BEAM_WIDTH,
        beam_prune_logp: float = DEFAULT_PRUNE_LOGP,
        token_min_logp: float = DEFAULT_MIN_TOKEN_LOGP,
        hotwords: Optional[Iterable[str]] = None,
        hotword_weight: float = DEFAULT_HOTWORD_WEIGHT,
        token_frames: bool = False,
        confidence: Optional[str] = None,
    ) -> Any:
        fold = _confidence_fold(confidence)
        token_frames = bool(token_frames) or bool(fold)
        if getattr(logits_list, "ndim", 0) != 3:
            logits_list = list(logits_list)
        if len(logits_list) == 0:
            return ([], self._empty_token_frames(bool(fold))) if token_frames else []
        if type(pool).__name__ == "DevicePool":
            kw = dict(confidence=confidence) if fold else dict(token_frames=True) if token_frames else {}
            return pool.decode_batch(logits_list, beam_width=beam_width, beam_prune_logp=beam_prune_logp,
                                     token_min_logp=token_min_logp, hotwords=hotwords, hotword_weight=hotword_weight, **kw)
        hotwords, hotword_weight, hot_sets = self._resolve_hot(hotwords, hotword_weight, len(logits_list))
        params = self._params(beam_width, beam_prune_logp, token_min_logp, True, hotword_weight, 1)
        if token_frames:
            params.token_frames = fold or 1
        else:
            params.texts_only = 1
        res = self._run(logits_list, params, hotwords, hot_sets=hot_sets)
        try:
            texts = self._texts(res)
            return (texts, self._token_frames(res, len(texts), bool(fold))) if token_frames else texts
        finally:
            self._lib.dll.ctcdec_result_free(res)

    def _empty_token_frames(self, with_logp: bool = False) -> TokenFrames:
        z = np.zeros(0, dtype=np.int32)
        return TokenFrames(z, z.copy(), z.copy(), np.zeros(1, dtype=np.int64), self._alphabet.labels,
                           np.zeros(0, dtype=np.float64) if with_logp else None)

    def _token_frames(self, res, n_beams: int, with_logp: bool = False) -> TokenFrames:
        off_p, lab_p, st_p, en_p = (C.POINTER(C.c_int64)(), C.POINTER(C.c_int32)(), C.POINTER(C.c_int32)(),
                                    C.POINTER(C.c_int32)())
        n = C.c_int64()
        self._lib.check(self._lib.dll.ctcdec_result_token_frames(res, C.byref(off_p), C.byref(lab_p), C.byref(st_p),
                                                                 C.byref(en_p), C.byref(n)))
        nt = int(n.value)
        offsets = np.ctypeslib.as_array(off_p, shape=(n_beams + 1,)).copy()
        if nt:
            arrs = [np.ctypeslib.as_array(q, shape=(nt,)).copy() for q in (lab_p, st_p, en_p)]
        else:
            arrs = [np.zeros(0, dtype=np.int32) for _ in range(3)]
        logp = None
        if with_logp:
            logp = self._token_logp(res)
            if len(logp) != nt:
                raise B.NativeError("token confidences and token frames differ in number")
        return TokenFrames(arrs[0], arrs[1], arrs[2], offsets, self._alphabet.labels, logp)

    def _token_logp(self, res) -> np.ndarray:
        lp_p, n = C.POINTER(C.c_double)(), C.c_int64()
        self._lib.check(self._lib.dll.ctcdec_result_token_logp(res, C.byref(lp_p), C.byref(n)))
        nt = int(n.value)
        return np.ctypeslib.as_array(lp_p, shape=(nt,)).copy() if nt else np.zeros(0, dtype=np.float64)

    def _with_tokens(self, res, beams: List[List[OutputBeam]], with_logp: bool = False) -> List[List[TokenOutputBeam]]:
        tf = self._token_frames(res, sum(len(bs) for bs in beams), with_logp)
        out, k = [], 0
        for bs in beams:
            row = []
            for b in bs:
                toks = tf.of(k)
                if with_logp:
                    lps = tf.logp_of(k)
                    row.append(ConfidenceOutputBeam(b.text, b.last_lm_state, b.text_frames, b.logit_score, b.lm_score, toks,
                                                    lps, _word_logps(b.text_frames, toks, lps)))
                else:
                    row.append(TokenOutputBeam(b.text, b.last_lm_state, b.text_frames, b.logit_score, b.lm_score, toks))
                k += 1
            out.append(row)
        return out

    def _texts(self, res) -> List[str]:
        texts = B.texts_of(self._lib, res)
        if texts is not None:
            return texts
        if self._texts_sep is not None:
            blob_p, nbytes, n = C.c_void_p(), C.c_int64(), C.c_int64()
            self._lib.check(self._lib.dll.ctcdec_result_texts_joined(res, self._texts_sep, C.byref(blob_p), C.byref(nbytes),
                                                                     C.byref(n)))
            if n.value == 0:
                return []
            parts = B.split_texts(blob_p, int(nbytes.value), int(n.value), self._texts_sep)
            if len(parts) == n.value:
                return parts
        blob_p, off_p, n = C.c_void_p(), C.POINTER(C.c_int64)(), C.c_int64()
        self._lib.check(self._lib.dll.ctcdec_result_texts(res, C.byref(blob_p), C.byref(off_p), C.byref(n)))
        nb = int(n.value)
        text_off = np.ctypeslib.as_array(off_p, shape=(nb + 1,))
        blob = C.string_at(blob_p, int(text_off[nb])) if text_off[nb] else b""
        off = text_off.tolist()
        if blob.isascii():
            text = blob.decode("ascii")
            return [text[off[k] : off[k + 1]] for k in range(nb)]
        return [blob[off[k] : off[k + 1]].decode("utf-8") for k in range(nb)]

    def decode_beams_batch(
        self,
        pool: Any,
        logits_list: Sequence[Any],
        beam_width: int = DEFAULT_BEAM_WIDTH,
# ... 460 lines not shown
```

Baseline: 184.9 million.

## Stream decoded texts from device waves to a host sink as they finish

Adds a text-sink API in which each beam-wave, on finishing, backtracks its text and writes it straight into host-mapped memory with a ticket record. A host thread polls the tickets and passes batches of texts to a Python sink while other waves are still running. The aim is to overlap text transfer and Python string creation with kernel execution instead of doing them serially after the kernel. It adds system-scope stores, host polling with sleeps, and more complexity around generation tags and overflow handling.

```diff
diff --git a/include/ctcdec.h b/include/ctcdec.h
--- a/include/ctcdec.h
+++ b/include/ctcdec.h
@@ -99,6 +99,11 @@
 int ctcdec_decode_batch(ctcdec_decoder* dec, const void* const* utt_logits,
                         const int32_t* utt_frames, int32_t n_utts, int32_t dtype, int32_t is_device,
                         const ctcdec_params* params, const ctcdec_lm_state* start_states,
+                        ctcdec_result** out);
+
+typedef int (*ctcdec_text_sink)(void* user, int32_t n, const int32_t* utt, const char* const* utf8, const int64_t* len);
+int ctcdec_decode_texts(ctcdec_decoder* dec, const void* const* utt_logits, const int32_t* utt_frames, int32_t n_utts,
+                        int32_t dtype, int32_t is_device, const ctcdec_params* params, ctcdec_text_sink sink, void* user,
                         ctcdec_result** out);
 
 typedef struct ctcdec_beam_in {
diff --git a/pyctcdecode_amd/_binding.py b/pyctcdecode_amd/_binding.py
--- a/pyctcdecode_amd/_binding.py
+++ b/pyctcdecode_amd/_binding.py
@@ -106,6 +106,8 @@
                                           C.POINTER(C.c_double), C.POINTER(C.c_int32), C.c_int32]),
     "ctcdec_decode_batch": (C.c_int, [_VP, C.POINTER(_VP), C.POINTER(C.c_int32), C.c_int32, C.c_int32, C.c_int32,
                                       C.POINTER(Params), C.POINTER(LmState), C.POINTER(_VP)]),
+    "ctcdec_decode_texts": (C.c_int, [_VP, C.POINTER(_VP), C.POINTER(C.c_int32), C.c_int32, C.c_int32, C.c_int32,
+                                      C.POINTER(Params), _VP, C.py_object, C.POINTER(_VP)]),
     "ctcdec_decode_stream_batch": (C.c_int, [_VP, C.POINTER(_VP), C.POINTER(C.c_int32), C.c_int32, C.c_int32, C.c_int32,
                                              C.POINTER(Params), C.POINTER(C.c_int32), C.POINTER(BeamIn),
                                              C.POINTER(C.c_int64), C.c_char_p, C.c_int32, C.c_int32, C.POINTER(_VP)]),
@@ -220,6 +222,9 @@
                                                    C.POINTER(C.c_int64), C.POINTER(C.c_int32), C.POINTER(C.c_int32),
                                                    C.POINTER(C.c_int32), C.POINTER(C.c_int32), C.POINTER(C.c_double),
                                                    C.POINTER(C.c_double), C.py_object]
+                dll.ctcdec_py_text_sink_finish.restype = C.py_object
+                dll.ctcdec_py_text_sink_finish.argtypes = [C.py_object]
+                dll.text_sink_ptr = C.cast(dll.ctcdec_py_text_sink, C.c_void_p)
                 _PYTEXTS = dll
             except (OSError, AttributeError):
                 _PYTEXTS = False
@@ -235,6 +240,13 @@
     if n.value == 0:
         return []
     return dll.ctcdec_py_texts_from_blocks(pool, off, ln, n.value)
+
+
+def text_sink():
+    dll = _pytexts()
+    if not dll:
+        return None
+    return dll.text_sink_ptr, dll.ctcdec_py_text_sink_finish
 
 
 def output_beams(cls, pk: "Packed", states: Optional[list], frames_of=None) -> Optional[list]:
diff --git a/pyctcdecode_amd/csrc/api.cpp b/pyctcdecode_amd/csrc/api.cpp
--- a/pyctcdecode_amd/csrc/api.cpp
+++ b/pyctcdecode_amd/csrc/api.cpp
@@ -30,6 +30,8 @@
   g_err = msg;
   return code;
 }
+
+static int sink_refused(int rc) { return fail(CTCDEC_ERR_ARG, "the text sink refused a batch (it returned " + std::to_string(rc) + ")"); }
 
 namespace {
 
@@ -64,6 +66,30 @@
 };
 using DevBuf = Buf<false>;
 using HostBuf = Buf<true>;
+
+#ifndef CTC_SIM
+struct MappedBuf {
+  void* p = nullptr;
+  size_t cap = 0;
+  MappedBuf() = default;
+  MappedBuf(const MappedBuf&) = delete;
+  MappedBuf& operator=(const MappedBuf&) = delete;
+  ~MappedBuf() {
+    if (p) be::release_host(p);
+  }
+  int ensure(size_t bytes, std::string* err) {
+    if (bytes <= cap && p) return 0;
+    if (p) be::release_host(p);
+    cap = 0;
+    const size_t want = bytes + bytes / 4 + 4096;
+    p = be::alloc_host_mapped(want, err);
+    if (!p) return -1;
+    memset(p, 0, want);
+    cap = want;
+    return 0;
+  }
+};
+#endif
 
 template <class T>
 int upload(DevBuf& b, const std::vector<T>& v, std::string* err) {
@@ -200,6 +226,10 @@
   int dense_calls = 0;
   HostBuf h_stage;
   size_t stage_used = 0;
+#ifndef CTC_SIM
+  MappedBuf h_texts;
+  uint32_t ticket_gen = 0;
+#endif
   bool profile = false;
   unsigned long long prof[N_PROF] = {0};
 };
@@ -787,6 +817,8 @@
   ctcdec_stream* rs = nullptr;
   bool want_result = true;
   const AfterLaunch* after_launch = nullptr;
+  ctcdec_text_sink sink = nullptr;
+  void* sink_user = nullptr;
 };
 static int decode_impl(ctcdec_decoder* dec, const void* const* utt_logits, const int32_t* utt_frames, int32_t n_utts,
                        int32_t dtype, int32_t is_device, const ctcdec_params* p, const ctcdec_lm_state* start_states,
@@ -808,6 +840,51 @@
     }
   }
   return decode_impl(dec, utt_logits, utt_frames, n_utts, dtype, is_device, p, start_states, DecodeMode(), out);
+}
+
+int ctcdec_decode_texts(ctcdec_decoder* dec, const void* const* utt_logits, const int32_t* utt_frames, int32_t n_utts, int32_t dtype,
+                        int32_t is_device, const ctcdec_params* p, ctcdec_text_sink sink, void* user, ctcdec_result** out) {
+  if (!sink || !p || p->texts_only == 0 || p->token_frames != 0 || p->n_best != 1)
+    return fail(CTCDEC_ERR_ARG, "ctcdec_decode_texts: a sink, texts_only = 1, token_frames = 0 and n_best = 1 are required");
+  HotCallScope hot_scope(dec);
+  ctcdec_result* res = nullptr;
+  int rc = 1;
+  if (dec && !is_device && !dec->hot_call.armed && n_utts > 0 && utt_logits && utt_frames && dtype >= CTCDEC_F32 && dtype <= CTCDEC_BF16) {
+    const int n_slices = host_slices_wanted(dec, utt_frames, n_utts, dtype);
+    if (n_slices >= 2) {
+      rc = decode_host_sliced(dec, utt_logits, utt_frames, n_utts, dtype, p, nullptr, n_slices, &res);
+      if (rc == CTCDEC_OK) {
+        const char* pool = nullptr;
+        const int64_t *off = nullptr, *len = nullptr;
+        int64_t n = 0;
+        rc = ctcdec_result_text_blocks(res, &pool, &off, &len, &n);
+        if (rc == CTCDEC_OK && n != n_utts) rc = fail(CTCDEC_ERR_INTERNAL, "an utterance without a beam");
+        if (rc == CTCDEC_OK) {
+          std::vector<int32_t> utt((size_t)n);
+          std::vector<const char*> ptr((size_t)n);
+          for (int64_t u = 0; u < n; ++u) {
+            utt[(size_t)u] = (int32_t)u;
+            ptr[(size_t)u] = pool + off[u];
+          }
+          if (const int s = sink(user, (int32_t)n, utt.data(), ptr.data(), len)) rc = sink_refused(s);
+        }
+        if (rc != CTCDEC_OK) {
+          ctcdec_result_free(res);
+          res = nullptr;
+        }
+      }
+    }
+  }
+  if (rc == 1) {
+    DecodeMode mode;
+    mode.sink = sink;
+    mode.sink_user = user;
+    rc = decode_impl(dec, utt_logits, utt_frames, n_utts, dtype, is_device, p, nullptr, mode, &res);
+  }
+  if (rc != CTCDEC_OK) return rc;
+  if (out) *out = res;
+  else ctcdec_result_free(res);
+  return CTCDEC_OK;
 }
 
 int ctcdec_decode_stream_batch(ctcdec_decoder* dec, const void* const* utt_logits, const int32_t* utt_frames,
@@ -928,6 +1005,11 @@
   bool outgrown_redone = false;
   int32_t led = 0;
   std::vector<int64_t> led_rows;
+  bool ticket_launch = false, streamed = false;
+  int32_t delivered = 0;
+  std::vector<uint8_t> got;
+  int sink_rc = 0;
+  double sink_ms = 0, tail_ms = 0;
   bool host_timing = false;
   Clock::time_point t_begin, t_launch, t_kernel, t_end;
   std::string err;
@@ -1146,6 +1228,8 @@
   return CTCDEC_OK;
 }
 
+static constexpr bool TEXT_STREAM_DEFAULT = true;
+
 static int reserve_device_texts(DecodeCall& c) {
   ctcdec_decoder* dec = c.dec;
   std::vector<uint64_t> soff((size_t)c.n_utts + 1, 0);
@@ -1158,6 +1242,18 @@
   c.ba.text_soff = (const uint64_t*)dec->w_tsoff.p;
   c.ba.text_pool = (uint8_t*)dec->w_tpool.p;
   c.ba.text_pool_cap = soff[(size_t)c.n_utts];
+  if (const char* e = getenv("CTCDEC_TEXT_POOL_CAP")) c.ba.text_pool_cap = std::min<unsigned long long>(c.ba.text_pool_cap, strtoull(e, nullptr, 10));
+#ifndef CTC_SIM
+  const char* ts = getenv("CTCDEC_TEXT_STREAM");
+  if (c.sink && (ts ? ts[0] != '0' : TEXT_STREAM_DEFAULT) && (uint64_t)c.n_utts < (1ull << (64 - be::TICKET_SHIFT)) && soff[(size_t)c.n_utts] < be::TICKET_ONE) {
+    const size_t ring = ((size_t)c.n_utts * sizeof(be::TextTicket) + 63) & ~(size_t)63;
+    if (dec->h_texts.ensure(64 + ring + (size_t)soff[(size_t)c.n_utts] + 16, &c.err)) return fail(CTCDEC_ERR_DEVICE, c.err);
+    char* base = (char*)dec->h_texts.p;
+    c.ba.tickets_written = (unsigned long long*)base;
+    c.ba.tickets = (be::TextTicket*)(base + 64);
+    c.ba.host_pool = (uint8_t*)(base + 64 + ring);
+  }
+#endif
   return CTCDEC_OK;
 }
 
@@ -1262,10 +1358,98 @@
   return CTCDEC_OK;
 }
 
+static int launch_beam_stage(DecodeCall& c) {
+  c.ticket_launch = false;
+#ifndef CTC_SIM
+  if (c.ba.host_pool) {
+    be::BeamArgs a = c.ba;
+    if (a.pay && be::wave_kernel_chosen(a)) {
+      if (++c.dec->ticket_gen >= (1u << 24)) {
+        memset(c.dec->h_texts.p, 0, c.dec->h_texts.cap);
+        c.dec->ticket_gen = 1;
+      }
+      a.ticket_gen = c.dec->ticket_gen;
+      __atomic_store_n(a.tickets_written, 0ull, __ATOMIC_RELEASE);
+      c.ticket_launch = true;
+      c.delivered = 0;
+      c.got.assign((size_t)c.n_utts, 0);
+    } else {
+      a.host_pool = nullptr;
+      a.tickets = nullptr;
+      a.tickets_written = nullptr;
+    }
+    c.streamed = c.ticket_launch;
+    if (be::launch_beam(a, &c.err)) return fail(CTCDEC_ERR_DEVICE, c.err);
+    return CTCDEC_OK;
+  }
+#endif
+  if (be::launch_beam(c.ba, &c.err)) return fail(CTCDEC_ERR_DEVICE, c.err);
+  return CTCDEC_OK;
+}
+
 static int run_beam(DecodeCall& c) {
   if (be::zero(c.dec->w_head.p, 16, &c.err)) return fail(CTCDEC_ERR_DEVICE, c.err);
   if (c.dec->hot_call.armed && !c.ba.hot_sets && upload_hot_sets(c.dec, &c.ba, &c.err)) return fail(CTCDEC_ERR_DEVICE, c.err);
-  if (be::launch_beam(c.ba, &c.err)) return fail(CTCDEC_ERR_DEVICE, c.err);
+  return launch_beam_stage(c);
+}
+
+static int deliver_tickets(DecodeCall& c) {
+#ifndef CTC_SIM
+  if (!c.ticket_launch) return CTCDEC_OK;
+  c.ticket_launch = false;
+  const int32_t n = c.n_utts;
+  const be::TextTicket* ring = c.ba.tickets;
+  const char* pool = (const char*)c.ba.host_pool;
+  const uint32_t gen = c.dec->ticket_gen;
+  constexpr int MIN_BATCH = 32, MAX_BATCH = 512;
+  int32_t utt[MAX_BATCH];
+  const char* ptr[MAX_BATCH];
+  int64_t len[MAX_BATCH];
+  int32_t next = 0, nb = 0;
+  int done = 0, polls = 0;
+  Clock::time_point t_done{}, t_last{};
+  for (;;) {
+    if (!done && (++polls & 3) == 0) {
+      if (be::beam_done(&done, &c.err)) return fail(CTCDEC_ERR_DEVICE, c.err);
+      if (done) t_done = Clock::now();
+    }
+    const int32_t before = next;
+    {
+      while (next < n && nb < MAX_BATCH) {
+        const be::TextTicket& t = ring[next];
+        const uint32_t tag = __atomic_load_n(&t.tag, __ATOMIC_ACQUIRE);
+        if ((tag >> 8) != gen) break;
+        ++next;
+        const uint64_t off = (uint64_t)t.off16 * 16;
+        if (tag & ST_TOK_OVERFLOW) continue;
+        if (t.utt >= (uint32_t)n || off + t.len > c.ba.text_pool_cap) return fail(CTCDEC_ERR_INTERNAL, "text ticket out of range");
+        if (!c.got[t.utt]) {
+          c.got[t.utt] = 1;
+          ++c.delivered;
+        }
+        utt[nb] = (int32_t)t.utt;
+        ptr[nb] = pool + off;
+        len[nb] = (int64_t)t.len;
+        ++nb;
+      }
+    }
+    if (nb >= MIN_BATCH || ((done || next == n) && nb > 0)) {
+      if (!c.sink_rc) {
+        const auto t0 = Clock::now();
+        c.sink_rc = c.sink(c.sink_user, nb, utt, ptr, len);
+        t_last = Clock::now();
+        c.sink_ms += ms(t0, t_last);
+      }
+      nb = 0;
+      continue;
+    }
+    if ((done && next == before) || next == n) break;
+    if (!done) std::this_thread::sleep_for(std::chrono::microseconds(50));
+  }
+  c.tail_ms = done && t_last > t_done ? ms(t_done, t_last) : 0.0;
+#else
+  (void)c;
+#endif
   return CTCDEC_OK;
 }
 
@@ -1340,6 +1524,8 @@
     if (early_beam)
       if (int rc = run_beam(*beam)) return rc;
     s.t_queued = Clock::now();
+    if (early_beam)
+      if (int rc = deliver_tickets(*beam)) return rc;
     if (be::d2h(flags, dec->w_flags.p, 32, &err)) return fail(CTCDEC_ERR_DEVICE, err);
     s.t_flags = Clock::now();
     s.surv_total = flags[4];
@@ -1351,8 +1537,10 @@
       pa.pass = 1;
       if (be::zero(dec->w_flags.p, 4, &err) || be::zero((char*)dec->w_flags.p + 16, 4, &err)) return fail(CTCDEC_ERR_DEVICE, err);
       if (be::launch_prune(pa, &err)) return fail(CTCDEC_ERR_DEVICE, err);
-      if (early_beam)
+      if (early_beam) {
         if (int rc = run_beam(*beam)) return rc;
+        if (int rc = deliver_tickets(*beam)) return rc;
+      }
       if (be::d2h(flags, dec->w_flags.p, 32, &err)) return fail(CTCDEC_ERR_DEVICE, err);
       s.surv_total = flags[4];
     }
@@ -1469,8 +1657,10 @@
   }
   if (c.led)
     if (int rc = reserve_ledger(c)) return rc;
-  if (c.late_beam)
+  if (c.late_beam) {
     if (int rc = run_beam(c)) return rc;
+    if (int rc = deliver_tickets(c)) return rc;
+  }
   return c.led && c.R > 0 ? append_ledger(c) : CTCDEC_OK;
 }
 
@@ -1491,8 +1681,10 @@
   c.ba.emit_nodes = (EmitNode*)dec->w_emit.p;
   c.ba.text_off = (const uint64_t*)dec->w_toff.p;
   c.ba.emit_off = (const uint64_t*)dec->w_eoff.p;
-  if (be::zero(dec->w_head.p, 16, &err) || be::launch_beam(c.ba, &err) ||
-      be::d2h(c.n_out, dec->w_nout.p, (size_t)n_utts * 4, &err) || be::d2h(c.status, dec->w_status.p, (size_t)n_utts * 4, &err) ||
+  if (be::zero(dec->w_head.p, 16, &err)) return fail(CTCDEC_ERR_DEVICE, err);
+  if (int rc = launch_beam_stage(c)) return rc;
+  if (int rc = deliver_tickets(c)) return rc;
+  if (be::d2h(c.n_out, dec->w_nout.p, (size_t)n_utts * 4, &err) || be::d2h(c.status, dec->w_status.p, (size_t)n_utts * 4, &err) ||
       be::d2h(&c.head, dec->w_head.p, 8, &err))
     return fail(CTCDEC_ERR_DEVICE, err);
   return CTCDEC_OK;
@@ -1583,6 +1775,46 @@
   *c.out = c.res.release();
 }
 
+static int feed_sink_once(DecodeCall& c) {
+  if (!c.sink) return CTCDEC_OK;
+  const ctcdec_result* res = c.res.get();
+  const size_t n = (size_t)c.n_utts;
+  std::vector<int32_t> utt(n);
+  std::vector<const char*> ptr(n);
+  std::vector<int64_t> len(n);
+  for (size_t u = 0; u < n; ++u) {
+    utt[u] = (int32_t)u;
+    if (res->device_texts) {
+      ptr[u] = res->dev_texts.data() + res->dev_out[u].tok_off;
+      len[u] = (int64_t)res->dev_out[u].tok_cnt;
+    } else {
+      if (res->utts[u].empty()) return fail(CTCDEC_ERR_INTERNAL, "an utterance without a beam");
+      ptr[u] = res->utts[u][0].text.data();
+      len[u] = (int64_t)res->utts[u][0].text.size();
+    }
+  }
+  const auto t0 = Clock::now();
+  c.sink_rc = c.sink(c.sink_user, (int32_t)n, utt.data(), ptr.data(), len.data());
+  c.sink_ms += ms(t0, Clock::now());
+  return c.sink_rc ? sink_refused(c.sink_rc) : CTCDEC_OK;
+}
+
+static int finish_streamed_texts(DecodeCall& c) {
+  ctcdec_result* res = c.res.get();
+  if (int rc = kernel_stats(c)) return rc;
+  if (c.host_timing) {
+    const PruneStage& s = c.prune;
+    fprintf(stderr, "[ctcdec host] texts to the sink as the waves finish: %d of %d utterances, native call so far %.3f ms (kernels %.3f + %.3f): "
+                    "setup %.3f, launches %.3f, wait for the kernels %.3f, counters back %.3f; in the sink %.3f, launch end to last ticket delivered %.3f\n",
+            c.delivered, c.n_utts, ms(c.t_begin, Clock::now()), res->ms[0], res->ms[1], ms(c.t_begin, s.t_setup), ms(s.t_setup, s.t_queued),
+            ms(s.t_queued, s.t_flags), ms(s.t_flags, c.t_kernel), c.sink_ms, c.tail_ms);
+  }
+  if (c.sink_rc) return sink_refused(c.sink_rc);
+  if (c.delivered != c.n_utts) return fail(CTCDEC_ERR_INTERNAL, "texts of " + std::to_string(c.n_utts - c.delivered) + " utterances never arrived from the device");
+  close_call(c);
+  return CTCDEC_OK;
+}
+
 static int finish_device_texts(DecodeCall& c) {
   ctcdec_result* res = c.res.get();
   std::string& err = c.err;
@@ -1599,12 +1831,15 @@
     if (c.n_out[u] != 1 || (unsigned long long)ob.tok_off + ob.tok_cnt > heads[1]) return fail(CTCDEC_ERR_INTERNAL, "text pool range");
   }
   if (int rc = kernel_stats(c)) return rc;
+  const auto t_back = Clock::now();
+  if (int rc = feed_sink_once(c)) return rc;
   close_call(c);
   if (c.host_timing) {
     const PruneStage& s = c.prune;
     fprintf(stderr, "[ctcdec host] texts from the device: %llu bytes, native call %.3f ms (kernels %.3f + %.3f): setup %.3f, launches %.3f, "
-                    "wait for the kernels %.3f, counters back %.3f, records + texts back %.3f\n", heads[1], res->ms[2], res->ms[0], res->ms[1],
-            ms(c.t_begin, s.t_setup), ms(s.t_setup, s.t_queued), ms(s.t_queued, s.t_flags), ms(s.t_flags, c.t_kernel), ms(c.t_kernel, Clock::now()));
+                    "wait for the kernels %.3f, counters back %.3f, records + texts back %.3f; in the sink %.3f, launch end to last ticket delivered %.3f\n",
+            heads[1], res->ms[2], res->ms[0], res->ms[1], ms(c.t_begin, s.t_setup), ms(s.t_setup, s.t_queued), ms(s.t_queued, s.t_flags),
+            ms(s.t_flags, c.t_kernel), ms(c.t_kernel, t_back), c.sink_ms, c.sink ? ms(c.t_kernel, Clock::now()) : 0.0);
   }
   return CTCDEC_OK;
 }
@@ -1813,6 +2048,7 @@
   }
   if (c.fold)
     if (int rc = token_confidences(c)) return rc;
+  if (int rc = feed_sink_once(c)) return rc;
   close_call(c);
   if (c.host_timing)
     fprintf(stderr, "[ctcdec host] setup+launch %.3f ms, wait kernels %.3f ms, copy back %.3f ms (%llu tokens), replay %.3f ms\n",
@@ -1840,6 +2076,7 @@
   if (int rc = prune_and_launch(c)) return rc;
   if (c.after_launch && *c.after_launch && (*c.after_launch)(&c.err)) return fail(CTCDEC_ERR_DEVICE, c.err);
   if (int rc = collect_counters(c)) return rc;
+  if (c.streamed) return finish_streamed_texts(c);
   return c.device_texts ? finish_device_texts(c) : c.want_result ? finish_beams(c) : finish_stream_push(c);
 }
 
diff --git a/pyctcdecode_amd/csrc/backend.h b/pyctcdecode_amd/csrc/backend.h
--- a/pyctcdecode_amd/csrc/backend.h
+++ b/pyctcdecode_amd/csrc/backend.h
@@ -61,6 +61,15 @@
 };
 int launch_prune(const PruneArgs& a, std::string* err);
 int launch_sniff_exact(const PruneArgs& a, std::string* err);
+
+struct TextTicket {
+  uint32_t utt;
+  uint32_t len;
+  uint32_t off16;
+  uint32_t tag;
+};
+constexpr int TICKET_SHIFT = 40;
+constexpr unsigned long long TICKET_ONE = 1ull << TICKET_SHIFT;
 
 struct BeamArgs {
   DeviceTables tables;
@@ -114,8 +123,16 @@
   const HotSet* hot_sets = nullptr;
   const int32_t* utt_hot = nullptr;
   int32_t n_hot_sets = 0;
+  uint8_t* host_pool = nullptr;
+  TextTicket* tickets = nullptr;
+  unsigned long long* tickets_written = nullptr;
+  uint32_t ticket_gen = 0;
 };
 int launch_beam(const BeamArgs& a, std::string* err);
+#ifndef CTC_SIM
+void* alloc_host_mapped(size_t bytes, std::string* err);
+int beam_done(int* done, std::string* err);
+#endif
 bool wave_kernel_chosen(const BeamArgs& a);
 bool beam_kernel_depends_on_input(const BeamArgs& a);
 
diff --git a/pyctcdecode_amd/csrc/backend_hip.hip b/pyctcdecode_amd/csrc/backend_hip.hip
--- a/pyctcdecode_amd/csrc/backend_hip.hip
+++ b/pyctcdecode_amd/csrc/backend_hip.hip
@@ -95,6 +95,24 @@
   return p;
 }
 void release_host(void* p) { (void)hipHostFree(p); }
+void* alloc_host_mapped(size_t bytes, std::string* err) {
+  void* p = nullptr;
+  hipError_t e = hipHostMalloc(&p, bytes ? bytes : 16, hipHostMallocMapped | hipHostMallocCoherent);
+  if (e != hipSuccess) {
+    if (err) *err = std::string("hipHostMalloc(") + std::to_string(bytes) + ", mapped | coherent): " + hipGetErrorString(e);
+    return nullptr;
+  }
+  return p;
+}
+int beam_done(int* done, std::string* err) {
+  const hipError_t e = hipEventQuery(g_ev[2]);
+  *done = e == hipErrorNotReady ? 0 : 1;
+  if (e != hipSuccess && e != hipErrorNotReady) {
+    if (err) *err = std::string("hipEventQuery: ") + hipGetErrorString(e);
+    return -1;
+  }
+  return 0;
+}
 int h2d(void* d, const void* s, size_t n, std::string* err) {
   HIP_TRY(hipMemcpyAsync(d, s, n, hipMemcpyHostToDevice, g_stream));
   HIP_TRY(hipStreamSynchronize(g_stream));
@@ -2031,7 +2049,7 @@
     HIP_TRY(hipGetLastError());
     g_last_kernel = 2;
   }
-  if (a.n_utts > 0 && a.params.texts_only && a.text_scratch) {
+  if (a.n_utts > 0 && a.params.texts_only && a.text_scratch && !(wave && a.tickets)) {
     hipLaunchKernelGGL(assemble_texts, dim3((unsigned)a.n_utts), dim3(64), 0, g_stream, a);
     HIP_TRY(hipGetLastError());
   }
diff --git a/pyctcdecode_amd/csrc/beam_wave.h b/pyctcdecode_amd/csrc/beam_wave.h
--- a/pyctcdecode_amd/csrc/beam_wave.h
+++ b/pyctcdecode_amd/csrc/beam_wave.h
@@ -164,6 +164,8 @@
   bool pf_live = false;
   bool run_ok = false;
   unsigned long long t_last = 0;
+  uint32_t text_enode = 0;
+  bool has_text = false;
 
   CTC_HD WaveDecoder(Ctx& c, WaveLds& l, const UttIO& i) : ctx(c), L(l), io(i), lane(c.lane) {}
 
@@ -1574,10 +1576,12 @@
     uint32_t n_out = io.want_out ? n : 0u;
     if (prm().n_best > 0 && n_out > (uint32_t)prm().n_best) n_out = (uint32_t)prm().n_best;
     if (prm().texts_only != 0 && n_out > 0) {
+      const uint64_t a2 = L.pa[L.sel[0] & 0x7FFFFFFFu];
+      const uint32_t d = (uint32_t)(a2 >> 32);
+      text_enode = cold_cur()[d].enode;
+      has_text = true;
       if (lane == 0) {
-        const uint64_t a2 = L.pa[L.sel[0] & 0x7FFFFFFFu];
         const PoolPay& pp = io.pay[((uint32_t)a2 >> 16) & 0xFFFFu];
-        const uint32_t d = (uint32_t)(a2 >> 32);
         OutBeam& ob = io.out[0];
         ob.logit_score = pp.logit;
         ob.lm_score = bits_f64(pp.part_h);
@@ -1588,7 +1592,7 @@
         ob.last_char = NO_CHAR;
         ob.pstart = ob.pend = -1;
         ob.pad[0] = 0;
-        ob.pad[1] = cold_cur()[d].enode;
+        ob.pad[1] = text_enode;
         *io.n_out = 1;
         *io.status = status;
       }
diff --git a/pyctcdecode_amd/csrc/beam_wave_hip.hip b/pyctcdecode_amd/csrc/beam_wave_hip.hip
--- a/pyctcdecode_amd/csrc/beam_wave_hip.hip
+++ b/pyctcdecode_amd/csrc/beam_wave_hip.hip
@@ -7,6 +7,7 @@
 #include "backend.h"
 #include "beam_core.h"
 #include "beam_wave.h"
+#include "text_wave.h"
 #include "wave_ops_hip.h"
 
 namespace ctc {
@@ -137,6 +138,78 @@
     return atomicAdd(p, v);
   }
 };
+
+#ifndef CTC_TEXT_PUBLISH
+#define CTC_TEXT_PUBLISH 2
+#endif
+__device__ __forceinline__ void host_store64(void* p, uint64_t v) {
+#if CTC_TEXT_PUBLISH == 1 || CTC_TEXT_PUBLISH == 5
+  *(uint64_t*)p = v;
+#else
+  __hip_atomic_store((uint64_t*)p, v, __ATOMIC_RELAXED, __HIP_MEMORY_SCOPE_SYSTEM);
+#endif
+}
+__device__ __forceinline__ void host_store128(void* p, u32x4 v) {
+#if CTC_TEXT_PUBLISH == 1 || CTC_TEXT_PUBLISH == 5
+  *(u32x4a*)p = v;
+#elif CTC_TEXT_PUBLISH == 6
+  host_store64(p, (uint64_t)v[0] | ((uint64_t)v[1] << 32));
+  host_store64((char*)p + 8, (uint64_t)v[2] | ((uint64_t)v[3] << 32));
+#else
+  asm volatile("global_store_dwordx4 %0, %1, off sc0 sc1" ::"v"(p), "v"(v) : "memory");
+#endif
+}
+__device__ __forceinline__ void text_order(WaveGpuCtx& ctx) {
+#if CTC_TEXT_PUBLISH == 1 || CTC_TEXT_PUBLISH == 5
+  __builtin_amdgcn_fence(__ATOMIC_RELEASE, "");
+#else
+  ctx.wsync();
+  ctx.vm_wait();
+  ctx.wsync();
+#endif
+}
+__device__ __forceinline__ void hand_text(WaveGpuCtx& ctx, lds_bytes_t smem, int u, uint32_t enode, uint32_t status) {
+  const KernArgs k = ctx.fresh();
+  const uint32_t lane = (uint32_t)ctx.lane;
+  TextLds tl;
+  text_lds_carve(tl, smem);
+  const uint64_t s0 = k->text_soff[u], e0 = k->emit_off[u];
+  uint8_t* scratch = k->text_scratch + s0;
+  const uint32_t cap = (uint32_t)(k->text_soff[u + 1] - s0);
+  ctx.mem_sync();
+  const uint32_t pos = wave_text_backwards(ctx, tl, k->emit_nodes + e0, ctx.tables(), enode, scratch, cap, (uint32_t)(k->emit_off[u + 1] - e0));
+  uint32_t len = cap - pos;
+  const uint32_t room = (len + 15u) & ~15u;
+  unsigned long long old = 0;
+  if (lane == 0) old = atomicAdd(k->tok_pool_head + 1, (unsigned long long)room | TICKET_ONE);
+  old = ctx.bcast64(old, 0);
+  const uint32_t slot = (uint32_t)(old >> TICKET_SHIFT);
+  const unsigned long long base = old & (TICKET_ONE - 1ull);
+  if (base + room > k->text_pool_cap) {
+    status |= ST_TOK_OVERFLOW;
+    len = 0;
+  }
+  ctx.mem_sync();
+#if CTC_TEXT_PUBLISH != 0
+  const uint8_t* src = scratch + pos;
+  uint8_t* dst = k->host_pool + base;
+  for (uint32_t b = lane * 16u; b < len; b += 1024u) {
+    u32x4 v;
+    __builtin_memcpy(&v, src + b, 16);
+    host_store128(dst + b, v);
+  }
+  const bool mine = lane == 0 && slot < (uint32_t)k->n_utts;
+  TextTicket* t = k->tickets + slot;
+  if (mine) host_store64(&t->utt, (uint64_t)(uint32_t)u | ((uint64_t)len << 32));
+  text_order(ctx);
+  if (mine) host_store64(&t->off16, (uint64_t)(uint32_t)(base >> 4) | ((uint64_t)((k->ticket_gen << 8) | (status & 0xFFu)) << 32));
+#if CTC_TEXT_PUBLISH == 1 || CTC_TEXT_PUBLISH == 3
+  text_order(ctx);
+  if (lane == 0) __hip_atomic_fetch_add(k->tickets_written, 1ull, __ATOMIC_RELAXED, __HIP_MEMORY_SCOPE_SYSTEM);
+#endif
+#endif
+  if (lane == 0 && (status & ST_TOK_OVERFLOW)) k->status[u] = status;
+}
 
 template <int BW, int ORD, bool PROF>
 __global__ __launch_bounds__(64) __attribute__((amdgpu_waves_per_eu(BW <= 100 ? 4 : 3, BW <= 100 ? 4 : 3))) void beam_wave(BeamArgs a) {
@@ -190,6 +263,10 @@
   ctx.start_prio(io.T);
   WaveDecoder<WaveGpuCtx, BW, ORD, PROF> dec(ctx, view, io);
   dec.run();
+  if (dec.has_text && ctx.fresh()->tickets) {
+    const KernArgs k = ctx.fresh();
+    hand_text(ctx, (lds_bytes_t)smem, k->order ? k->order[blockIdx.x] : (int)blockIdx.x, dec.text_enode, dec.status);
+  }
   if (rec && threadIdx.x == 0) {
     uint32_t hw, xcc;
     asm volatile("s_getreg_b32 %0, hwreg(HW_REG_HW_ID)" : "=s"(hw));
@@ -202,7 +279,7 @@
 
 template <int BW, int ORD, bool PROF>
 static int launch_wave_p(const BeamArgs& a, hipStream_t stream, std::string* err) {
-  const size_t lds = wave_lds_bytes<BW>();
+  const size_t lds = wave_lds_bytes<BW>() > TEXT_LDS_BYTES ? wave_lds_bytes<BW>() : TEXT_LDS_BYTES;
   HIP_TRY_W(hipFuncSetAttribute((const void*)beam_wave<BW, ORD, PROF>, hipFuncAttributeMaxDynamicSharedMemorySize, (int)lds));
   hipLaunchKernelGGL((beam_wave<BW, ORD, PROF>), dim3((unsigned)a.n_utts), dim3(64), lds, stream, a);
   return 0;
diff --git a/pyctcdecode_amd/csrc/pytexts.c b/pyctcdecode_amd/csrc/pytexts.c
--- a/pyctcdecode_amd/csrc/pytexts.c
+++ b/pyctcdecode_amd/csrc/pytexts.c
@@ -37,6 +37,47 @@
     }
     PyList_SET_ITEM(list, (Py_ssize_t)i, s);
   }
+  return list;
+}
+
+int ctcdec_py_text_sink(void* user, int32_t n, const int32_t* utt, const char* const* utf8, const int64_t* len) {
+  PyGILState_STATE g = PyGILState_Ensure();
+  PyObject* list = (PyObject*)user;
+  const Py_ssize_t size = PyList_GET_SIZE(list);
+  for (int32_t i = 0; i < n; ++i) {
+    if (utt[i] < 0 || (Py_ssize_t)utt[i] >= size) continue;
+    PyObject* s = PyUnicode_DecodeUTF8(utf8[i], (Py_ssize_t)len[i], "strict");
+    if (!s) {
+      PyObject *type, *value, *tb;
+      PyErr_Fetch(&type, &value, &tb);
+      PyErr_NormalizeException(&type, &value, &tb);
+      s = value ? value : (Py_INCREF(Py_None), Py_None);
+      Py_XDECREF(type);
+      Py_XDECREF(tb);
+    }
+    PyList_SetItem(list, (Py_ssize_t)utt[i], s);
+  }
+  PyGILState_Release(g);
+  return 0;
+}
+
+PyObject* ctcdec_py_text_sink_finish(PyObject* list) {
+  const Py_ssize_t size = PyList_GET_SIZE(list);
+  for (Py_ssize_t i = 0; i < size; ++i) {
+    PyObject* s = PyList_GET_ITEM(list, i);
+    if (PyUnicode_Check(s)) continue;
+    if (PyExceptionInstance_Check(s)) {
+      Py_INCREF(s);
+      PyList_SetSlice(list, 0, size, NULL);
+      PyErr_SetObject((PyObject*)Py_TYPE(s), s);
+      Py_DECREF(s);
+    } else {
+      PyList_SetSlice(list, 0, size, NULL);
+      PyErr_Format(PyExc_RuntimeError, "no text was delivered for utterance %zd", i);
+    }
+    return NULL;
+  }
+  Py_INCREF(list);
   return list;
 }
 
diff --git a/pyctcdecode_amd/decoder.py b/pyctcdecode_amd/decoder.py
--- a/pyctcdecode_amd/decoder.py
+++ b/pyctcdecode_amd/decoder.py
@@ -1017,11 +1017,12 @@
         p.token_frames = 0
         return p
 
-    def _run(self, logits_list: Sequence[Any], params: B.Params, hotwords, start_states=None, hot_sets=None):
+    def _run(self, logits_list: Sequence[Any], params: B.Params, hotwords, start_states=None, hot_sets=None, sink=None):
         with self._call_lock:
-            return self._run_locked(logits_list, params, hotwords, start_states, hot_sets)
-
-    def _run_locked(self, logits_list: Sequence[Any], params: B.Params, hotwords, start_states=None, hot_sets=None):
+            return self._run_locked(logits_list, params, hotwords, start_states, hot_sets, sink)
+
+    def _run_locked(self, logits_list: Sequence[Any], params: B.Params, hotwords, start_states=None, hot_sets=None,
+                    sink=None):
         if hot_sets is None:
             self._set_hotwords(hotwords)
         batch = _Batch(logits_list, len(self._idx2vocab))
@@ -1056,10 +1057,13 @@
         res = C.c_void_p()
         if hot_sets is not None:
             self._arm_hot_sets(hot_sets)
-        self._lib.check(
-            self._lib.dll.ctcdec_decode_batch(self._handle, ptrs, frames, n, batch.dtype, int(batch.is_device),
-                                              C.byref(params), st_arr, C.byref(res))
-        )
+        if sink is not None:
+            rc = self._lib.dll.ctcdec_decode_texts(self._handle, ptrs, frames, n, batch.dtype, int(batch.is_device),
+                                                   C.byref(params), sink[0], sink[1], C.byref(res))
+        else:
+            rc = self._lib.dll.ctcdec_decode_batch(self._handle, ptrs, frames, n, batch.dtype, int(batch.is_device),
+                                                   C.byref(params), st_arr, C.byref(res))
+        self._lib.check(rc)
         ms = (C.c_double * 3)()
         self._lib.dll.ctcdec_result_timing(res, ms)
         self.last_timing_ms = (float(ms[0]), float(ms[1]), float(ms[2]))
@@ -1194,6 +1198,12 @@
             params.token_frames = fold or 1
         else:
             params.texts_only = 1
+            sink = B.text_sink()
+            if sink is not None:
+                texts = [None] * len(logits_list)
+                res = self._run(logits_list, params, hotwords, hot_sets=hot_sets, sink=(sink[0], texts))
+                self._lib.dll.ctcdec_result_free(res)
+                return sink[1](texts)
         res = self._run(logits_list, params, hotwords, hot_sets=hot_sets)
         try:
             texts = self._texts(res)
```

Result: faster. 191.7 million, median of 5 (+3.7%).
